# ProjectZKM/Ziren

Measured on AMD Instinct MI355X. Metric: shard-proofs/sec, higher is better.
Workload: dtype u32

## Files before the change

### ziren_amd/csrc/api_tracegen.hpp

```cpp
#pragma once
size_t zkm_tracegen_alu_width(int chip) { return chip >= 0 && chip < tracegen::NUM_ALU_CHIPS ? (size_t)tracegen::chip_width(chip) : 0; }

static size_t padded_trace_rows(size_t n_records, int fixed_log2_rows, const char* what) {
  size_t height = 16;
  if (fixed_log2_rows >= 0) {
    if (fixed_log2_rows > 30) throw std::runtime_error(std::string(what) + ": fixed log2 rows out of range");
    height = (size_t)1 << fixed_log2_rows;
    if (n_records > height) throw std::runtime_error(std::string(what) + ": fixed log2 rows is too small");
  } else {
    while (height < n_records) height <<= 1;
  }
  return height;
}

struct TraceBatch {
  zkm_ctx* ctx;
  std::vector<void*> scratch;
  std::vector<zkm_matrix*> made;
  std::vector<std::vector<zkm_syscall_event>> host_keep;
  enum { F_CPU, F_GLOBAL, F_SYSCALL_CORE };
  static constexpr int MAX_FLAGS = 256;
  uint32_t* d_flags = nullptr;
  std::vector<int> flag_kind;
  explicit TraceBatch(zkm_ctx* c) : ctx(c) {}
  zkm_matrix* matrix(size_t h, size_t w) {
    zkm_matrix* m = new zkm_matrix();
    made.push_back(m);
    m->h = h; m->w = w;
    m->d = ctx->alloc_n<uint32_t>(std::max<size_t>(h * w, 1));
    return m;
  }
  void* temp(size_t bytes) { void* p = ctx->alloc(bytes); scratch.push_back(p); return p; }
  const uint32_t* events(const void* ev, size_t bytes) {
    uint32_t* owned = nullptr;
    const uint32_t* d = ctx->events_on_device(ev, bytes, &owned);
    if (owned) scratch.push_back(owned);
    return d;
  }
  uint32_t* flag(int kind) {
    if (!d_flags) {
      d_flags = (uint32_t*)temp(MAX_FLAGS * 4);
      HIP_CHECK(hipMemsetAsync(d_flags, 0, MAX_FLAGS * 4, ctx->stream));
    }
    if ((int)flag_kind.size() == MAX_FLAGS) throw std::runtime_error("zkm_tracegen: too many generators in one batch");
    flag_kind.push_back(kind);
    return d_flags + flag_kind.size() - 1;
  }
  void finish(const char* mark) {
    const uint32_t* h_flags = flag_kind.empty() ? nullptr : ctx->download_async(d_flags, flag_kind.size());
    ctx->mark(mark);
    ctx->end_timing(false);
    for (size_t i = 0; i < flag_kind.size(); i++) {
      const uint32_t f = h_flags[i];
      if (!f) continue;
      if (flag_kind[i] == F_CPU) {
        if (f & 1) throw std::runtime_error("zkm_tracegen_cpu: an event's pc lies outside the program");
        throw std::runtime_error("zkm_tracegen_cpu: an event's clock does not fit 24 bits (a shard holds fewer than 2^24 / 5 cycles)");
      }
      if (flag_kind[i] == F_GLOBAL) {
        if (f & tracegen::GLOBAL_ERR_NOT_U16) throw std::runtime_error("zkm_tracegen_global: message[0] of an event is not a u16");
        if (f & tracegen::GLOBAL_ERR_NO_POINT) throw std::runtime_error("zkm_tracegen_global: a message has no curve point within 256 offsets");
        if (f & tracegen::GLOBAL_ERR_INFINITY) throw std::runtime_error("zkm_tracegen_global: the running sum reached the point at infinity");
        throw std::runtime_error("zkm_tracegen_global: a message's point has the running sum's x-coordinate");
      }
      throw std::runtime_error("zkm_tracegen_syscall: fixed log2 rows is too small");
    }
    for (void* p : scratch) ctx->release(p);
    scratch.clear();
    made.clear();
    host_keep.clear();
  }
  void abort() {
    (void)hipStreamSynchronize(ctx->stream);
    for (void* p : scratch) ctx->release(p);
    for (zkm_matrix* m : made) { if (m->d) ctx->release(m->d); delete m; }
    scratch.clear(); made.clear(); host_keep.clear();
  }
};

static zkm_matrix* enqueue_rows(TraceBatch& b, int chip, const void* events, size_t n_events, int fixed_log2_rows, zkm_byte_lookups* blu,
                                const uint32_t* n_dev = nullptr, const uint32_t* dev_events_given = nullptr, size_t height_given = 0) {
  static_assert(sizeof(zkm_alu_event) == 28 && sizeof(zkm_jump_event) == 28 && sizeof(zkm_mov_cond_event) == 28 &&
                sizeof(zkm_comp_alu_event) == 64, "event records mirror the #[repr(C)] executor structs");
  zkm_ctx* ctx = b.ctx;
  if (chip < 0 || chip >= tracegen::NUM_CHIPS) throw std::runtime_error("zkm_tracegen: unknown chip");
  if (n_events && !events && !dev_events_given) throw std::runtime_error("zkm_tracegen: null events");
  const size_t height = height_given ? height_given : padded_trace_rows(n_events, fixed_log2_rows, "zkm_tracegen_alu");
  const size_t w = (size_t)tracegen::chip_width(chip);
  zkm_matrix* m = b.matrix(height, w);
  m->uniform_rows = n_events == 0 && !n_dev && !dev_events_given;
  const size_t event_bytes = 4 * (size_t)tracegen::event_words(chip);
  const uint32_t* dev_events = dev_events_given ? dev_events_given : b.events(events, n_events * event_bytes);
  uint32_t* counts = blu ? blu->counts : nullptr;
  if (n_dev) {
    if (chip != tracegen::SYSCALL_CORE) throw std::runtime_error("zkm_tracegen: a device-side event count is for SyscallCore only");
    const int tiles = counts ? tracegen::TILES_PER_BLOCK : 1;
    KLAUNCH(ctx, "tracegen_alu", event_bytes * n_events + 4.0 * height * w, tracegen::alu_rows_counted<tracegen::SYSCALL_CORE>,
            dim3(div_up(height, (size_t)tiles * tracegen::THREADS)), dim3(tracegen::THREADS), counts ? 2 * tracegen::HASH_SLOTS * sizeof(uint32_t) : 0,
            dev_events, n_dev, height, m->d, counts, tiles);
    return m;
  }
  switch (chip) {
    case tracegen::ADD_SUB: launch_alu_rows<tracegen::ADD_SUB>(ctx, dev_events, n_events, height, m->d, counts); break;
    case tracegen::BITWISE: launch_alu_rows<tracegen::BITWISE>(ctx, dev_events, n_events, height, m->d, counts); break;
    case tracegen::LT: launch_alu_rows<tracegen::LT>(ctx, dev_events, n_events, height, m->d, counts); break;
    case tracegen::SHIFT_LEFT: launch_alu_rows<tracegen::SHIFT_LEFT>(ctx, dev_events, n_events, height, m->d, counts); break;
    case tracegen::SHIFT_RIGHT: launch_alu_rows<tracegen::SHIFT_RIGHT>(ctx, dev_events, n_events, height, m->d, counts); break;
    case tracegen::CLO_CLZ: launch_alu_rows<tracegen::CLO_CLZ>(ctx, dev_events, n_events, height, m->d, counts); break;
    case tracegen::JUMP: launch_alu_rows<tracegen::JUMP>(ctx, dev_events, n_events, height, m->d, counts); break;
    case tracegen::MOV_COND: launch_alu_rows<tracegen::MOV_COND>(ctx, dev_events, n_events, height, m->d, counts); break;
    case tracegen::BRANCH: launch_alu_rows<tracegen::BRANCH>(ctx, dev_events, n_events, height, m->d, counts); break;
    case tracegen::MUL: launch_alu_rows<tracegen::MUL>(ctx, dev_events, n_events, height, m->d, counts); break;
    case tracegen::DIVREM: launch_alu_rows<tracegen::DIVREM>(ctx, dev_events, n_events, height, m->d, counts); break;
    case tracegen::MEMORY_INSTRS: launch_alu_rows<tracegen::MEMORY_INSTRS>(ctx, dev_events, n_events, height, m->d, counts); break;
    case tracegen::SYSCALL_INSTRS: launch_alu_rows<tracegen::SYSCALL_INSTRS>(ctx, dev_events, n_events, height, m->d, counts); break;
    case tracegen::MISC_INSTRS: launch_alu_rows<tracegen::MISC_INSTRS>(ctx, dev_events, n_events, height, m->d, counts); break;
    case tracegen::SYSCALL_CORE: launch_alu_rows<tracegen::SYSCALL_CORE>(ctx, dev_events, n_events, height, m->d, counts); break;
    case tracegen::SYSCALL_PRECOMPILE: launch_alu_rows<tracegen::SYSCALL_PRECOMPILE>(ctx, dev_events, n_events, height, m->d, counts); break;
  }
  return m;
}

static int tracegen_single(zkm_ctx* ctx, zkm_matrix** out, const std::function<zkm_matrix*(TraceBatch&)>& enqueue) {
  API_BEGIN
  std::lock_guard<std::mutex> lk(ctx->mu);
  HIP_CHECK(hipSetDevice(ctx->device));
  CallScope call_scope(ctx);
  ctx->begin_timing();
  TraceBatch b(ctx);
  zkm_matrix* m = nullptr;
  try {
    m = enqueue(b);
    b.finish("trace generation");
  } catch (...) {
    b.abort();
    throw;
  }
  *out = m;
  API_END
}

static int tracegen_events(zkm_ctx* ctx, int chip, const void* events, size_t n_events, int fixed_log2_rows,
                           zkm_byte_lookups* blu, zkm_matrix** out) {
  return tracegen_single(ctx, out, [&](TraceBatch& b) { return enqueue_rows(b, chip, events, n_events, fixed_log2_rows, blu); });
}

int zkm_tracegen_alu(zkm_ctx* ctx, int chip, const zkm_alu_event* events, size_t n_events, int fixed_log2_rows,
                     zkm_byte_lookups* blu, zkm_matrix** out) {
  if (chip < 0 || chip >= tracegen::NUM_ALU_CHIPS) { g_err = "zkm_tracegen_alu: unknown chip"; return -1; }
  return tracegen_events(ctx, chip, events, n_events, fixed_log2_rows, blu, out);
}
size_t zkm_tracegen_jump_width(void) { return (size_t)tracegen::chip_width(tracegen::JUMP); }
int zkm_tracegen_jump(zkm_ctx* ctx, const zkm_jump_event* events, size_t n_events, int fixed_log2_rows, zkm_matrix** out) {
  return tracegen_events(ctx, tracegen::JUMP, events, n_events, fixed_log2_rows, nullptr, out);
}

static zkm_matrix* enqueue_flat(TraceBatch& b, const uint32_t* words, size_t n_words, size_t width, int fixed_log2_rows) {
  zkm_ctx* ctx = b.ctx;
  if (width == 0) throw std::runtime_error("zkm_tracegen_flat: zero width");
  if (n_words && !words) throw std::runtime_error("zkm_tracegen_flat: null records");
  const size_t rows = (n_words + width - 1) / width;
  size_t height = 16;
  if (fixed_log2_rows >= 0) {
    if (fixed_log2_rows > 30) throw std::runtime_error("zkm_tracegen_flat: fixed log2 rows out of range");
    height = (size_t)1 << fixed_log2_rows;
    if (rows > height) throw std::runtime_error("zkm_tracegen_flat: fixed log2 rows is too small");
  } else {
    while (height < rows) height <<= 1;
  }
  zkm_matrix* m = b.matrix(height, width);
  m->uniform_rows = n_words == 0;
  const uint32_t* dev = n_words ? b.events(words, n_words * 4) : nullptr;
  ctx->flush_staged();
  hipLaunchKernelGGL(open::flat_rows, dim3(div_up(width, 32), div_up(height, 32)), dim3(32, 8), 0, ctx->stream, dev, n_words, m->d, width, height);
  LAUNCH_CHECK();
  return m;
}
int zkm_tracegen_flat(zkm_ctx* ctx, const uint32_t* words, size_t n_words, size_t width, int fixed_log2_rows, zkm_matrix** out) {
  return tracegen_single(ctx, out, [&](TraceBatch& b) { return enqueue_flat(b, words, n_words, width, fixed_log2_rows); });
}

size_t zkm_tracegen_branch_width(void) { return (size_t)tracegen::chip_width(tracegen::BRANCH); }
int zkm_tracegen_branch(zkm_ctx* ctx, const zkm_branch_event* events, size_t n_events, int fixed_log2_rows, zkm_byte_lookups* blu,
                        zkm_matrix** out) {
  return tracegen_events(ctx, tracegen::BRANCH, events, n_events, fixed_log2_rows, blu, out);
}
size_t zkm_tracegen_mul_width(void) { return (size_t)tracegen::chip_width(tracegen::MUL); }
int zkm_tracegen_mul(zkm_ctx* ctx, const zkm_comp_alu_event* events, size_t n_events, int fixed_log2_rows, zkm_byte_lookups* blu,
                     zkm_matrix** out) {
  return tracegen_events(ctx, tracegen::MUL, events, n_events, fixed_log2_rows, blu, out);
}
size_t zkm_tracegen_memory_instrs_width(void) { return (size_t)tracegen::chip_width(tracegen::MEMORY_INSTRS); }
int zkm_tracegen_memory_instrs(zkm_ctx* ctx, const zkm_mem_instr_event* events, size_t n_events, int fixed_log2_rows, zkm_byte_lookups* blu,
                               zkm_matrix** out) {
  static_assert(sizeof(zkm_mem_instr_event) == 64, "event records mirror the #[repr(C)] executor structs");
  return tracegen_events(ctx, tracegen::MEMORY_INSTRS, events, n_events, fixed_log2_rows, blu, out);
}
size_t zkm_tracegen_syscall_instrs_width(void) { return (size_t)tracegen::chip_width(tracegen::SYSCALL_INSTRS); }
int zkm_tracegen_syscall_instrs(zkm_ctx* ctx, const zkm_syscall_event* events, size_t n_events, int fixed_log2_rows, zkm_matrix** out) {
  static_assert(sizeof(zkm_syscall_event) == 56, "event records mirror the #[repr(C)] executor structs");
  return tracegen_events(ctx, tracegen::SYSCALL_INSTRS, events, n_events, fixed_log2_rows, nullptr, out);
}
size_t zkm_tracegen_misc_instrs_width(void) { return (size_t)tracegen::chip_width(tracegen::MISC_INSTRS); }
int zkm_tracegen_misc_instrs(zkm_ctx* ctx, const zkm_misc_event* events, size_t n_events, int fixed_log2_rows, zkm_byte_lookups* blu,
                             zkm_matrix** out) {
  static_assert(sizeof(zkm_misc_event) == 60, "event records mirror the #[repr(C)] executor structs");
  return tracegen_events(ctx, tracegen::MISC_INSTRS, events, n_events, fixed_log2_rows, blu, out);
}
size_t zkm_tracegen_divrem_width(void) { return (size_t)tracegen::chip_width(tracegen::DIVREM); }
int zkm_tracegen_divrem(zkm_ctx* ctx, const zkm_comp_alu_event* events, size_t n_events, int fixed_log2_rows, zkm_byte_lookups* blu,
                        zkm_matrix** out) {
  return tracegen_events(ctx, tracegen::DIVREM, events, n_events, fixed_log2_rows, blu, out);
}
size_t zkm_tracegen_mov_cond_width(void) { return (size_t)tracegen::chip_width(tracegen::MOV_COND); }
int zkm_tracegen_mov_cond(zkm_ctx* ctx, const zkm_mov_cond_event* events, size_t n_events, int fixed_log2_rows, zkm_matrix** out) {
  return tracegen_events(ctx, tracegen::MOV_COND, events, n_events, fixed_log2_rows, nullptr, out);
}

size_t zkm_tracegen_cpu_width(void) { return (size_t)tracegen::CPU_WIDTH; }
static zkm_matrix* enqueue_cpu(TraceBatch& b, const zkm_cpu_event* events, size_t n_events, const zkm_instruction* program, size_t n_instr,
                               uint32_t pc_base, uint32_t shard, int fixed_log2_rows, int program_fixed_log2_rows, zkm_byte_lookups* blu,
                               zkm_matrix** program_mults_out) {
  static_assert(sizeof(zkm_cpu_event) == 4 * tracegen::CPU_EVENT_WORDS && sizeof(zkm_instruction) == 4 * tracegen::INSTRUCTION_WORDS,
                "event records mirror the #[repr(C)] executor structs");
  zkm_ctx* ctx = b.ctx;
  if (n_events && (!events || !program || !n_instr)) throw std::runtime_error("zkm_tracegen_cpu: null events or program");
  const size_t height = padded_trace_rows(n_events, fixed_log2_rows, "zkm_tracegen_cpu");
  const size_t pheight = program_mults_out ? padded_trace_rows(n_instr, program_fixed_log2_rows, "zkm_tracegen_cpu (program)") : 0;
  zkm_matrix* m = b.matrix(height, tracegen::CPU_WIDTH);
  zkm_matrix* pm = program_mults_out ? b.matrix(pheight, 1) : nullptr;
  if (pm) HIP_CHECK(hipMemsetAsync(pm->d, 0, pheight * 4, ctx->stream));
  const uint32_t* dev_events = b.events(events, n_events * sizeof(zkm_cpu_event));
  const uint32_t* d_program = (const uint32_t*)ctx->upload_staged(program, n_instr * sizeof(zkm_instruction), &b.scratch);
  uint32_t* d_bad = b.flag(TraceBatch::F_CPU);
  uint32_t* counts = blu ? blu->counts : nullptr;
  const int tiles = counts ? tracegen::TILES_PER_BLOCK : 1;
  KLAUNCH(ctx, "tracegen_cpu", 280.0 * n_events + 4.0 * height * tracegen::CPU_WIDTH, tracegen::cpu_rows,
          dim3(div_up(height, (size_t)tiles * tracegen::THREADS)), dim3(tracegen::THREADS),
          counts ? 2 * tracegen::HASH_SLOTS * sizeof(uint32_t) : 0, dev_events, n_events, d_program, n_instr,
          pc_base, shard, height, m->d, counts, tiles, (int*)d_bad, pm ? pm->d : (uint32_t*)nullptr);
  if (pm) {
    hipLaunchKernelGGL(tracegen::counts_to_field, dim3(div_up(pheight, 256)), dim3(256), 0, ctx->stream, pm->d, pheight);
    LAUNCH_CHECK();
    *program_mults_out = pm;
  }
  return m;
}

int zkm_tracegen_cpu_and_program(zkm_ctx* ctx, const zkm_cpu_event* events, size_t n_events, const zkm_instruction* program, size_t n_instr,
                                 uint32_t pc_base, uint32_t shard, int fixed_log2_rows, int program_fixed_log2_rows, zkm_byte_lookups* blu,
                                 zkm_matrix** out, zkm_matrix** program_mults_out) {
  zkm_matrix* pm = nullptr;
  const int rc = tracegen_single(ctx, out, [&](TraceBatch& b) {
    return enqueue_cpu(b, events, n_events, program, n_instr, pc_base, shard, fixed_log2_rows, program_fixed_log2_rows, blu, program_mults_out ? &pm : nullptr);
  });
  if (rc == 0 && program_mults_out) *program_mults_out = pm;
  return rc;
}

int zkm_tracegen_cpu(zkm_ctx* ctx, const zkm_cpu_event* events, size_t n_events, const zkm_instruction* program, size_t n_instr,
                     uint32_t pc_base, uint32_t shard, int fixed_log2_rows, zkm_byte_lookups* blu, zkm_matrix** out) {
  return zkm_tracegen_cpu_and_program(ctx, events, n_events, program, n_instr, pc_base, shard, fixed_log2_rows, -1, blu, out, nullptr);
}

int zkm_tracegen_program(zkm_ctx* ctx, const zkm_instruction* program, size_t n_instr, uint32_t pc_base, int fixed_log2_rows,
                         zkm_matrix** out) {
  API_BEGIN
  std::lock_guard<std::mutex> lk(ctx->mu);
  HIP_CHECK(hipSetDevice(ctx->device));
  CallScope call_scope(ctx);
  if (n_instr && !program) throw std::runtime_error("zkm_tracegen_program: null program");
  const size_t height = padded_trace_rows(n_instr, fixed_log2_rows, "zkm_tracegen_program");
  ctx->begin_call();
  zkm_matrix* m = new zkm_matrix();
  m->h = height; m->w = tracegen::PROGRAM_PREP_WIDTH;
  uint32_t* d_program = nullptr;
  try {
    m->d = ctx->alloc_n<uint32_t>(height * m->w);
    d_program = (uint32_t*)ctx->alloc(std::max<size_t>(n_instr * sizeof(zkm_instruction), 4));
    if (n_instr) HIP_CHECK(hipMemcpyAsync(d_program, program, n_instr * sizeof(zkm_instruction), hipMemcpyHostToDevice, ctx->stream));
    hipLaunchKernelGGL(tracegen::program_rows, dim3(div_up(height, 256)), dim3(256), 0, ctx->stream, (const uint32_t*)d_program, n_instr,
                       pc_base, height, m->d);
    LAUNCH_CHECK();
    ctx->sync(ctx->stream);
  } catch (...) {
    if (d_program) ctx->release(d_program);
    if (m->d) ctx->release(m->d);
    delete m;
    throw;
  }
  ctx->release(d_program);
  *out = m;
  API_END
}

int zkm_tracegen_program_mults(zkm_ctx* ctx, const zkm_cpu_event* events, size_t n_events, size_t n_instr, uint32_t pc_base,
                               int fixed_log2_rows, zkm_matrix** out) {
  API_BEGIN
  std::lock_guard<std::mutex> lk(ctx->mu);
  HIP_CHECK(hipSetDevice(ctx->device));
  CallScope call_scope(ctx);
  if (n_events && !events) throw std::runtime_error("zkm_tracegen_program_mults: null events");
  const size_t height = padded_trace_rows(n_instr, fixed_log2_rows, "zkm_tracegen_program_mults");
  ctx->begin_call();
  zkm_matrix* m = new zkm_matrix();
  m->h = height; m->w = 1;
  uint32_t* d_events = nullptr;
  try {
    m->d = ctx->alloc_n<uint32_t>(height);
    HIP_CHECK(hipMemsetAsync(m->d, 0, height * 4, ctx->stream));
    const uint32_t* dev_events = ctx->events_on_device(events, n_events * sizeof(zkm_cpu_event), &d_events);
    if (n_events) {
      hipLaunchKernelGGL(tracegen::program_count, dim3(div_up(n_events, 256)), dim3(256), 0, ctx->stream, dev_events, n_events,
                         n_instr, pc_base, m->d);
      LAUNCH_CHECK();
    }
    hipLaunchKernelGGL(tracegen::counts_to_field, dim3(div_up(height, 256)), dim3(256), 0, ctx->stream, m->d, height);
    LAUNCH_CHECK();
    ctx->sync(ctx->stream);
  } catch (...) {
    if (d_events) ctx->release(d_events);
    if (m->d) ctx->release(m->d);
    delete m;
    throw;
  }
  ctx->release(d_events);
  *out = m;
  API_END
}

static zkm_matrix* enqueue_memory_local(TraceBatch& b, const zkm_memory_local_event* events, size_t n_events, int fixed_log2_rows) {
  static_assert(sizeof(zkm_memory_local_event) == 28, "event records mirror the #[repr(C)] executor structs");
  zkm_ctx* ctx = b.ctx;
  if (n_events && !events) throw std::runtime_error("zkm_tracegen_memory_local: null events");
  const size_t height = padded_trace_rows(div_up(n_events, (size_t)tracegen::MEMORY_LOCAL_ENTRIES), fixed_log2_rows, "zkm_tracegen_memory_local");
  zkm_matrix* m = b.matrix(height, tracegen::MEMORY_LOCAL_WIDTH);
  const uint32_t* dev_events = b.events(events, n_events * sizeof(zkm_memory_local_event));
  ctx->flush_staged();
  hipLaunchKernelGGL(tracegen::memory_local_rows, dim3(div_up(height * tracegen::MEMORY_LOCAL_ENTRIES, (size_t)256)), dim3(256), 0, ctx->stream,
                     dev_events, n_events, height, m->d);
  LAUNCH_CHECK();
  return m;
}

int zkm_tracegen_memory_local(zkm_ctx* ctx, const zkm_memory_local_event* events, size_t n_events, int fixed_log2_rows, zkm_matrix** out) {
  return tracegen_single(ctx, out, [&](TraceBatch& b) { return enqueue_memory_local(b, events, n_events, fixed_log2_rows); });
}

static zkm_matrix* enqueue_global(TraceBatch& b, const zkm_global_lookup_event* events, size_t n_events, int fixed_log2_rows, zkm_byte_lookups* blu) {
  static_assert(sizeof(zkm_global_lookup_event) == 32, "event records mirror the #[repr(C)] executor structs");
  zkm_ctx* ctx = b.ctx;
  if (n_events && !events) throw std::runtime_error("zkm_tracegen_global: null events");
  if (!blu) throw std::runtime_error("zkm_tracegen_global: null byte lookups");
  const size_t height = padded_trace_rows(n_events, fixed_log2_rows, "zkm_tracegen_global");
  zkm_matrix* m = b.matrix(height, tracegen::GLOBAL_WIDTH);
  const uint32_t* d_events = b.events(events, n_events * sizeof(zkm_global_lookup_event));
  uint32_t* d_err = b.flag(TraceBatch::F_GLOBAL);
  std::vector<uint32_t*> levels;
  std::vector<size_t> sizes;
  for (size_t n = n_events + 1;; n = div_up(n, (size_t)tracegen::SCAN_CHUNK)) {
    levels.push_back((uint32_t*)b.temp(n * tracegen::POINT_WORDS * sizeof(uint32_t)));
    sizes.push_back(n);
    if (n <= (size_t)tracegen::SCAN_BLOCK) break;
  }
  const double bytes = 32.0 * n_events + 4.0 * height * tracegen::GLOBAL_WIDTH;
  KLAUNCH(ctx, "tracegen_global_points", bytes, tracegen::global_point_rows, dim3(div_up(height, (size_t)256)), dim3(256), 0,
          d_events, n_events, height, m->d, levels[0], blu->counts, d_err);
  for (size_t l = 0; l + 1 < levels.size(); l++)
    KLAUNCH(ctx, "tracegen_global_scan", 64.0 * sizes[l], tracegen::global_scan_reduce, dim3(div_up(sizes[l + 1], (size_t)64)), dim3(64), 0,
            (const uint32_t*)levels[l], sizes[l], levels[l + 1], sizes[l + 1]);
  KLAUNCH(ctx, "tracegen_global_scan", 128.0 * sizes.back(), tracegen::global_scan_block, dim3(1), dim3(tracegen::SCAN_BLOCK), 0, levels.back(),
          sizes.back());
  for (size_t l = levels.size() - 1; l-- > 0;)
    KLAUNCH(ctx, "tracegen_global_scan", 128.0 * sizes[l], tracegen::global_scan_apply, dim3(div_up(sizes[l + 1], (size_t)64)), dim3(64), 0, levels[l],
            sizes[l], (const uint32_t*)levels[l + 1], sizes[l + 1]);
  KLAUNCH(ctx, "tracegen_global_accum", bytes, tracegen::global_accum_rows, dim3(div_up(height, (size_t)256)), dim3(256), 0,
          (const uint32_t*)levels[0], n_events, height, m->d, d_err);
  return m;
}

int zkm_tracegen_global(zkm_ctx* ctx, const zkm_global_lookup_event* events, size_t n_events, int fixed_log2_rows, zkm_byte_lookups* blu,
                        zkm_matrix** out) {
  return tracegen_single(ctx, out, [&](TraceBatch& b) { return enqueue_global(b, events, n_events, fixed_log2_rows, blu); });
}

static zkm_matrix* enqueue_poseidon2_wide(TraceBatch& b, const uint32_t* events, size_t n_events, int fixed_log2_rows) {
  zkm_ctx* ctx = b.ctx;
  if (n_events && !events) throw std::runtime_error("zkm_tracegen_poseidon2_wide: null events");
  const size_t height = padded_trace_rows(n_events, fixed_log2_rows, "zkm_tracegen_poseidon2_wide");
  zkm_matrix* m = b.matrix(height, tracegen::POSEIDON2_WIDE_WIDTH);
  const uint32_t* d_events = n_events ? b.events(events, n_events * 128) : (const uint32_t*)b.temp(4);
  KLAUNCH(ctx, "tracegen_poseidon2_wide", 128.0 * n_events + 4.0 * height * tracegen::POSEIDON2_WIDE_WIDTH, tracegen::poseidon2_wide_rows,
          dim3(div_up(height, (size_t)tracegen::THREADS)), dim3(tracegen::THREADS), 0, d_events, n_events, height, m->d);
  return m;
}
int zkm_tracegen_poseidon2_wide(zkm_ctx* ctx, const uint32_t* events, size_t n_events, int fixed_log2_rows, zkm_matrix** out) {
  return tracegen_single(ctx, out, [&](TraceBatch& b) { return enqueue_poseidon2_wide(b, events, n_events, fixed_log2_rows); });
}

static zkm_matrix* enqueue_syscall(TraceBatch& b, const zkm_syscall_event* events, size_t n_events, int precompile, int fixed_log2_rows, zkm_byte_lookups* blu) {
  static_assert(sizeof(zkm_syscall_event) == 56, "event records mirror the #[repr(C)] executor structs");
  zkm_ctx* ctx = b.ctx;
  if (precompile) return enqueue_rows(b, tracegen::SYSCALL_PRECOMPILE, events, n_events, fixed_log2_rows, blu);
  if (n_events && !events) throw std::runtime_error("zkm_tracegen: null events");
  if (n_events && ctx->prefetched.count(events)) {
    const uint32_t* d_all = b.events(events, n_events * sizeof(zkm_syscall_event));
    const size_t cap = fixed_log2_rows >= 0 ? std::min(n_events, padded_trace_rows(0, fixed_log2_rows, "zkm_tracegen_syscall")) : n_events;
    uint32_t* d_kept = (uint32_t*)b.temp(cap * sizeof(zkm_syscall_event));
    uint32_t* d_n = (uint32_t*)b.temp(4);
    uint32_t* d_flag = b.flag(TraceBatch::F_SYSCALL_CORE);
    KLAUNCH(ctx, "tracegen_syscall_compact", 2.0 * n_events * sizeof(zkm_syscall_event), tracegen::syscall_core_compact, dim3(1), dim3(1024), 0,
            d_all, n_events, d_kept, d_n, cap, d_flag);
    if (fixed_log2_rows < 0) {
      const uint32_t* h_n = ctx->download_async(d_n, 1);
      ctx->sync(ctx->stream);
      return enqueue_rows(b, tracegen::SYSCALL_CORE, nullptr, *h_n, -1, blu, nullptr, d_kept);
    }
    return enqueue_rows(b, tracegen::SYSCALL_CORE, nullptr, cap, fixed_log2_rows, blu, d_n, d_kept, (size_t)1 << fixed_log2_rows);
  }
  b.host_keep.emplace_back();
  std::vector<zkm_syscall_event>& kept = b.host_keep.back();
  for (size_t i = 0; i < n_events; i++) {
    const uint32_t code = events[i].a_record.prev_value;
    if (((code >> 16) & 0xff) == 1 || ((code >> 8) & 0xff) != 0) kept.push_back(events[i]);
  }
  return enqueue_rows(b, tracegen::SYSCALL_CORE, kept.empty() ? nullptr : (const void*)kept.data(), kept.size(), fixed_log2_rows, blu);
}

int zkm_tracegen_syscall(zkm_ctx* ctx, const zkm_syscall_event* events, size_t n_events, int precompile, int fixed_log2_rows, zkm_byte_lookups* blu,
                         zkm_matrix** out) {
  return tracegen_single(ctx, out, [&](TraceBatch& b) { return enqueue_syscall(b, events, n_events, precompile, fixed_log2_rows, blu); });
}

int zkm_tracegen_memory_global(zkm_ctx* ctx, const zkm_memory_init_finalize_event* events, size_t n_events, uint32_t previous_addr, int fixed_log2_rows,
                               zkm_matrix** out) {
  API_BEGIN
  static_assert(sizeof(zkm_memory_init_finalize_event) == 16, "event records mirror the #[repr(C)] executor structs");
  std::lock_guard<std::mutex> lk(ctx->mu);
  HIP_CHECK(hipSetDevice(ctx->device));
  CallScope call_scope(ctx);
  if (n_events && !events) throw std::runtime_error("zkm_tracegen_memory_global: null events");
  const size_t height = padded_trace_rows(n_events, fixed_log2_rows, "zkm_tracegen_memory_global");
  std::vector<zkm_memory_init_finalize_event> sorted(events, events + n_events);
  std::stable_sort(sorted.begin(), sorted.end(), [](const zkm_memory_init_finalize_event& a, const zkm_memory_init_finalize_event& b) { return a.addr < b.addr; });
  ctx->begin_timing();
  zkm_matrix* m = new zkm_matrix();
  m->h = height; m->w = tracegen::MEMORY_GLOBAL_WIDTH;
  uint32_t* d_events = nullptr;
  int* d_bad = nullptr;
  try {
    m->d = ctx->alloc_n<uint32_t>(height * m->w);
    d_events = (uint32_t*)ctx->alloc(std::max<size_t>(n_events * 16, 4));
    d_bad = (int*)ctx->alloc(4);
    HIP_CHECK(hipMemsetAsync(d_bad, 0, 4, ctx->stream));
    if (n_events) HIP_CHECK(hipMemcpyAsync(d_events, sorted.data(), n_events * 16, hipMemcpyHostToDevice, ctx->stream));
    KLAUNCH(ctx, "tracegen_memory_global", 16.0 * n_events + 4.0 * height * m->w, tracegen::memory_global_rows, dim3(div_up(height, (size_t)tracegen::THREADS)),
            dim3(tracegen::THREADS), 0, (const uint32_t*)d_events, n_events, previous_addr, height, m->d, d_bad);
    int bad = 0;
    HIP_CHECK(hipMemcpyAsync(&bad, d_bad, 4, hipMemcpyDeviceToHost, ctx->stream));
    ctx->mark("trace generation");
    ctx->end_timing(false);
    if (bad) throw std::runtime_error("zkm_tracegen_memory_global: addresses are not strictly increasing (from the previous shard's last address on)");
  } catch (...) {
    if (d_events) ctx->release(d_events);
    if (d_bad) ctx->release(d_bad);
    if (m->d) ctx->release(m->d);
    delete m;
    throw;
  }
  ctx->release(d_events);
  ctx->release(d_bad);
  *out = m;
  API_END
}

int zkm_tracegen_poseidon2_permute(zkm_ctx* ctx, const zkm_poseidon2_permute_event* events, size_t n_events, int fixed_log2_rows, zkm_byte_lookups* blu,
                                   zkm_matrix** out) {
  API_BEGIN
  static_assert(sizeof(zkm_poseidon2_permute_event) == 4 * tracegen::POSEIDON2_PERMUTE_EVENT_WORDS, "flattened Poseidon2PermuteEvent is 99 words");
  std::lock_guard<std::mutex> lk(ctx->mu);
  HIP_CHECK(hipSetDevice(ctx->device));
  CallScope call_scope(ctx);
  if (n_events && !events) throw std::runtime_error("zkm_tracegen_poseidon2_permute: null events");
  const size_t height = padded_trace_rows(n_events, fixed_log2_rows, "zkm_tracegen_poseidon2_permute");
  ctx->begin_timing();
  zkm_matrix* m = new zkm_matrix();
  m->h = height; m->w = tracegen::POSEIDON2_PERMUTE_WIDTH;
  uint32_t* d_events = nullptr;
  int* d_bad = nullptr;
  try {
    m->d = ctx->alloc_n<uint32_t>(height * m->w);
    const size_t ev_bytes = n_events * sizeof(zkm_poseidon2_permute_event);
    d_events = (uint32_t*)ctx->alloc(std::max<size_t>(ev_bytes, 4));
    d_bad = (int*)ctx->alloc(4);
    HIP_CHECK(hipMemsetAsync(d_bad, 0, 4, ctx->stream));
    if (n_events) HIP_CHECK(hipMemcpyAsync(d_events, events, ev_bytes, hipMemcpyHostToDevice, ctx->stream));
    uint32_t* counts = blu ? blu->counts : nullptr;
    KLAUNCH(ctx, "tracegen_poseidon2_permute", (double)ev_bytes + 4.0 * height * m->w, tracegen::poseidon2_permute_rows,
            dim3(div_up(height, (size_t)tracegen::THREADS)), dim3(tracegen::THREADS), counts ? 2 * tracegen::HASH_SLOTS * sizeof(uint32_t) : 0,
            (const uint32_t*)d_events, n_events, height, m->d, counts, d_bad);
    int bad = 0;
    HIP_CHECK(hipMemcpyAsync(&bad, d_bad, 4, hipMemcpyDeviceToHost, ctx->stream));
    ctx->mark("trace generation");
    ctx->end_timing(false);
    if (bad) throw std::runtime_error("zkm_tracegen_poseidon2_permute: a state word is not a field element, or the post-state is not the permutation of the pre-state");
  } catch (...) {
    if (d_events) ctx->release(d_events);
    if (d_bad) ctx->release(d_bad);
    if (m->d) ctx->release(m->d);
    delete m;
    throw;
  }
  ctx->release(d_events);
  ctx->release(d_bad);
  *out = m;
  API_END
}

int zkm_tracegen_keccak_sponge(zkm_ctx* ctx, const zkm_keccak_sponge_block* blocks, size_t n_blocks, int fixed_log2_rows, zkm_byte_lookups* blu,
                               zkm_matrix** out) {
  API_BEGIN
  static_assert(sizeof(zkm_keccak_sponge_block) == 4 * tracegen::KECCAK_SPONGE_BLOCK_WORDS, "a KeccakSpongeEvent block is 337 words");
  std::lock_guard<std::mutex> lk(ctx->mu);
  HIP_CHECK(hipSetDevice(ctx->device));
  CallScope call_scope(ctx);
  if (n_blocks && !blocks) throw std::runtime_error("zkm_tracegen_keccak_sponge: null blocks");
  const size_t height = padded_trace_rows(24 * n_blocks, fixed_log2_rows, "zkm_tracegen_keccak_sponge");
  ctx->begin_timing();
  zkm_matrix* m = new zkm_matrix();
  m->h = height; m->w = tracegen::KECCAK_SPONGE_WIDTH;
  uint32_t* d_blocks = nullptr;
  int* d_bad = nullptr;
// ... 875 lines not shown
```

### ziren_amd/csrc/host_ctx.hpp

```cpp
#pragma once
static thread_local std::string g_err;

#define HIP_CHECK(expr)                                                                          \
  do {                                                                                           \
    hipError_t _e = (expr);                                                                      \
    if (_e != hipSuccess)                                                                        \
      throw std::runtime_error(std::string(#expr) + ": " + hipGetErrorString(_e) + " (" + __FILE__ + ":" + \
                               std::to_string(__LINE__) + ")");                                  \
  } while (0)
#define LAUNCH_CHECK() HIP_CHECK(hipGetLastError())
#define KLAUNCH(ctx, name, bytes, kernel, grid, block, lds, ...)                                        \
  do {                                                                                                   \
    (ctx)->flush_staged();                                                                               \
    if ((ctx)->kbegin(name, (double)(bytes))) {                                                          \
       \
      hipExtLaunchKernelGGL(kernel, grid, block, lds, (ctx)->cur, (ctx)->krecs.back().start,             \
                            (ctx)->krecs.back().stop, 0, __VA_ARGS__);                                   \
    } else {                                                                                             \
      hipLaunchKernelGGL(kernel, grid, block, lds, (ctx)->cur, __VA_ARGS__);                             \
    }                                                                                                    \
    LAUNCH_CHECK();                                                                                      \
  } while (0)

static inline int log2_strict(size_t n) {
  int k = 0;
  while (((size_t)1 << k) < n) k++;
  if (((size_t)1 << k) != n) throw std::runtime_error("height is not a power of two");
  return k;
}
static inline unsigned div_up(size_t a, size_t b) { return (unsigned)((a + b - 1) / b); }
static inline uint64_t fnv1a(const uint32_t* w, size_t n);
static inline uint64_t perm_key(const uint32_t* lookups, size_t len, uint32_t log_quotient_degree) {
  return fnv1a(lookups, len) * 1099511628211ull + log_quotient_degree + 1;
}
static inline uint64_t fnv1a(const uint32_t* w, size_t n) {
  uint64_t h = 1469598103934665603ull;
  const unsigned char* p = (const unsigned char*)w;
  for (size_t i = 0; i < n * 4; i++) { h ^= p[i]; h *= 1099511628211ull; }
  return h;
}

namespace chal {
static void duplexing(zkm_challenger* c) {
  for (uint32_t i = 0; i < c->num_inputs; i++) c->sponge_state[i] = c->input_buffer[i];
  c->num_inputs = 0;
  p2::permute_host(c->sponge_state);
  for (int i = 0; i < 8; i++) c->output_buffer[i] = c->sponge_state[i];
  c->num_outputs = 8;
}
static void observe(zkm_challenger* c, uint32_t v) {
  c->num_outputs = 0;
  c->input_buffer[c->num_inputs++] = v;
  if (c->num_inputs == 8) duplexing(c);
}
static void observe_slice(zkm_challenger* c, const uint32_t* v, size_t n) {
  for (size_t i = 0; i < n; i++) observe(c, v[i]);
}
static void observe_ext(zkm_challenger* c, const E4& e) { observe_slice(c, e.c, 4); }
static uint32_t sample(zkm_challenger* c) {
  if (c->num_inputs != 0 || c->num_outputs == 0) duplexing(c);
  return c->output_buffer[--c->num_outputs];
}
static E4 sample_ext(zkm_challenger* c) {
  E4 e;
  for (int i = 0; i < 4; i++) e.c[i] = sample(c);
  return e;
}
static uint32_t sample_bits(zkm_challenger* c, uint32_t bits) {
  return kb::from_monty(sample(c)) & ((1u << bits) - 1);
}
}

enum HandleKind { H_MATRIX = 1, H_PCS_DATA = 2, H_PK = 3, H_MAIN_DATA = 4 };
struct HandleTable {
  std::mutex mu;
  std::unordered_map<const void*, int> live;
  static HandleTable& get() { static HandleTable t; return t; }
  void add(const void* p, int kind) { std::lock_guard<std::mutex> lk(mu); live[p] = kind; }
  void drop(const void* p) { std::lock_guard<std::mutex> lk(mu); live.erase(p); }
  bool is_live(const void* p, int kind) { std::lock_guard<std::mutex> lk(mu); auto it = live.find(p); return it != live.end() && it->second == kind; }
};
template <int KIND>
struct Handle {
  Handle() { HandleTable::get().add(this, KIND); }
  Handle(const Handle&) { HandleTable::get().add(this, KIND); }
  Handle& operator=(const Handle&) { return *this; }
  ~Handle() { HandleTable::get().drop(this); }
};
static inline void check_handle(const void* p, int kind, const char* fn, const char* what) {
  if (!p) throw std::runtime_error(std::string(fn) + ": null " + what);
  if (!HandleTable::get().is_live(p, kind)) throw std::runtime_error(std::string(fn) + ": " + what + " is not a live handle (freed, or never returned by this library)");
}

struct zkm_ctx {
  int device = 0;
  hipStream_t stream = nullptr;
  hipStream_t stream2 = nullptr;
  hipStream_t up_dma = nullptr, up_tr = nullptr;
  uint32_t* up_stage[2] = {nullptr, nullptr};
  hipEvent_t up_freed[2] = {nullptr, nullptr}, up_landed[2] = {nullptr, nullptr};
  bool up_freed_set[2] = {false, false};
  int up_next = 0;
  static constexpr size_t UP_SLAB_BYTES = (size_t)32 << 20;
  hipStream_t cur = nullptr;
  hipStream_t ev_dma = nullptr;
  struct Prefetched { size_t bytes; hipEvent_t landed; };
  std::map<const void*, Prefetched> prefetched;
  const uint32_t* events_on_device(const void* events, size_t bytes, uint32_t** owned) {
    *owned = nullptr;
    auto it = prefetched.find(events);
    if (it != prefetched.end()) {
      if (bytes > it->second.bytes) throw std::runtime_error("zkm_tracegen: more events asked for than zkm_events_upload_async copied");
      HIP_CHECK(hipStreamWaitEvent(stream, it->second.landed, 0));
      return (const uint32_t*)events;
    }
    uint32_t* d = (uint32_t*)alloc(std::max<size_t>(bytes, 4));
    *owned = d;
    if (bytes) HIP_CHECK(hipMemcpyAsync(d, events, bytes, hipMemcpyHostToDevice, stream));
    return d;
  }
  std::mutex mu;
  std::multimap<size_t, void*> free_list;
  std::map<void*, size_t> live;
  std::map<int, uint32_t*> tw_fwd, tw_inv;
  std::vector<std::pair<std::string, hipEvent_t>> marks;
  std::vector<hipEvent_t> event_pool;
  std::vector<std::string> timing_names;
  std::vector<float> timing_ms;
  struct KRec { const char* name; double bytes; hipEvent_t start, stop; };
  struct KStat { double ms = 0, bytes = 0; uint32_t calls = 0; };
  std::vector<KRec> krecs;
  std::map<std::string, KStat> kstats;
  int kernel_timing = 2;
  bool lde_overlap = !(getenv("ZKM_LDE_OVERLAP") && atoi(getenv("ZKM_LDE_OVERLAP")) == 0);
  bool rows_up_front = !(getenv("ZKM_ROWS_UP_FRONT") && atoi(getenv("ZKM_ROWS_UP_FRONT")) == 0);
  bool root_poll = !(getenv("ZKM_ROOT_POLL") && atoi(getenv("ZKM_ROOT_POLL")) == 0);
  int root_spin_before_yield = getenv("ZKM_ROOT_SPIN") ? atoi(getenv("ZKM_ROOT_SPIN")) : 4096;
  int root_sleep_ns = getenv("ZKM_ROOT_SLEEP_NS") ? atoi(getenv("ZKM_ROOT_SLEEP_NS")) : 0;
  bool host_wait_blocking = getenv("ZKM_HOST_WAIT") && !strcmp(getenv("ZKM_HOST_WAIT"), "blocking");
  int wait_sleep_ns = getenv("ZKM_WAIT_SLEEP_NS") ? atoi(getenv("ZKM_WAIT_SLEEP_NS")) : 20000;
  struct TimerSlack {
    long saved = -1;
    void tighten() {
      if (saved >= 0) return;
      saved = prctl(PR_GET_TIMERSLACK, 0, 0, 0, 0);
      if (saved >= 0) prctl(PR_SET_TIMERSLACK, 1000UL, 0, 0, 0);
    }
    ~TimerSlack() { if (saved >= 0) prctl(PR_SET_TIMERSLACK, (unsigned long)saved, 0, 0, 0); }
  };
  static void sleep_ns(long ns, TimerSlack& slack) {
    slack.tighten();
    timespec ts{0, ns};
    nanosleep(&ts, nullptr);
  }
  void sync(hipStream_t s) {
    if (!host_wait_blocking) { HIP_CHECK(hipStreamSynchronize(s)); return; }
    TimerSlack slack;
    for (int i = 0;; i++) {
      const hipError_t e = hipStreamQuery(s);
      if (e == hipSuccess) return;
      if (e != hipErrorNotReady) HIP_CHECK(e);
      if (i >= 4) sleep_ns(wait_sleep_ns, slack);
    }
  }
  std::map<uint64_t, std::vector<hipFunction_t>> quotient_fns;
  std::map<uint64_t, hipFunction_t> quotient_uniform_fns;
  std::map<uint64_t, hipFunction_t> perm_fns;
  std::vector<hipModule_t> modules;
  hipEvent_t get_event() {
    hipEvent_t e;
    if (!event_pool.empty()) { e = event_pool.back(); event_pool.pop_back(); }
    else HIP_CHECK(hipEventCreate(&e));
    return e;
  }
  std::string timing_only;
  bool kbegin(const char* name, double bytes) {
    if (!(kernel_timing == 1 || (kernel_timing == 2 && bytes >= 262144.0) || (kernel_timing == 3 && timing_only == name))) return false;
    KRec r{name, bytes, get_event(), get_event()};
    krecs.push_back(r);
    return true;
  }

  char* pin = nullptr;
  size_t pin_cap = (size_t)32 << 20, pin_off = 0;
  void* pin_alloc(size_t bytes) {
    if (!pin) HIP_CHECK(hipHostMalloc((void**)&pin, pin_cap, hipHostMallocCoherent));
    size_t off = (pin_off + 63) & ~(size_t)63;
    if (off + bytes > pin_cap) return nullptr;
    pin_off = off + bytes;
    return pin + off;
  }
  void begin_call() {
    sync(stream);
    sync(stream2);
    cur = stream;
    side_join();
    pin_off = 0;
    dirty_lo = SIZE_MAX; dirty_hi = 0;
  }
  char* arena = nullptr;
  size_t dirty_lo = SIZE_MAX, dirty_hi = 0;
  void* upload_staged(const void* src, size_t bytes, std::vector<void*>* scratch = nullptr) {
    const size_t room = bytes ? bytes : 4;
    void* h = room <= ((size_t)1 << 20) ? pin_alloc(room) : nullptr;
    if (!h) return upload(src, bytes, scratch);
    if (!arena) HIP_CHECK(hipMalloc((void**)&arena, pin_cap));
    if (bytes) memcpy(h, src, bytes);
    bytes = room;
    const size_t off = (char*)h - pin;
    dirty_lo = std::min(dirty_lo, off);
    dirty_hi = std::max(dirty_hi, off + bytes);
    return arena + off;
  }
  void flush_staged() {
    if (dirty_hi <= dirty_lo) return;
    HIP_CHECK(hipMemcpyAsync(arena + dirty_lo, pin + dirty_lo, dirty_hi - dirty_lo, hipMemcpyHostToDevice, stream));
    dirty_lo = SIZE_MAX; dirty_hi = 0;
    if (cur != stream) {
      hipEvent_t e = get_event();
      HIP_CHECK(hipEventRecord(e, stream));
      HIP_CHECK(hipStreamWaitEvent(cur, e, 0));
      event_pool.push_back(e);
    }
  }
  std::vector<void*> side_deferred;
  hipEvent_t side_done = nullptr;
  bool side_pending = false;
  void release_here(void* p) {
    if (cur != stream) side_deferred.push_back(p);
    else release(p);
  }
  void side_begin() {
    hipEvent_t e = get_event();
    HIP_CHECK(hipEventRecord(e, stream));
    HIP_CHECK(hipStreamWaitEvent(stream2, e, 0));
    event_pool.push_back(e);
    cur = stream2;
  }
  void side_end() {
    if (!side_done) HIP_CHECK(hipEventCreateWithFlags(&side_done, hipEventDisableTiming));
    HIP_CHECK(hipEventRecord(side_done, stream2));
    cur = stream;
    side_pending = true;
  }
  void side_join() {
    if (!side_pending) return;
    HIP_CHECK(hipStreamWaitEvent(stream, side_done, 0));
    for (void* p : side_deferred) release(p);
    side_deferred.clear();
    side_pending = false;
  }
  void* upload(const void* src, size_t bytes, std::vector<void*>* scratch) {
    void* d = alloc(bytes);
    if (scratch) scratch->push_back(d);
    if (bytes == 0) return d;
    void* h = pin_alloc(bytes);
    if (h) {
      memcpy(h, src, bytes);
      HIP_CHECK(hipMemcpyAsync(d, h, bytes, hipMemcpyHostToDevice, cur));
    } else {
      HIP_CHECK(hipMemcpyAsync(d, src, bytes, hipMemcpyHostToDevice, cur));
      sync(cur);
    }
    return d;
  }
  template <class T>
  T* download_async(const T* dev, size_t count) {
    T* h = (T*)pin_alloc(count * sizeof(T));
    if (!h) throw std::runtime_error("pinned staging ring exhausted");
    HIP_CHECK(hipMemcpyAsync(h, dev, count * sizeof(T), hipMemcpyDeviceToHost, stream));
    return h;
  }

  size_t pool_bytes = 0;
  size_t pool_limit = getenv("ZKM_POOL_LIMIT_MB") ? (size_t)atoll(getenv("ZKM_POOL_LIMIT_MB")) << 20 : 0;
  std::vector<void*> call_allocs;
  int call_depth = 0;
  void drop_cached() {
    if (free_list.empty()) return;
    (void)hipStreamSynchronize(stream);
    if (stream2) (void)hipStreamSynchronize(stream2);
    for (auto& kv : free_list) { (void)hipFree(kv.second); pool_bytes -= kv.first; }
    free_list.clear();
  }
  void* alloc(size_t bytes) {
    if (bytes == 0) bytes = 4;
    bytes = (bytes + 255) & ~(size_t)255;
    auto it = free_list.find(bytes);
    void* p;
    if (it != free_list.end()) {
      p = it->second;
      free_list.erase(it);
    } else {
      if (pool_limit && pool_bytes + bytes > pool_limit) drop_cached();
      if (pool_limit && pool_bytes + bytes > pool_limit)
        throw std::runtime_error("out of device memory: " + std::to_string(bytes) + " bytes on top of " + std::to_string(pool_bytes) +
                                 " held would cross the context's pool limit of " + std::to_string(pool_limit) + " bytes");
      hipError_t e = hipMalloc(&p, bytes);
      if (e != hipSuccess) {
        (void)hipGetLastError();
        drop_cached();
        e = hipMalloc(&p, bytes);
      }
      if (e != hipSuccess) {
        (void)hipGetLastError();
        throw std::runtime_error(std::string("out of device memory: hipMalloc of ") + std::to_string(bytes) + " bytes failed (" + hipGetErrorString(e) + "), " +
                                 std::to_string(pool_bytes) + " bytes held by this context's pool");
      }
      pool_bytes += bytes;
    }
    live[p] = bytes;
    if (call_depth > 0) call_allocs.push_back(p);
    return p;
  }
  template <class T>
  T* alloc_n(size_t n) { return (T*)alloc(n * sizeof(T)); }
  void release(void* p) {
    if (!p) return;
    auto it = live.find(p);
    if (it == live.end()) return;
    free_list.insert({it->second, p});
    live.erase(it);
  }
  void mark(const char* name) {
    hipEvent_t e = get_event();
    HIP_CHECK(hipEventRecord(e, stream));
    marks.push_back({name, e});
  }
  void begin_timing() {
    begin_call();
    for (auto& m : marks) event_pool.push_back(m.second);
    marks.clear();
    for (auto& r : krecs) { event_pool.push_back(r.start); if (r.stop) event_pool.push_back(r.stop); }
    krecs.clear();
    mark("begin");
  }
  void end_timing(bool append) {
    sync(stream);
    sync(stream2);
    if (!append) { timing_names.clear(); timing_ms.clear(); kstats.clear(); }
    for (auto& r : krecs) {
      float ms = 0;
      if (r.stop) HIP_CHECK(hipEventElapsedTime(&ms, r.start, r.stop));
      KStat& k = kstats[r.name];
      k.ms += ms; k.bytes += r.bytes; k.calls++;
    }
    for (size_t i = 1; i < marks.size(); i++) {
      float ms = 0;
      HIP_CHECK(hipEventElapsedTime(&ms, marks[i - 1].second, marks[i].second));
      timing_names.push_back(marks[i].first);
      timing_ms.push_back(ms);
    }
  }
  const uint32_t* twiddles(int log_size, bool inverse) {
    auto& tab = inverse ? tw_inv : tw_fwd;
    auto it = tab.find(log_size);
    if (it != tab.end()) return it->second;
    size_t count = (size_t)1 << log_size;
    uint32_t* d;
    HIP_CHECK(hipMalloc(&d, count * 4));
    uint32_t w = kb::two_adic_generator(log_size);
    if (inverse) w = kb::inv(w);
    if (log_size > 0) {
      hipLaunchKernelGGL(lde::fill_stage_twiddles, dim3(div_up(count / 2, 256), log_size), dim3(256), 0, stream, d, w, log_size);
      LAUNCH_CHECK();
    }
    tab[log_size] = d;
    return d;
  }
  std::map<int, uint32_t*> ct_fwd, ct_inv;
  const uint32_t* twiddles_ct(int log_size, bool inverse) {
    auto& tab = inverse ? ct_inv : ct_fwd;
    auto it = tab.find(log_size);
    if (it != tab.end()) return it->second;
    const size_t count = (size_t)1 << log_size;
    uint32_t* d;
    HIP_CHECK(hipMalloc(&d, count * 4));
    uint32_t w = kb::two_adic_generator(log_size);
    if (inverse) w = kb::inv(w);
    hipLaunchKernelGGL(lde::fill_ct_twiddles, dim3(div_up(count, 256)), dim3(256), 0, stream, d, w, log_size);
    LAUNCH_CHECK();
    tab[log_size] = d;
    return d;
  }
  std::map<int, std::pair<uint32_t*, uint32_t*>> pow_tabs;
  std::pair<const uint32_t*, const uint32_t*> pow_tables(int k) {
    auto it = pow_tabs.find(k);
    if (it != pow_tabs.end()) return {it->second.first, it->second.second};
    const uint32_t n_hi = (uint32_t)(((size_t)1 << k) >> 10);
    uint32_t *lo, *hi;
    HIP_CHECK(hipMalloc(&lo, 1024 * 4));
    HIP_CHECK(hipMalloc(&hi, std::max<uint32_t>(n_hi, 1) * 4));
    hipLaunchKernelGGL(lde::fill_pow_tables, dim3(div_up(std::max<uint32_t>(1024, n_hi), 256)), dim3(256), 0, stream, lo, hi,
                       kb::two_adic_generator(k), n_hi);
    LAUNCH_CHECK();
    pow_tabs[k] = {lo, hi};
    return {lo, hi};
  }
  std::map<std::pair<int, int>, uint32_t*> selector_tabs;
  const uint32_t* selectors(int log_n, int lqd, uint32_t w_q, uint32_t g_inv, const uint32_t* d_consts) {
    auto key = std::make_pair(log_n, lqd);
    auto it = selector_tabs.find(key);
    if (it != selector_tabs.end()) return it->second;
    const size_t Q = (size_t)1 << (log_n + lqd);
    uint32_t* d;
    HIP_CHECK(hipMalloc(&d, 3 * Q * 4));
    flush_staged();
    hipLaunchKernelGGL(stark::fill_selectors, dim3(div_up(Q, 256)), dim3(256), 0, cur, d, log_n + lqd, lqd, w_q, g_inv, d_consts);
    LAUNCH_CHECK();
    selector_tabs[key] = d;
    return d;
  }
  std::map<int, uint32_t*> row_tabs;
  const uint32_t* row_twiddles(int k) {
    auto it = row_tabs.find(k);
    if (it != row_tabs.end()) return it->second;
    const int lb = lde::LOG_ROW_MAX, la = k - lb;
    const size_t n = (size_t)1 << k;
    uint32_t* d;
    HIP_CHECK(hipMalloc(&d, n * 4));
    auto pw = pow_tables(k);
    hipLaunchKernelGGL(lde::fill_row_twiddles, dim3(div_up(n, 256)), dim3(256), 0, stream, d, la, lb, pw.first, pw.second);
    LAUNCH_CHECK();
    row_tabs[k] = d;
    return d;
  }
  struct CosetTabs { uint32_t* twf; uint32_t* cs; };
  std::map<std::tuple<int, int, uint32_t>, CosetTabs> coset_tabs;
  CosetTabs coset_tables(int k, int bl, uint32_t shift) {
    auto key = std::make_tuple(k, bl, shift);
    auto it = coset_tabs.find(key);
    if (it != coset_tabs.end()) return it->second;
    const int lb = lde::LOG_ROW_MAX, la = k - lb;
    const size_t B = (size_t)1 << lb, A = (size_t)1 << la, cosets = (size_t)1 << bl;
    CosetTabs t;
    HIP_CHECK(hipMalloc(&t.twf, cosets * B * 4));
    HIP_CHECK(hipMalloc(&t.cs, cosets * A * 4));
    const uint32_t w_N = kb::two_adic_generator(k + bl), w_B = kb::two_adic_generator(lb);
    const uint32_t n_inv = kb::inv(kb::to_monty((uint32_t)(((size_t)1 << k) % kb::P)));
    uint32_t sj = shift;
    for (size_t j = 0; j < cosets; j++) {
      uint32_t sA = sj;
      for (int i = 0; i < la; i++) sA = kb::sqr(sA);
      hipLaunchKernelGGL(lde::fill_scaled_stage_twiddles, dim3(div_up(B / 2, 256), lb), dim3(256), 0, stream, t.twf + j * B, w_B, lb, sA);
      LAUNCH_CHECK();
      sj = kb::mul(sj, w_N);
    }
    hipLaunchKernelGGL(lde::fill_row_scales, dim3(div_up(A * cosets, 256)), dim3(256), 0, stream, t.cs, shift, w_N, n_inv, (uint32_t)A, (uint32_t)cosets);
    LAUNCH_CHECK();
    coset_tabs[key] = t;
    return t;
  }
  void drop_coset_tables() {
    for (auto& kv : coset_tabs) { (void)hipFree(kv.second.twf); (void)hipFree(kv.second.cs); }
    coset_tabs.clear();
  }
};

struct zkm_matrix : Handle<H_MATRIX> {
  uint32_t* d = nullptr;
  size_t h = 0, w = 0;
  bool owned = true;
  bool uniform_rows = false;
  hipEvent_t ready = nullptr;
};

static inline void wait_ready(hipStream_t stream, const zkm_matrix& m) {
  if (m.ready) HIP_CHECK(hipStreamWaitEvent(stream, m.ready, 0));
}

struct zkm_byte_lookups {
  uint32_t* counts = nullptr;
};

struct Tree {
  const uint32_t* h_root = nullptr;
  uint32_t* digests = nullptr;
  std::vector<size_t> layer_off;
  size_t max_height = 0;
  int log_max = 0;
  const uint32_t* node(int layer, size_t i) const { return digests + (layer_off[layer] + i) * 8; }
};

struct zkm_pcs_data : Handle<H_PCS_DATA> {
  std::vector<zkm_matrix> ldes;
  std::vector<const uint32_t*> evals;
  std::vector<size_t> eval_heights;
  std::vector<uint32_t> domain_shifts;
  std::vector<zkm_matrix> owned_evals;
  Tree tree;
  uint32_t root[8];
  int log_blowup = 1;
  uint32_t* cflags = nullptr;
  std::vector<const uint32_t*> col_flags;
};

struct zkm_pk : Handle<H_PK> {
  std::vector<zkm_matrix> prep;
  std::vector<uint32_t> local_only;
  zkm_pcs_data* data = nullptr;
  uint32_t commit[8];
  uint32_t pc_start;
  uint32_t igcs[14];
};

struct zkm_main_data : Handle<H_MAIN_DATA> {
  std::vector<size_t> order;
  std::vector<zkm_matrix> traces;
  zkm_pcs_data* data = nullptr;
  std::vector<uint32_t> public_values;
};
```

### ziren_amd/csrc/host_open.hpp

```cpp
#pragma once
static E4 host_pow2k(E4 a, int k) { return kb::epow2k(a, k); }

struct Writer {
  uint32_t* dst;
  size_t cap, n = 0;
  Writer(uint32_t* d, size_t c) : dst(d), cap(d ? c : 0) {}
  void u(uint32_t v) { if (n < cap) dst[n] = v; n++; }
  void words(const uint32_t* p, size_t cnt) {
    if (n < cap) memcpy(dst + n, p, std::min(cnt, cap - n) * 4);
    n += cnt;
  }
  void ext(const E4& e) { words(e.c, 4); }
  size_t size() const { return n; }
};

struct RoundMat {
  const uint32_t* evals; size_t n; size_t width; uint32_t shift;
  const zkm_matrix* lde;
  int n_points;
  std::vector<E4> y[2];
  size_t col0 = 0;
};
struct Round { const zkm_pcs_data* data; std::vector<RoundMat> mats; };

static const uint32_t SEPTIC_X[7] = {637514027, 1595065213, 1998064738, 72333738, 1211544370, 822986770, 1518535784};
static const uint32_t SEPTIC_Y[7] = {1604177449, 90440090, 259343427, 140470264, 1162099742, 941559812, 1064053343};

struct ChipMeta {
  const zkm_chip_desc* desc;
  int log_n;
  size_t n;
  int n_lookups, n_sends, perm_ext_w, max_values;
};

static ChipMeta chip_meta(const zkm_chip_desc* d, size_t n, size_t n_public_values) {
  ChipMeta m;
  m.desc = d; m.n = n; m.log_n = log2_strict(n);
  m.n_lookups = m.n_sends = m.max_values = 0;
  const std::string who = std::string(" (chip ") + (d->name ? d->name : "?") + ")";
  if (d->log_quotient_degree > 3) throw std::runtime_error("log_quotient_degree > 3 unsupported" + who);
  if (d->lookups_len) {
    const uint32_t* w = d->lookups;
    const size_t len = d->lookups_len;
    size_t pos = 0;
    auto need = [&](size_t k) { if (pos + k > len) throw std::runtime_error("lookup blob truncated" + who); };
    need(2);
    uint32_t ns = w[pos++], nr = w[pos++];
    if ((uint64_t)ns + nr > 4096) throw std::runtime_error("too many lookups" + who);
    m.n_sends = ns; m.n_lookups = ns + nr;
    for (uint32_t i = 0; i < ns + nr; i++) {
      need(2);
      pos++;
      uint32_t nv = w[pos++];
      if (nv > 64) throw std::runtime_error("lookup with more than 64 values" + who);
      m.max_values = std::max<int>(m.max_values, nv);
      for (uint32_t v = 0; v <= nv; v++) {
        need(2);
        uint32_t nt = w[pos++];
        if (w[pos++] >= kb::P) throw std::runtime_error("lookup constant not a field element" + who);
        need(2 * (size_t)nt);
        for (uint32_t t = 0; t < nt; t++) {
          uint32_t cw = w[pos++], weight = w[pos++];
          uint32_t col = cw & 0x7fffffffu;
          if ((cw >> 31) ? col >= d->main_width : col >= d->prep_width) throw std::runtime_error("lookup column out of range" + who);
          if (weight >= kb::P) throw std::runtime_error("lookup weight not a field element" + who);
        }
      }
    }
    if (pos != len) throw std::runtime_error("lookup blob length mismatch" + who);
  }
  int batch = 1 << d->log_quotient_degree;
  m.perm_ext_w = m.n_lookups ? (m.n_lookups + batch - 1) / batch + 1 : 0;
  if (d->program_len) {
    if (d->program_len < 4 || d->program_len != 4 + 2 * (size_t)d->program[0]) throw std::runtime_error("program blob length mismatch" + who);
    if (d->program[2] != d->num_constraints) throw std::runtime_error("program constraint count mismatch" + who);
    const uint32_t ne = std::max<uint32_t>(d->program[1], 1), nb = std::max<uint32_t>(d->program[3], 1);
    if (ne > 256 || nb > 256) throw std::runtime_error("program register count out of range" + who);
    size_t asserts = 0;
    for (uint32_t k = 0; k < d->program[0]; k++) {
      uint32_t w0 = d->program[4 + 2 * k], imm = d->program[5 + 2 * k];
      uint32_t op = w0 & 0xff, dst = (w0 >> 8) & 0xff, ra = (w0 >> 16) & 0xff, rb = w0 >> 24;
      bool ok = true;
      switch (op) {
        case ZKM_OP_LD_MAIN: ok = dst < nb && ra < 2 && imm < d->main_width; break;
        case ZKM_OP_LD_PREP: ok = dst < nb && ra < 2 && imm < d->prep_width; break;
        case ZKM_OP_LD_PERM: ok = dst < ne && ra < 2 && imm < (uint32_t)m.perm_ext_w; break;
        case ZKM_OP_LD_CONST: ok = dst < nb && imm < kb::P; break;
        case ZKM_OP_LD_PV: ok = dst < nb && imm < n_public_values; break;
        case ZKM_OP_LD_CHALLENGE: ok = dst < ne && imm < 2; break;
        case ZKM_OP_LD_LOCAL_SUM: ok = dst < ne; break;
        case ZKM_OP_LD_GLOBAL_SUM: ok = dst < nb && imm < 14; break;
        case ZKM_OP_LD_IS_FIRST: case ZKM_OP_LD_IS_LAST: case ZKM_OP_LD_IS_TRANS: ok = dst < nb; break;
        case ZKM_OP_ADD_B: case ZKM_OP_SUB_B: case ZKM_OP_MUL_B: ok = dst < nb && ra < nb && rb < nb; break;
        case ZKM_OP_NEG_B: ok = dst < nb && ra < nb; break;
        case ZKM_OP_ADD_E: case ZKM_OP_SUB_E: case ZKM_OP_MUL_E: ok = dst < ne && ra < ne && rb < ne; break;
        case ZKM_OP_NEG_E: ok = dst < ne && ra < ne; break;
        case ZKM_OP_ADD_EB: case ZKM_OP_SUB_EB: case ZKM_OP_MUL_EB: ok = dst < ne && ra < ne && rb < nb; break;
        case ZKM_OP_ASSERT_B: ok = ra < nb; asserts++; break;
        case ZKM_OP_ASSERT_E: ok = ra < ne; asserts++; break;
        default: ok = false;
      }
      if (!ok) throw std::runtime_error("invalid instruction " + std::to_string(k) + " in constraint program" + who);
    }
    if (asserts != d->num_constraints) throw std::runtime_error("program asserts do not match num_constraints" + who);
  } else if (d->num_constraints) {
    throw std::runtime_error("num_constraints > 0 but no program" + who);
  }
  return m;
}

template <typename Alloc>
static void launch_permutation_trace(zkm_ctx* ctx, const ChipMeta& c, const uint32_t* d_blob, const uint32_t* trace, const uint32_t* prep, const E4& alpha,
                                     const E4* d_beta_powers, zkm_matrix& pt, Alloc&& salloc, std::vector<stark::ScanJob>& scans) {
  const double pbytes = 4.0 * c.n * (c.desc->main_width + c.desc->prep_width + pt.w);
  auto fit = c.desc->lookups_len ? ctx->perm_fns.find(perm_key(c.desc->lookups, c.desc->lookups_len, c.desc->log_quotient_degree)) : ctx->perm_fns.end();
  if (fit != ctx->perm_fns.end()) {
    stark::PermArgs a;
    a.main = trace; a.prep = prep; a.n = c.n; a.alpha = alpha; a.beta_pows = d_beta_powers; a.perm = pt.d;
    size_t arg_size = sizeof(a);
    void* config[] = {HIP_LAUNCH_PARAM_BUFFER_POINTER, &a, HIP_LAUNCH_PARAM_BUFFER_SIZE, &arg_size, HIP_LAUNCH_PARAM_END};
    ctx->flush_staged();
    const bool timed = ctx->kbegin("perm_rows", pbytes);
    HIP_CHECK(hipExtModuleLaunchKernel(fit->second, div_up(c.n, 256) * 256, 1, 1, 256, 1, 1, 0, ctx->cur, nullptr, config,
                                       timed ? ctx->krecs.back().start : nullptr, timed ? ctx->krecs.back().stop : nullptr, 0));
  } else {
    KLAUNCH(ctx, "perm_rows", pbytes, stark::perm_rows, dim3(div_up(c.n, stark::THREADS)), dim3(stark::THREADS), 0,
            d_blob, c.n_lookups, c.n_sends, 1 << c.desc->log_quotient_degree, trace, prep, c.n, alpha, d_beta_powers, pt.d, c.perm_ext_w);
  }
  stark::ScanJob j;
  j.data = pt.d + (size_t)(c.perm_ext_w - 1) * 4 * c.n;
  j.n = c.n;
  j.nchunks = (c.n + stark::SCAN_BLOCK - 1) / stark::SCAN_BLOCK;
  j.totals = (uint32_t*)salloc(j.nchunks * 4 * 4);
  j.blk_end = (scans.empty() ? 0 : scans.back().blk_end) + (uint32_t)(j.nchunks * 4);
  j.pad = 0;
  scans.push_back(j);
}
static void launch_scans(zkm_ctx* ctx, const std::vector<stark::ScanJob>& scans, std::vector<void*>* scratch) {
  if (scans.empty()) return;
  const stark::ScanJob* d = (const stark::ScanJob*)ctx->upload_staged(scans.data(), scans.size() * sizeof(stark::ScanJob), scratch);
  double bytes = 0;
  bool multi = false;
  for (auto& j : scans) { bytes += 32.0 * j.n; multi |= j.nchunks > 1; }
  KLAUNCH(ctx, "scan", bytes, stark::scan_chunks, dim3(scans.back().blk_end), dim3(stark::THREADS), 0, d);
  if (multi) {
    KLAUNCH(ctx, "scan", 0.0, stark::scan_totals, dim3((unsigned)(4 * scans.size())), dim3(stark::THREADS), 0, d);
    KLAUNCH(ctx, "scan", bytes, stark::scan_add_offsets, dim3(scans.back().blk_end), dim3(stark::THREADS), 0, d);
  }
}

struct ShardOpening {
  struct Loose {
    zkm_ctx* ctx;
    std::vector<void*> v;
    void disown(void* p) { v.erase(std::remove(v.begin(), v.end(), p), v.end()); }
    ~Loose() { for (void* p : v) ctx->release(p); }
  };
  struct Guard { zkm_ctx* c; std::vector<zkm_pcs_data*> d; ~Guard() { for (auto p : d) free_pcs_data(c, p); } };

  zkm_ctx* ctx;
  const zkm_pk* pk;
  zkm_main_data* md;
  const zkm_fri_config* fri;
  uint32_t num_pv_elts;
  zkm_challenger* ch;
  hipStream_t st;
  const int bl;
  const size_t nc;
  std::vector<ChipMeta> chips;
  Loose loose;
  std::vector<void*>& scratch;
  Guard guard;
  E4 perm_ch[2];
  uint32_t* d_pv = nullptr;
  std::vector<zkm_matrix> perm_traces;
  std::vector<E4> local_sums;
  std::vector<std::array<uint32_t, 14>> global_sums;
  zkm_pcs_data* perm_data = nullptr;
  std::vector<zkm_matrix> qchunks;
  std::vector<uint32_t> qshifts;
  zkm_pcs_data* quot_data = nullptr;
  E4 zeta;
  std::vector<Round> rounds;
  int log_max = 0;
  std::vector<E4*> ro = std::vector<E4*>(32, nullptr);
  const uint32_t** col_ptr_lde = nullptr;
  const uint32_t** col_ptr_eval = nullptr;
  uint32_t* col_mask = nullptr;
  std::vector<E4*> layers;
  std::vector<Tree> ftrees;
  std::vector<std::array<uint32_t, 8>> commits;
  E4 final_poly;
  uint32_t pow_witness = 0;
  std::vector<size_t> indices;
  const uint32_t* gathered = nullptr;
  std::vector<uint32_t> gathered_big;

  void* salloc(size_t bytes) { void* p = ctx->alloc(bytes); scratch.push_back(p); return p; }

  ShardOpening(zkm_ctx* ctx_, const zkm_pk* pk_, zkm_main_data* md_, const zkm_chip_desc* chips_in, const zkm_fri_config* fri_, uint32_t num_pv_elts_,
               zkm_challenger* ch_)
      : ctx(ctx_), pk(pk_), md(md_), fri(fri_), num_pv_elts(num_pv_elts_), ch(ch_), st(ctx_->stream), bl((int)fri_->log_blowup), nc(md_->order.size()),
        loose{ctx_, {}}, scratch(loose.v), guard{ctx_, {}} {
  for (size_t i = 0; i < nc; i++) chips.push_back(chip_meta(&chips_in[md->order[i]], md->traces[i].h, md->public_values.size()));
  for (size_t i = 0; i < nc; i++) {
    if (chips[i].desc->main_width != md->traces[i].w) throw std::runtime_error("chip main_width does not match its trace");
    if ((int)chips[i].desc->log_quotient_degree > bl) throw std::runtime_error("log_quotient_degree > log_blowup unsupported");
    if (chips[i].desc->prep_index >= 0 && (!pk->data || (size_t)chips[i].desc->prep_index >= pk->prep.size()))
      throw std::runtime_error("chip references a preprocessed trace the proving key does not hold");
  }
  if (bl < 1 || bl > 4) throw std::runtime_error("fri.log_blowup out of range (1..4)");
  if (fri->proof_of_work_bits > 30) throw std::runtime_error("fri.proof_of_work_bits out of range (0..30)");
  if (fri->num_queries < 1 || fri->num_queries > 1024) throw std::runtime_error("fri.num_queries out of range (1..1024)");
  if (num_pv_elts > md->public_values.size()) throw std::runtime_error("num_pv_elts exceeds public_values length");
  chal::observe_slice(ch, md->public_values.data(), num_pv_elts);
  chal::observe_slice(ch, md->data->root, 8);
  perm_ch[0] = chal::sample_ext(ch);
  perm_ch[1] = chal::sample_ext(ch);
  d_pv = (uint32_t*)ctx->upload_staged(md->public_values.data(), md->public_values.size() * 4, &scratch);
  }

  void permutation_phase() {
  perm_traces.assign(nc, zkm_matrix());
  local_sums.assign(nc, kb::ezero());
  global_sums.assign(nc, std::array<uint32_t, 14>());
  std::vector<uint32_t*> d_blobs(nc, nullptr);
  std::vector<stark::ScanJob> scans;
  std::vector<const uint32_t*> sum_src;
  uint32_t* h_sums = nullptr;
  {
    int maxv = 0;
    for (auto& c : chips) maxv = std::max(maxv, c.max_values);
    std::vector<E4> bp(maxv + 2);
    bp[0] = kb::eone();
    for (int i = 1; i < maxv + 2; i++) bp[i] = kb::emul(bp[i - 1], perm_ch[1]);
    E4* d_bp = (E4*)ctx->upload_staged(bp.data(), bp.size() * sizeof(E4), &scratch);
    for (size_t i = 0; i < nc; i++)
      if (chips[i].perm_ext_w > 0) d_blobs[i] = (uint32_t*)ctx->upload_staged(chips[i].desc->lookups, chips[i].desc->lookups_len * 4, &scratch);
    for (size_t i = 0; i < nc; i++) {
      const ChipMeta& c = chips[i];
      zkm_matrix& pt = perm_traces[i];
      pt.h = c.n; pt.w = (size_t)c.perm_ext_w * 4;
      pt.d = ctx->alloc_n<uint32_t>(std::max<size_t>(pt.h * pt.w, 1));
      scratch.push_back(pt.d);
      if (c.perm_ext_w > 0) {
        const uint32_t* prep = c.desc->prep_index >= 0 ? pk->prep[c.desc->prep_index].d : nullptr;
        launch_permutation_trace(ctx, c, (const uint32_t*)d_blobs[i], (const uint32_t*)md->traces[i].d, prep, perm_ch[0], (const E4*)d_bp, pt,
                                 [&](size_t bytes) { return salloc(bytes); }, scans);
        uint32_t* last = pt.d + (size_t)(c.perm_ext_w - 1) * 4 * c.n;
        for (int e = 0; e < 4; e++) sum_src.push_back(last + (size_t)e * c.n + (c.n - 1));
      } else {
        for (int e = 0; e < 4; e++) sum_src.push_back(nullptr);
      }
      if (c.desc->commit_scope_global) {
        const zkm_matrix& m = md->traces[i];
        for (int k = 0; k < 14; k++) sum_src.push_back(m.d + (m.w - 14 + k) * m.h + (m.h - 1));
      } else {
        for (int k = 0; k < 14; k++) sum_src.push_back(nullptr);
      }
    }
    launch_scans(ctx, scans, &scratch);
    const uint32_t* d_zero = (const uint32_t*)ctx->upload_staged("\0\0\0\0", 4, &scratch);
    for (auto& p : sum_src) if (!p) p = d_zero;
    const uint32_t** d_sum_src = (const uint32_t**)ctx->upload_staged(sum_src.data(), sum_src.size() * sizeof(void*), &scratch);
    uint32_t* d_sums = (uint32_t*)salloc(sum_src.size() * 4);
    KLAUNCH(ctx, "gather_words", 0.0, open::gather_words, dim3(div_up(sum_src.size(), open::THREADS)), dim3(open::THREADS), 0,
            (const uint32_t* const*)d_sum_src, sum_src.size(), d_sums);
    h_sums = ctx->download_async(d_sums, sum_src.size());
  }
  ctx->mark("permutation traces");
  perm_data = pcs_commit(ctx, perm_traces, {}, bl);
  guard.d.push_back(perm_data);
  perm_data->owned_evals = perm_traces;
  for (auto& m : perm_traces) loose.disown(m.d);
  ctx->mark("commit permutation");
  for (size_t i = 0; i < nc; i++) {
    for (int e = 0; e < 4; e++) local_sums[i].c[e] = h_sums[18 * i + e];
    if (chips[i].desc->commit_scope_global) {
      for (int k = 0; k < 14; k++) global_sums[i][k] = h_sums[18 * i + 4 + k];
    } else {
      for (int k = 0; k < 7; k++) { global_sums[i][k] = kb::to_monty(SEPTIC_X[k]); global_sums[i][7 + k] = kb::to_monty(SEPTIC_Y[k]); }
    }
  }
  chal::observe_slice(ch, perm_data->root, 8);
  for (size_t i = 0; i < nc; i++) {
    chal::observe_ext(ch, local_sums[i]);
    chal::observe_slice(ch, global_sums[i].data(), 14);
  }
  }

  void quotient_phase() {
  E4 alpha = chal::sample_ext(ch);
  std::vector<std::function<void()>> launches;
  for (size_t i = 0; i < nc; i++) {
    const ChipMeta& c = chips[i];
    const zkm_chip_desc* d = c.desc;
    int lqd = d->log_quotient_degree;
    int lq = c.log_n + lqd;
    size_t Q = (size_t)1 << lq;
    size_t nchunks = (size_t)1 << lqd;
    uint32_t* qbuf = ctx->alloc_n<uint32_t>(Q * 4);
    scratch.push_back(qbuf);
    size_t C = d->num_constraints;
    std::vector<E4> ap(std::max<size_t>(C, 1));
    E4 p = kb::eone();
    for (size_t k = 0; k < C; k++) { ap[C - 1 - k] = p; p = kb::emul(p, alpha); }
    E4* d_ap = (E4*)ctx->upload_staged(ap.data(), ap.size() * sizeof(E4), &scratch);
    uint32_t consts[32] = {0};
    for (int k = 0; k < 14; k++) consts[k] = global_sums[i][k];
    uint32_t w_q = kb::two_adic_generator(lq);
    uint32_t s_pow_n = kb::pow(kb::GEN, (uint64_t)c.n);
    uint32_t wr = kb::two_adic_generator(lqd), wp = kb::ONE;
    for (size_t k = 0; k < nchunks; k++) {
      consts[16 + k] = kb::sub(kb::mul(s_pow_n, wp), kb::ONE);
      consts[24 + k] = kb::inv(consts[16 + k]);
      wp = kb::mul(wp, wr);
    }
    uint32_t* d_consts = (uint32_t*)ctx->upload_staged(consts, sizeof consts, &scratch);
    static const uint32_t empty_prog[4] = {0, 1, 0, 1};
    uint32_t* d_prog = (uint32_t*)ctx->upload_staged(d->program_len ? d->program : empty_prog, std::max<size_t>(d->program_len, 4) * 4, &scratch);
    stark::QuotientArgs a;
    a.program = d_prog + 4;
    a.n_instr = d->program_len ? d->program[0] : 0;
    a.n_regs = d->program_len ? d->program[1] : 1;
    a.main_lde = md->data->ldes[i].d; a.main_stride = md->data->ldes[i].h;
    a.prep_lde = d->prep_index >= 0 ? pk->data->ldes[d->prep_index].d : nullptr;
    a.prep_stride = d->prep_index >= 0 ? pk->data->ldes[d->prep_index].h : 0;
    a.perm_lde = perm_data->ldes[i].d; a.perm_stride = perm_data->ldes[i].h;
    a.log_n = c.log_n; a.lqd = lqd;
    a.alpha_pows = d_ap; a.public_values = d_pv;
    a.perm_alpha = perm_ch[0]; a.perm_beta = perm_ch[1];
    a.local_sum = local_sums[i];
    a.consts = d_consts;
    a.w_q = w_q; a.g_inv = kb::inv(kb::two_adic_generator(c.log_n));
    a.out = qbuf;
    a.selectors = ctx->selectors(c.log_n, lqd, w_q, a.g_inv, d_consts);
    a.n_base_regs = d->program_len ? std::max<uint32_t>(d->program[3], 1) : 1;
    size_t per_thread = (size_t)a.n_regs * 16 + (size_t)a.n_base_regs * 4;
    int bd = 256;
    while (per_thread * bd > 64 * 1024 && bd > 64) bd >>= 1;
    size_t lds = per_thread * bd;
    if (lds > 152 * 1024) throw std::runtime_error(std::string("constraint program of chip ") + d->name + " needs too many registers");
    double qbytes = 4.0 * Q * (d->main_width + d->prep_width + 4.0 * c.perm_ext_w) + 16.0 * Q;
    auto fit = d->program_len ? ctx->quotient_fns.find(fnv1a(d->program, d->program_len)) : ctx->quotient_fns.end();
    const bool special = fit != ctx->quotient_fns.end();
    const std::vector<hipFunction_t>* fns = special ? &fit->second : nullptr;
    hipFunction_t uni_fn = nullptr;
    a.uniforms = nullptr;
    if (special) {
      auto uit = ctx->quotient_uniform_fns.find(fit->first);
      if (uit != ctx->quotient_uniform_fns.end()) {
        uni_fn = uit->second;
        a.uniforms = ctx->alloc_n<uint32_t>(stark::QUOTIENT_UNIFORM_WORDS);
        scratch.push_back(a.uniforms);
      }
    }
    launches.push_back([this, a, fns, uni_fn, Q, bd, lds, qbytes]() mutable {
      if (fns) {
        size_t arg_size = sizeof(a);
        void* config[] = {HIP_LAUNCH_PARAM_BUFFER_POINTER, &a, HIP_LAUNCH_PARAM_BUFFER_SIZE, &arg_size, HIP_LAUNCH_PARAM_END};
        ctx->flush_staged();
        if (uni_fn)
          HIP_CHECK(hipExtModuleLaunchKernel(uni_fn, 64, 1, 1, 64, 1, 1, 0, st, nullptr, config, nullptr, nullptr, 0));
        for (hipFunction_t fn : *fns) {
          const bool timed = ctx->kbegin("quotient", qbytes);
          HIP_CHECK(hipExtModuleLaunchKernel(fn, div_up(Q, 256) * 256, 1, 1, 256, 1, 1, 0, st, nullptr, config,
                                             timed ? ctx->krecs.back().start : nullptr, timed ? ctx->krecs.back().stop : nullptr, 0));
        }
      } else {
        KLAUNCH(ctx, "quotient", qbytes, stark::quotient_kernel, dim3(div_up(Q, bd)), dim3(bd), lds, a);
      }
    });
    uint32_t wqp = kb::ONE;
    for (size_t k = 0; k < nchunks; k++) {
      zkm_matrix m; m.h = c.n; m.w = 4; m.d = qbuf + k * 4 * c.n; m.owned = (k == 0);
      qchunks.push_back(m);
      qshifts.push_back(kb::mul(kb::GEN, wqp));
      wqp = kb::mul(wqp, w_q);
    }
    if (i == 0) { launches[0](); launches[0] = [] {}; }
  }
  for (auto& l : launches) l();
  ctx->mark("quotient values");
  quot_data = pcs_commit(ctx, qchunks, qshifts, bl);
  for (auto& m : qchunks) if (m.owned) { quot_data->owned_evals.push_back(m); loose.disown(m.d); }
  guard.d.push_back(quot_data);
  ctx->mark("commit quotient");
  chal::observe_slice(ch, quot_data->root, 8);
  zeta = chal::sample_ext(ch);
  }

  void opened_values() {
  if (pk->data) {
    Round r; r.data = pk->data;
    for (size_t j = 0; j < pk->prep.size(); j++)
      r.mats.push_back(RoundMat{pk->prep[j].d, pk->prep[j].h, pk->prep[j].w, kb::ONE, &pk->data->ldes[j], pk->local_only[j] ? 1 : 2, {}});
    rounds.push_back(r);
  }
  {
    Round r; r.data = md->data;
    for (size_t i = 0; i < nc; i++)
      r.mats.push_back(RoundMat{md->traces[i].d, md->traces[i].h, md->traces[i].w, kb::ONE, &md->data->ldes[i], chips[i].desc->local_only ? 1 : 2, {}});
    rounds.push_back(r);
    Round rp; rp.data = perm_data;
    for (size_t i = 0; i < nc; i++)
      rp.mats.push_back(RoundMat{perm_traces[i].d, perm_traces[i].h, perm_traces[i].w, kb::ONE, &perm_data->ldes[i], 2, {}});
    rounds.push_back(rp);
    Round rq; rq.data = quot_data;
    for (size_t i = 0; i < qchunks.size(); i++)
      rq.mats.push_back(RoundMat{qchunks[i].d, qchunks[i].h, 4, qshifts[i], &quot_data->ldes[i], 1, {}});
    rounds.push_back(rq);
  }
  {
    std::vector<open::ColJob> cjobs;
    size_t total = 0;
    for (auto& r : rounds)
      for (auto& m : r.mats) {
        m.col0 = total;
        if (m.width == 0) continue;
        const size_t idx = (size_t)(m.lde - r.data->ldes.data());
        const uint32_t* cf = idx < r.data->col_flags.size() ? r.data->col_flags[idx] : nullptr;
        cjobs.push_back(open::ColJob{m.lde->d, m.evals, cf, m.lde->h, m.n, (uint32_t)total, (uint32_t)m.width});
        total += m.width;
      }
    const size_t tn = std::max<size_t>(total, 1);
    col_ptr_lde = (const uint32_t**)salloc(tn * sizeof(void*));
    col_ptr_eval = (const uint32_t**)salloc(tn * sizeof(void*));
    col_mask = (uint32_t*)salloc(tn * sizeof(uint32_t));
    uint32_t* cword = (uint32_t*)salloc(tn * 8 * sizeof(uint32_t));
    if (total) {
      const open::ColJob* d_c = (const open::ColJob*)ctx->upload_staged(cjobs.data(), cjobs.size() * sizeof(open::ColJob), &scratch);
      KLAUNCH(ctx, "col_tables", 0.0, open::build_col_tables, dim3(div_up(total, 256)), dim3(256), 0, d_c, (int)cjobs.size(), (uint32_t)total, col_ptr_lde,
              col_ptr_eval, col_mask, cword);
    }
  }
  {
    std::map<std::pair<size_t, uint32_t>, E4*> wcache;
    size_t total_y = 0;
    for (auto& r : rounds) for (auto& m : r.mats) total_y += m.width * 2;
    E4* d_y = (E4*)salloc(std::max<size_t>(total_y, 1) * sizeof(E4));
    std::vector<open::WeightJob> wjobs;
    std::vector<open::EvalJob> ejobs;
    std::vector<open::SumJob> sjobs;
    uint32_t wblk = 0, eblk = 0, sblk = 0;
    double wbytes = 0, ebytes = 0;
    size_t ypos = 0;
    for (auto& r : rounds)
      for (auto& m : r.mats) {
        if (m.width == 0) continue;
        auto key = std::make_pair(m.n, m.shift);
        E4* wts;
        auto it = wcache.find(key);
        if (it == wcache.end()) {
          int ln = log2_strict(m.n);
          open::WeightJob wj;
          wj.u = kb::escale(zeta, kb::inv(m.shift));
          wj.c = kb::escale(kb::esub_base(host_pow2k(wj.u, ln), kb::ONE), kb::inv(kb::to_monty((uint32_t)(m.n % kb::P))));
          wts = (E4*)salloc(m.n * sizeof(E4));
          wj.w_n = kb::two_adic_generator(ln); wj.n = m.n; wj.out = wts;
          wblk += div_up(div_up(m.n, 4), open::THREADS);
          wj.blk_end = wblk;
          wjobs.push_back(wj);
          wbytes += 16.0 * m.n;
          wcache[key] = wts;
        } else wts = it->second;
        open::EvalJob ej;
        ej.mat = m.evals; ej.weights = wts; ej.n = m.n; ej.width = (int)m.width;
        ej.colptr = col_ptr_eval + m.col0; ej.colmask = col_mask + m.col0;
        ej.groups = (int)div_up(m.width, open::EVAL_COLS);
        ej.split = 1;
        if (m.n >= 4 * open::THREADS) {
          ej.split = (int)std::min<size_t>(std::max<size_t>(1, 3072 / ej.groups), m.n / (4 * open::THREADS));
          ej.kind = m.n_points > 1 ? 1 : 0;
        } else {
          ej.kind = m.n_points > 1 ? 3 : 2;
        }
        ej.lead = 0;
        if (ej.split >= 8 && ej.groups > 1) {
          ej.split &= ~7;
          const uint32_t lead = (8 - eblk % 8) % 8;
          ej.lead = open::EVAL_XCD_AWARE | lead;
          eblk += lead;
        }
        ej.partials = (E4*)salloc((size_t)ej.split * m.width * 2 * sizeof(E4));
        eblk += (uint32_t)ej.groups * (uint32_t)ej.split;
        ej.blk_end = eblk;
        ejobs.push_back(ej);
        ebytes += 4.0 * m.n * m.width + 16.0 * m.n;
        sblk += (uint32_t)(m.width * 2);
        sjobs.push_back(open::SumJob{ej.partials, ej.split, (int)(m.width * 2), (uint32_t)ypos, sblk});
        ypos += m.width * 2;
      }
    if (!ejobs.empty()) {
      const open::WeightJob* d_w = (const open::WeightJob*)ctx->upload_staged(wjobs.data(), wjobs.size() * sizeof(open::WeightJob), &scratch);
      const open::EvalJob* d_e = (const open::EvalJob*)ctx->upload_staged(ejobs.data(), ejobs.size() * sizeof(open::EvalJob), &scratch);
      const open::SumJob* d_s = (const open::SumJob*)ctx->upload_staged(sjobs.data(), sjobs.size() * sizeof(open::SumJob), &scratch);
      KLAUNCH(ctx, "bary_weights", wbytes, open::bary_weights_batch, dim3(wblk), dim3(open::THREADS), 0, d_w);
      KLAUNCH(ctx, "eval_columns", ebytes, open::eval_columns_batch, dim3(eblk), dim3(open::THREADS), 0, d_e);
      KLAUNCH(ctx, "reduce_partials", 0.0, open::reduce_partials_batch, dim3(sblk), dim3(64), 0, d_s, d_y);
    }
    const E4* hy = ctx->download_async(d_y, std::max<size_t>(total_y, 1));
    ctx->sync(st);
    ypos = 0;
    for (auto& r : rounds)
      for (auto& m : r.mats) {
        for (int pt = 0; pt < 2; pt++) m.y[pt].clear();
        if (m.width == 0) continue;
        for (int pt = 0; pt < m.n_points; pt++) {
          m.y[pt].resize(m.width);
          for (size_t c = 0; c < m.width; c++) m.y[pt][c] = hy[ypos + c * 2 + pt];
        }
        ypos += m.width * 2;
      }
  }
  ctx->mark("open: evaluations");
  }

  void reduced_openings() {
  E4 fa = chal::sample_ext(ch);
  log_max = 0;
  std::vector<size_t> count(32, 0);
  size_t max_count = 1;
  for (auto& r : rounds) for (auto& m : r.mats) {
    int lh = log2_strict(m.lde->h);
    log_max = std::max(log_max, lh);
    count[lh] += m.width * m.n_points;
    max_count = std::max(max_count, count[lh]);
  }
  std::vector<E4> fap(max_count + 1);
  fap[0] = kb::eone();
  for (size_t i = 1; i <= max_count; i++) fap[i] = kb::emul(fap[i - 1], fa);
  E4* d_fap = (E4*)ctx->upload_staged(fap.data(), fap.size() * sizeof(E4), &scratch);
  {
    std::vector<std::vector<open::ReduceMat>> per_h(32);
    std::vector<size_t> off(32, 0);
    std::vector<std::array<E4, 2>> Y(32, {kb::ezero(), kb::ezero()});
    for (auto& r : rounds)
      for (auto& m : r.mats) {
        int lh = log2_strict(m.lde->h);
        open::ReduceMat rm;
        rm.lde = m.lde->d; rm.width = (int)m.width; rm.n_points = m.n_points;
        rm.colptr = col_ptr_lde + m.col0; rm.colmask = col_mask + m.col0;
        rm.apow_off = (uint32_t)off[lh]; rm.pad = 0;
        rm.A1 = fap[m.width];
        for (int pt = 0; pt < m.n_points; pt++) {
          E4 ysum = kb::ezero();
          for (size_t c = 0; c < m.width; c++) ysum = kb::eadd(ysum, kb::emul(fap[off[lh] + c], m.y[pt][c]));
          Y[lh][pt] = kb::eadd(Y[lh][pt], ysum);
          off[lh] += m.width;
        }
        per_h[lh].push_back(rm);
      }
    std::vector<open::ReduceMat*> d_rms(32, nullptr);
    for (int lh = 0; lh < 32; lh++)
      if (!per_h[lh].empty()) d_rms[lh] = (open::ReduceMat*)ctx->upload_staged(per_h[lh].data(), per_h[lh].size() * sizeof(open::ReduceMat), &scratch);
    for (int lh = 0; lh < 32; lh++) {
      if (per_h[lh].empty()) continue;
      size_t N = (size_t)1 << lh;
      ro[lh] = (E4*)salloc(N * sizeof(E4));
      open::ReduceMat* d_rm = d_rms[lh];
      E4 z1 = kb::escale(zeta, kb::two_adic_generator(lh - bl));
      double rbytes = 16.0 * N;
      for (auto& rm : per_h[lh]) rbytes += 4.0 * N * rm.width;
      std::pair<const uint32_t*, const uint32_t*> pw{nullptr, nullptr};
      if (lh >= 12) pw = ctx->pow_tables(lh);
      KLAUNCH(ctx, "reduce_openings", rbytes, open::reduce_openings, dim3(div_up(N, open::THREADS)), dim3(open::THREADS), 0,
              (const open::ReduceMat*)d_rm, (int)per_h[lh].size(), lh, (const E4*)d_fap, Y[lh][0], Y[lh][1], zeta, z1, kb::two_adic_generator(lh),
              pw.first, pw.second, ro[lh]);
    }
  }
  ctx->mark("open: reduced openings");
  }

  void fri_commit_phase() {
  static_assert(sizeof(merkle::DevChallenger) == sizeof(zkm_challenger), "the device challenger is the ABI's challenger");
  E4* f = ro[log_max];
  int lf = log_max;
  uint32_t neg_half = kb::neg(kb::inv(kb::to_monty(2)));
  const int n_layers = log_max - bl;
  merkle::DevChallenger* d_ch = (merkle::DevChallenger*)ctx->upload(ch, sizeof(zkm_challenger), &scratch);
  E4* d_betas = (E4*)salloc((size_t)std::max(n_layers, 1) * 2 * sizeof(E4));
  uint32_t* h_roots = (uint32_t*)ctx->pin_alloc((size_t)std::max(n_layers, 1) * 32);
  if (!h_roots) throw std::runtime_error("pinned staging ring exhausted");
  for (int i = 0; i < n_layers * 8; i++) ((volatile uint32_t*)h_roots)[i] = 0xffffffffu;
  int li = 0;
  while (lf > bl) {
    size_t len = (size_t)1 << lf, half = len / 2;
    Tree t;
    t.max_height = half; t.log_max = lf - 1;
    size_t off = 0;
    for (size_t l = half; l >= 1; l >>= 1) { t.layer_off.push_back(off); off += l; if (l == 1) break; }
    t.digests = (uint32_t*)salloc(off * 8 * 4);
    int fuse = 0;
    static const size_t FRI_LANES_MAX = getenv("ZKM_FRI_LANES_MAX") ? (size_t)atol(getenv("ZKM_FRI_LANES_MAX")) : 4096;
    if (half > FRI_LANES_MAX && half >= (size_t)merkle::FRI_FUSE_LEAVES) fuse = std::min(merkle::FRI_FUSE_MAX_LEVELS, lf - 1);
    if (half <= FRI_LANES_MAX)
      KLAUNCH(ctx, "hash_fri_leaves_lanes", 64.0 * half, merkle::hash_fri_leaves_lanes, dim3(div_up(half * 16, merkle::THREADS)), dim3(merkle::THREADS), 0,
              (const E4*)f, half, t.digests);
    else if (fuse > 0)
      KLAUNCH(ctx, "hash_fri_leaves_tree", 32.0 * half + 32.0 * half * (2.0 - 1.0 / (1 << fuse)), merkle::hash_fri_leaves_tree,
              dim3(half / merkle::FRI_FUSE_LEAVES), dim3(merkle::FRI_FUSE_LEAVES), merkle::FRI_FUSE_LEAVES * 12 * sizeof(uint32_t), (const E4*)f, half, t.digests, fuse);
    else
      KLAUNCH(ctx, "hash_fri_leaves", 64.0 * half, merkle::hash_fri_leaves, dim3(div_up(half, merkle::THREADS)), dim3(merkle::THREADS), 0,
              (const E4*)f, half, t.digests);
    int layer = fuse;
    bool tail = false;
    for (size_t l = half >> (fuse + 1); l >= 1; l >>= 1, layer++)
      if (compress_small_layer(ctx, t, layer, l, d_ch, d_betas + 2 * li, h_roots + 8 * li)) { tail = true; break; }
    if (!tail)
      KLAUNCH(ctx, "fri_root_challenge", 0.0, merkle::fri_root_challenge, dim3(1), dim3(64), 0, t.node(t.log_max, 0), h_roots + 8 * li, d_ch, d_betas + 2 * li);
    t.h_root = nullptr;
    E4* g = (E4*)salloc(half * sizeof(E4));
    KLAUNCH(ctx, "fri_fold", 48.0 * half + (ro[lf - 1] ? 16.0 * half : 0.0), open::fri_fold, dim3(div_up(half, open::THREADS)),
            dim3(open::THREADS), 0, (const E4*)f, lf, (const E4*)(d_betas + 2 * li), kb::two_adic_generator(lf),
            kb::inv(kb::two_adic_generator(lf)), neg_half, (const E4*)ro[lf - 1], g);
    layers.push_back(f);
    ftrees.push_back(t);
    f = g;
    lf--;
    li++;
  }
  const size_t nfin = (size_t)1 << lf;
  const E4* fin = ctx->download_async((const E4*)f, nfin);
  const E4* used = n_layers > 0 ? ctx->download_async((const E4*)d_betas, (size_t)n_layers * 2) : nullptr;
  ctx->sync(st);
  for (int i = 0; i < n_layers; i++) {
    std::array<uint32_t, 8> root;
    memcpy(root.data(), h_roots + 8 * i, 32);
    for (int k = 0; k < 8; k++)
      if (root[k] == 0xffffffffu) throw std::runtime_error("an FRI layer's root did not arrive in page-locked memory (internal error)");
    chal::observe_slice(ch, root.data(), 8);
    commits.push_back(root);
    const E4 beta = chal::sample_ext(ch);
    if (!kb::eq(beta, used[2 * i])) throw std::runtime_error("the device transcript of the FRI commit phase diverged from the host's (internal error)");
  }
  for (size_t i = 1; i < nfin; i++)
    if (!kb::eq(fin[i], fin[0])) throw std::runtime_error("FRI final polynomial is not constant (internal error)");
  final_poly = fin[0];
  chal::observe_ext(ch, final_poly);
  ctx->mark("open: FRI commit phase");
  }

  void grind() {
  {
    uint32_t* d_state = (uint32_t*)ctx->upload_staged(ch->sponge_state, 64, &scratch);
    uint32_t* d_in = (uint32_t*)ctx->upload_staged(ch->input_buffer, 64, &scratch);
    unsigned int* d_best = (unsigned int*)salloc(4);
    uint32_t base = 0, found = 0xffffffffu;
    const uint32_t BATCH = 1u << 20;
    while (base < kb::P) {
      HIP_CHECK(hipMemsetAsync(d_best, 0xff, 4, st));
      uint32_t total = std::min<uint64_t>(BATCH, (uint64_t)kb::P - base);
      KLAUNCH(ctx, "grind", 0.0, merkle::grind, dim3(div_up(total, merkle::THREADS)), dim3(merkle::THREADS), 0, (const uint32_t*)d_state,
              (const uint32_t*)d_in, (int)ch->num_inputs, (int)fri->proof_of_work_bits, base, total, d_best);
      const unsigned int* h_best = ctx->download_async((const unsigned int*)d_best, 1);
      ctx->sync(st);
      found = *h_best;
      if (found != 0xffffffffu) break;
      base += total;
    }
    if (found == 0xffffffffu) throw std::runtime_error("proof-of-work search exhausted the field");
    pow_witness = kb::to_monty(found);
    chal::observe(ch, pow_witness);
    if (chal::sample_bits(ch, fri->proof_of_work_bits) != 0) throw std::runtime_error("proof-of-work witness rejected by host transcript");
  }
  ctx->mark("open: grind");
  }

  void query_phase() {
  indices.assign(fri->num_queries, 0);
  for (auto& q : indices) q = chal::sample_bits(ch, log_max);
  std::vector<open::QueryWord> tmpl;
  for (auto& r : rounds) {
    const Tree& t = r.data->tree;
    const uint32_t tree_shift = (uint32_t)(log_max - t.log_max);
    for (auto& m : r.mats) {
      const uint32_t sh = tree_shift + (uint32_t)(t.log_max - log2_strict(m.lde->h));
      for (size_t c = 0; c < m.width; c++) tmpl.push_back(open::QueryWord{m.lde->d + c * m.lde->h, sh, 0, 1, 0});
    }
    for (int l = 0; l < t.log_max; l++)
      for (uint32_t k = 0; k < 8; k++) tmpl.push_back(open::QueryWord{t.node(l, 0), tree_shift + (uint32_t)l, 1, 8, k});
  }
  for (size_t tI = 0; tI < ftrees.size(); tI++) {
    for (uint32_t k = 0; k < 4; k++) tmpl.push_back(open::QueryWord{(const uint32_t*)layers[tI], (uint32_t)tI, 1, 4, k});
    const Tree& t = ftrees[tI];
    for (int l = 0; l < t.log_max; l++)
      for (uint32_t k = 0; k < 8; k++) tmpl.push_back(open::QueryWord{t.node(l, 0), (uint32_t)(tI + 1 + l), 1, 8, k});
  }
  const size_t per_query = tmpl.size(), n_gather = per_query * indices.size();
  if (n_gather) {
    std::vector<uint32_t> idx32(indices.begin(), indices.end());
    const open::QueryWord* d_tmpl = (const open::QueryWord*)ctx->upload_staged(tmpl.data(), tmpl.size() * sizeof(open::QueryWord), &scratch);
    const uint32_t* d_idx = (const uint32_t*)ctx->upload_staged(idx32.data(), idx32.size() * 4, &scratch);
    uint32_t* d_dst = (uint32_t*)salloc(n_gather * 4);
    ctx->flush_staged();
    hipLaunchKernelGGL(open::gather_queries, dim3(div_up(n_gather, open::THREADS)), dim3(open::THREADS), 0, st, d_tmpl, per_query, d_idx, indices.size(), d_dst);
    LAUNCH_CHECK();
    uint32_t* h = (uint32_t*)ctx->pin_alloc(n_gather * 4);
    if (h) {
      HIP_CHECK(hipMemcpyAsync(h, d_dst, n_gather * 4, hipMemcpyDeviceToHost, st));
      gathered = h;
    } else {
      gathered_big.resize(n_gather);
      HIP_CHECK(hipMemcpyAsync(gathered_big.data(), d_dst, n_gather * 4, hipMemcpyDeviceToHost, st));
      gathered = gathered_big.data();
    }
    ctx->sync(st);
  }
  ctx->mark("open: queries");
  }

  void serialise(Writer& out) {
  out.words(md->data->root, 8);
  out.words(perm_data->root, 8);
  out.words(quot_data->root, 8);
  out.u((uint32_t)nc);
  size_t ri = pk->data ? 1 : 0;
  Round& rmain = rounds[ri];
  Round& rperm = rounds[ri + 1];
  Round& rquot = rounds[ri + 2];
  size_t qpos = 0;
  auto put_exts = [&](const std::vector<E4>& v) { for (auto& e : v) out.ext(e); };
  for (size_t i = 0; i < nc; i++) {
    const zkm_chip_desc* d = chips[i].desc;
    out.u((uint32_t)md->order[i]);
    out.u((uint32_t)chips[i].log_n);
    if (d->prep_index >= 0) {
      RoundMat& pm = rounds[0].mats[d->prep_index];
      out.u((uint32_t)pm.width);
      put_exts(pm.y[0]);
      if (pm.n_points > 1) put_exts(pm.y[1]); else put_exts(std::vector<E4>(pm.width, kb::ezero()));
    } else out.u(0);
    RoundMat& mm = rmain.mats[i];
    out.u((uint32_t)mm.width);
    put_exts(mm.y[0]);
    if (mm.n_points > 1) put_exts(mm.y[1]); else put_exts(std::vector<E4>(mm.width, kb::ezero()));
    RoundMat& pm = rperm.mats[i];
    out.u((uint32_t)pm.width);
    put_exts(pm.y[0]); put_exts(pm.y[1]);
    size_t nch = (size_t)1 << d->log_quotient_degree;
    out.u((uint32_t)nch);
    for (size_t k = 0; k < nch; k++) put_exts(rquot.mats[qpos++].y[0]);
    out.words(global_sums[i].data(), 14);
    out.ext(local_sums[i]);
  }
  out.u((uint32_t)commits.size());
  for (auto& c : commits) out.words(c.data(), 8);
  out.u((uint32_t)indices.size());
  size_t gp = 0;
  for (size_t qi = 0; qi < indices.size(); qi++) {
    out.u((uint32_t)rounds.size());
    for (auto& r : rounds) {
      out.u((uint32_t)r.mats.size());
      for (auto& m : r.mats) { out.u((uint32_t)m.width); out.words(gathered + gp, m.width); gp += m.width; }
      out.u((uint32_t)r.data->tree.log_max);
      out.words(gathered + gp, (size_t)r.data->tree.log_max * 8); gp += (size_t)r.data->tree.log_max * 8;
    }
    out.u((uint32_t)ftrees.size());
    for (auto& t : ftrees) {
      out.words(gathered + gp, 4); gp += 4;
      out.u((uint32_t)t.log_max);
      out.words(gathered + gp, (size_t)t.log_max * 8); gp += (size_t)t.log_max * 8;
    }
  }
  out.ext(final_poly);
  out.u(pow_witness);
  out.u((uint32_t)md->public_values.size());
  out.words(md->public_values.data(), md->public_values.size());
  }
};

static void open_impl(zkm_ctx* ctx, const zkm_pk* pk, zkm_main_data* md, const zkm_chip_desc* chips_in, const zkm_fri_config* fri,
                      uint32_t num_pv_elts, zkm_challenger* ch, Writer& out) {
  ShardOpening o(ctx, pk, md, chips_in, fri, num_pv_elts, ch);
  o.permutation_phase();
  o.quotient_phase();
  o.opened_values();
  o.reduced_openings();
  o.fri_commit_phase();
  o.grind();
  o.query_phase();
  o.serialise(out);
}
```

### ziren_amd/csrc/host_pcs.hpp

```cpp
#pragma once
struct LdeJob {
  const uint32_t* in; size_t n, w; uint32_t lde_shift; uint32_t* out;
  uint32_t* cflag = nullptr;
  bool uniform = false;
};

static void lde_batch_chunk(zkm_ctx* ctx, const std::vector<LdeJob>& jobs, int bl) {
  std::vector<size_t> order(jobs.size());
  std::iota(order.begin(), order.end(), 0);
  std::stable_sort(order.begin(), order.end(), [&](size_t a, size_t b) { return jobs[a].n > jobs[b].n; });
  std::vector<lde::Batch> hb(1);
  lde::Batch& b = hb[0];
  memset(&b, 0, sizeof b);
  b.log_blowup = bl;
  const size_t cosets = (size_t)1 << bl;
  size_t tmp1_words = 0, tmp2_words = 0;
  for (size_t oi : order) if (jobs[oi].n > ((size_t)1 << lde::LOG_ROW_MAX)) { tmp1_words += jobs[oi].n * jobs[oi].w; tmp2_words += (jobs[oi].n * jobs[oi].w) << bl; }
  uint32_t* tmp1 = tmp1_words ? ctx->alloc_n<uint32_t>(tmp1_words) : nullptr;
  uint32_t* tmp2 = tmp2_words ? ctx->alloc_n<uint32_t>(tmp2_words) : nullptr;
  size_t t1 = 0, t2 = 0;
  size_t big_cols = 0, fc = 0;
  for (size_t oi : order) if (jobs[oi].n > ((size_t)1 << lde::LOG_ROW_MAX) && !jobs[oi].cflag) big_cols += jobs[oi].w;
  uint32_t* cflags = big_cols ? ctx->alloc_n<uint32_t>(2 * big_cols) : nullptr;
  if (cflags) HIP_CHECK(hipMemsetAsync(cflags, 0, 2 * big_cols * sizeof(uint32_t), ctx->cur));
// ... 15 lines not shown
    g.twb_fwd = lb > 0 ? ctx->twiddles(lb, false) : nullptr;
    if (la) {
      g.twa_inv = ctx->twiddles_ct(la, true);
      g.twa_fwd = ctx->twiddles_ct(la, false);
      auto pw = ctx->pow_tables(k);
      g.pw_lo = pw.first; g.pw_hi = pw.second;
      g.tw_rows = ctx->row_twiddles(k);
    }
    uint32_t cols = 0;
    for (; p < order.size() && jobs[order[p]].n == n; p++) {
      const LdeJob& j = jobs[order[p]];
      lde::Mat& m = b.m[nm++];
      m.in = j.in; m.out = j.out; m.col0 = cols; m.w = (uint32_t)j.w; m.shift = j.lde_shift; m.uniform = j.uniform ? 1u : 0u;
      if (la) {
        m.tmp1 = tmp1 + t1; t1 += n * j.w;
        m.tmp2 = tmp2 + t2; t2 += (n * j.w) << bl;
        if (j.cflag) m.cflag = j.cflag;
        else { m.cflag = cflags + fc; fc += 2 * j.w; }
        auto ct = ctx->coset_tables(k, bl, j.lde_shift);
        m.twf = ct.twf; m.cs = ct.cs;
      }
      cols += (uint32_t)j.w;
    }
    g.n_cols = cols;
    g.n_mats = nm - g.first_mat;
    const double cells = (double)n * cols;
    if (la) {
      const size_t per_col = ((size_t)1 << lb) >> g.logT;
      blk[lde::K_COLS_INV] += (uint32_t)(per_col * cols);
      blk[lde::K_ROWS_BIG] += (uint32_t)(((size_t)1 << la) * cols);
      blk[lde::K_COLS_FWD] += (uint32_t)(per_col * cols * cosets);
      lds_cols = std::max(lds_cols, ((size_t)1 << la) * (((size_t)1 << g.logT) + 1) * 4);
      bytes_inv += 8.0 * cells; bytes_rows += 4.0 * cells * (1 + cosets); bytes_fwd += 8.0 * cells * cosets;
      for (int mi = (int)g.first_mat; mi < nm; mi++) if (b.m[mi].uniform) bytes_inv -= 8.0 * (double)n * b.m[mi].w;
    } else {
      blk[lde::K_ROWS_SMALL] += cols;
      const size_t B = (size_t)1 << lb;
      lds_small = std::max(lds_small, (2 * (B + (B >> 5)) + 64 + (B > 64 ? (B >> 6) : 1)) * 4);
      bytes_small += 4.0 * cells * (1 + cosets);
    }
    for (int q = 0; q < 4; q++) g.blk_end[q] = blk[q];
    b.n_groups++;
  }
  const lde::Batch* d = (const lde::Batch*)ctx->upload_staged(&b, sizeof b);
  if (blk[lde::K_COLS_INV]) {
    constexpr size_t B = (size_t)1 << lde::LOG_ROW_MAX;
    const size_t big_lds = (B + (B >> 5)) * 4;
    KLAUNCH(ctx, "lde_cols_inverse", bytes_inv, lde::lde_cols<false>, dim3(blk[lde::K_COLS_INV]), dim3(lde::THREADS), lds_cols, d);
    KLAUNCH(ctx, "lde_rows", bytes_rows, lde::lde_rows_big, dim3(blk[lde::K_ROWS_BIG]), dim3(lde::THREADS), big_lds, d);
    KLAUNCH(ctx, "lde_cols_forward", bytes_fwd, lde::lde_cols<true>, dim3(blk[lde::K_COLS_FWD]), dim3(lde::THREADS), lds_cols, d);
  }
  if (blk[lde::K_ROWS_SMALL])
    KLAUNCH(ctx, "lde_rows", bytes_small, lde::lde_rows, dim3(blk[lde::K_ROWS_SMALL]), dim3(lde::THREADS), lds_small, d);
  ctx->release_here(tmp1);
  ctx->release_here(tmp2);
  ctx->release_here(cflags);
  ctx->release_here((void*)d);
}

static void lde_batch(zkm_ctx* ctx, const std::vector<LdeJob>& all, int bl) {
  constexpr size_t SCRATCH_BUDGET_WORDS = ((size_t)12 << 30) / 4;
  std::vector<LdeJob> jobs;
  size_t scratch = 0;
  for (auto& j : all) {
    if (j.w == 0) continue;
    const size_t need = j.n > ((size_t)1 << lde::LOG_ROW_MAX) ? j.n * j.w + ((j.n * j.w) << bl) : 0;
    if (!jobs.empty() && ((int)jobs.size() == lde::MAX_MATS || scratch + need > SCRATCH_BUDGET_WORDS)) { lde_batch_chunk(ctx, jobs, bl); jobs.clear(); scratch = 0; }
    jobs.push_back(j);
    scratch += need;
  }
  if (!jobs.empty()) lde_batch_chunk(ctx, jobs, bl);
}

static void lde_columns(zkm_ctx* ctx, const uint32_t* in, size_t n, size_t w, int bl, uint32_t lde_shift, uint32_t* out) {
  lde_batch(ctx, {LdeJob{in, n, w, lde_shift, out}}, bl);
}

static const uint32_t** upload_ptrs(zkm_ctx* ctx, const std::vector<const uint32_t*>& ptrs) {
  return (const uint32_t**)ctx->upload_staged(ptrs.data(), ptrs.size() * sizeof(void*));
}

static bool compress_small_layer(zkm_ctx* ctx, Tree& t, int layer, size_t len, merkle::DevChallenger* d_ch = nullptr, kb::E4* d_beta = nullptr,
                                 uint32_t* h_root_slot = nullptr) {
  static const size_t LANES_MAX = getenv("ZKM_LANES_MAX") ? (size_t)atol(getenv("ZKM_LANES_MAX")) : 4096;
  const size_t TAIL = 64;
  if (len > LANES_MAX) {
    KLAUNCH(ctx, "compress_layer", 96.0 * len, merkle::compress_layer, dim3(div_up(len, merkle::THREADS)), dim3(merkle::THREADS), 0,
            (const uint32_t*)(t.digests + t.layer_off[layer] * 8), t.digests + t.layer_off[layer + 1] * 8, len,
            (const uint32_t* const*)nullptr, 0, (const uint32_t*)nullptr);
    return false;
  }
  if (len <= TAIL) {
    uint32_t* h_root = h_root_slot ? h_root_slot : (uint32_t*)ctx->pin_alloc(32);
    if (h_root) for (int k = 0; k < 8; k++) ((volatile uint32_t*)h_root)[k] = 0xffffffffu;
    KLAUNCH(ctx, "compress_tail", 96.0 * len, merkle::compress_tail_lanes, dim3(1), dim3(1024), 0, t.digests + t.layer_off[layer] * 8, len, h_root, d_ch, d_beta);
    t.h_root = h_root;
    return true;
  }
  KLAUNCH(ctx, "compress_small", 96.0 * len, merkle::compress_layer_lanes, dim3(div_up(len * 16, merkle::THREADS)), dim3(merkle::THREADS),
          0, (const uint32_t*)(t.digests + t.layer_off[layer] * 8), t.digests + t.layer_off[layer + 1] * 8, len);
  return false;
}

static inline void cpu_relax() {
#if defined(__x86_64__) || defined(__i386__)
  __builtin_ia32_pause();
#elif defined(__aarch64__)
  __asm__ __volatile__("yield");
#endif
}

static void wait_root(zkm_ctx* ctx, const uint32_t* h_root, bool pollable) {
  if (ctx->root_poll && pollable) {
    const volatile uint32_t* v = h_root;
    auto t0 = std::chrono::steady_clock::now();
    zkm_ctx::TimerSlack slack;
    for (int spins = 0;; spins++) {
      bool all = true;
      for (int k = 0; k < 8; k++) all &= v[k] != 0xffffffffu;
      if (all) { std::atomic_thread_fence(std::memory_order_acquire); return; }
      if ((ctx->host_wait_blocking || (spins & 4095) == 4095) && std::chrono::steady_clock::now() - t0 > std::chrono::seconds(1)) {
        const hipError_t q = hipStreamQuery(ctx->stream);
        if (q == hipErrorNotReady) { t0 = std::chrono::steady_clock::now(); continue; }
        if (q != hipSuccess) HIP_CHECK(q);
        bool now = true;
        for (int k = 0; k < 8; k++) now &= v[k] != 0xffffffffu;
        if (now) { std::atomic_thread_fence(std::memory_order_acquire); return; }
        ctx->root_poll = false;
        g_err = "a finished launch's tree root is not visible in page-locked memory: root polling is off for this context (stream synchronisation instead)";
        break;
      }
      if (ctx->host_wait_blocking) { if (spins >= 64) zkm_ctx::sleep_ns(std::min(ctx->wait_sleep_ns, 10000), slack); else cpu_relax(); }
      else if (spins < ctx->root_spin_before_yield) cpu_relax();
      else if (ctx->root_sleep_ns > 0) zkm_ctx::sleep_ns(ctx->root_sleep_ns, slack);
      else sched_yield();
    }
  }
  ctx->sync(ctx->stream);
}

static void build_tree(zkm_ctx* ctx, const std::vector<zkm_matrix>& mats, Tree& t,
                       const std::function<void(size_t)>& prepare_height = nullptr, const std::vector<const uint32_t*>* col_flags = nullptr,
                       bool rows_up_front = false) {
  auto wait_height = [&](size_t h) {
    if (prepare_height) prepare_height(h);
  };
  size_t maxh = 0;
  for (auto& m : mats) maxh = std::max(maxh, m.h);
  t.max_height = maxh;
  t.log_max = log2_strict(maxh);
  t.layer_off.clear();
  size_t off = 0;
  for (size_t len = maxh; len >= 1; len >>= 1) { t.layer_off.push_back(off); off += len; if (len == 1) break; }
  t.digests = ctx->alloc_n<uint32_t>(off * 8);
  auto cols_of_height = [&](size_t h) {
    std::vector<const uint32_t*> ptrs;
    for (auto& m : mats)
      if (m.h == h)
        for (size_t c = 0; c < m.w; c++) ptrs.push_back(m.d + c * m.h);
    return ptrs;
  };
  std::vector<const uint32_t**> to_free;
  std::map<size_t, const uint32_t**> flag_tables;
  uint32_t* prefixes = nullptr;
  if (col_flags) {
    size_t n_tab = 0;
    for (size_t i = 0; i < mats.size(); i++) {
      const size_t h = mats[i].h;
      if (h == maxh || flag_tables.count(h)) continue;
      size_t first = 0;
      while (mats[first].h != h) first++;
      if (!(*col_flags)[first]) { flag_tables[h] = nullptr; continue; }
      std::vector<const uint32_t*> fp;
      for (size_t j = 0; j < mats.size(); j++)
        if (mats[j].h == h)
          for (size_t c = 0; c < mats[j].w; c++) fp.push_back((*col_flags)[j] ? (*col_flags)[j] + 2 * c : nullptr);
      flag_tables[h] = upload_ptrs(ctx, fp);
      to_free.push_back(flag_tables[h]);
      n_tab++;
    }
    if (n_tab) prefixes = ctx->alloc_n<uint32_t>(32 * n_tab);
  }
  size_t prefix_no = 0;
  std::map<size_t, std::pair<const uint32_t**, size_t>> tables;
  for (auto& m : mats)
    if (!tables.count(m.h)) {
      auto ptrs = cols_of_height(m.h);
      const uint32_t** d = ptrs.empty() ? nullptr : upload_ptrs(ctx, ptrs);
      if (d) to_free.push_back(d);
      tables[m.h] = {d, ptrs.size()};
    }
  int fuse = 0;
  if (maxh >= (size_t)merkle::FUSE_LEAVES) {
    while (fuse < merkle::FUSE_MAX_LEVELS && (maxh >> (fuse + 1)) >= 1) {
      bool injected = false;
      for (auto& m : mats) injected |= m.h == (maxh >> (fuse + 1));
      if (injected) break;
      fuse++;
    }
  }
  {
    const uint32_t** d = tables[maxh].first;
    struct { size_t n; size_t size() const { return n; } } ptrs{tables[maxh].second};
    wait_height(maxh);
    if (fuse > 0)
      KLAUNCH(ctx, "hash_leaves_tree", 4.0 * maxh * ptrs.size() + 32.0 * maxh * (2.0 - 1.0 / (1 << fuse)), merkle::hash_leaves_tree,
              dim3(maxh / merkle::FUSE_LEAVES), dim3(merkle::FUSE_LEAVES), merkle::FUSE_LEAVES * 12 * sizeof(uint32_t), d, (int)ptrs.size(), maxh,
              t.digests, fuse);
    else
      KLAUNCH(ctx, "hash_leaves", 4.0 * maxh * ptrs.size() + 32.0 * maxh, merkle::hash_leaves, dim3(div_up(maxh, merkle::THREADS)),
              dim3(merkle::THREADS), 0, d, (int)ptrs.size(), maxh, t.digests);
  }
  size_t min_h = maxh;
  for (auto& m : mats) min_h = std::min(min_h, m.h);
  std::map<size_t, uint32_t*> rowdig;
  uint32_t* rowdig_buf = nullptr;
  if (rows_up_front && min_h < maxh) {
    std::vector<size_t> hs;
    size_t rows = 0;
    for (auto& kv : tables)
      if (kv.first < maxh && kv.second.first) { hs.push_back(kv.first); rows += kv.first; }
    std::sort(hs.begin(), hs.end(), [&](size_t a, size_t b) {
      const size_t pa = (tables[a].second + 7) / 8, pb = (tables[b].second + 7) / 8;
      return pa != pb ? pa > pb : a > b;
    });
    rowdig_buf = ctx->alloc_n<uint32_t>(rows * 8);
    std::vector<merkle::RowGroup> groups;
    size_t off = 0, blocks = 0;
    double bytes = 0;
    for (size_t h : hs) {
      wait_height(h);
      const uint32_t* prefix = nullptr;
      if (flag_tables.count(h) && flag_tables[h]) {
        uint32_t* out = prefixes + 32 * prefix_no++;
        KLAUNCH(ctx, "sponge_prefix", 0.0, merkle::sponge_prefix, dim3(1), dim3(64), 0, (const uint32_t* const*)flag_tables[h], (int)tables[h].second, out);
        prefix = out;
      }
      rowdig[h] = rowdig_buf + off * 8;
      groups.push_back(merkle::RowGroup{(const uint32_t* const*)tables[h].first, prefix, rowdig[h], (uint32_t)h, (int)tables[h].second, (uint32_t)blocks});
      off += h;
      blocks += div_up(h, merkle::THREADS);
      bytes += 4.0 * h * tables[h].second + 32.0 * h;
    }
    const merkle::RowGroup* d_groups = (const merkle::RowGroup*)ctx->upload_staged(groups.data(), groups.size() * sizeof(merkle::RowGroup));
    to_free.push_back((const uint32_t**)d_groups);
    KLAUNCH(ctx, "hash_rows", bytes, merkle::hash_rows, dim3((unsigned)blocks), dim3(merkle::THREADS), 0, d_groups, (int)groups.size());
  }
  int layer = fuse;
  for (size_t len = maxh >> (fuse + 1); len >= 1; len >>= 1, layer++) {
    if (min_h > len) {
      if (compress_small_layer(ctx, t, layer, len)) break;
      continue;
    }
    if (rowdig.count(len)) {
      KLAUNCH(ctx, "compress_layer_rowdig", 96.0 * len + 32.0 * len, merkle::compress_layer_rowdig, dim3(div_up(len, merkle::THREADS)), dim3(merkle::THREADS), 0,
              (const uint32_t*)(t.digests + t.layer_off[layer] * 8), t.digests + t.layer_off[layer + 1] * 8, len, (const uint32_t*)rowdig[len]);
      if (len == 1) break;
      continue;
    }
    const uint32_t** d = tables.count(len) ? tables[len].first : nullptr;
    struct { size_t n; size_t size() const { return n; } } ptrs{tables.count(len) ? tables[len].second : 0};
    if (d) wait_height(len);
    const uint32_t* prefix = nullptr;
    if (d && flag_tables.count(len) && flag_tables[len]) {
      uint32_t* out = prefixes + 32 * prefix_no++;
      KLAUNCH(ctx, "sponge_prefix", 0.0, merkle::sponge_prefix, dim3(1), dim3(64), 0, (const uint32_t* const*)flag_tables[len], (int)ptrs.size(), out);
      prefix = out;
    }
    KLAUNCH(ctx, "compress_layer", 96.0 * len + 4.0 * len * ptrs.size(), merkle::compress_layer, dim3(div_up(len, merkle::THREADS)),
            dim3(merkle::THREADS), 0, (const uint32_t*)(t.digests + t.layer_off[layer] * 8), t.digests + t.layer_off[layer + 1] * 8,
            len, (const uint32_t* const*)d, (int)ptrs.size(), prefix);
    if (len == 1) break;
  }
  for (auto d : to_free) ctx->release((void*)d);
  ctx->release(prefixes);
  ctx->release(rowdig_buf);
}

static void free_pcs_data(zkm_ctx* ctx, zkm_pcs_data* d) {
  if (!d) return;
  for (auto& m : d->ldes) ctx->release(m.d);
  for (auto& m : d->owned_evals) ctx->release(m.d);
  ctx->release(d->tree.digests);
  ctx->release(d->cflags);
  delete d;
}

static zkm_pcs_data* pcs_commit(zkm_ctx* ctx, const std::vector<zkm_matrix>& mats, const std::vector<uint32_t>& shifts,
                                int log_blowup) {
  zkm_pcs_data* d = new zkm_pcs_data();
  uint32_t* cflags = nullptr;
  try {
    d->log_blowup = log_blowup;
    for (size_t i = 0; i < mats.size(); i++) {
      const zkm_matrix& m = mats[i];
      zkm_matrix l;
      l.h = m.h << log_blowup;
      l.w = m.w;
      l.d = ctx->alloc_n<uint32_t>(l.h * l.w);
      d->ldes.push_back(l);
      d->evals.push_back(m.d);
      d->eval_heights.push_back(m.h);
      d->domain_shifts.push_back(shifts.empty() ? kb::ONE : shifts[i]);
    }
    auto shift_of = [&](size_t i) { return kb::mul(kb::GEN, kb::inv(d->domain_shifts[i])); };
    size_t flag_words = 0;
    for (auto& m : mats) if (m.h > ((size_t)1 << lde::LOG_ROW_MAX)) flag_words += 2 * m.w;
    cflags = flag_words ? ctx->alloc_n<uint32_t>(flag_words) : nullptr;
    if (cflags) HIP_CHECK(hipMemsetAsync(cflags, 0, flag_words * sizeof(uint32_t), ctx->stream));
    std::vector<const uint32_t*> col_flags(mats.size(), nullptr);
    {
      size_t off = 0;
      for (size_t i = 0; i < mats.size(); i++)
        if (mats[i].h > ((size_t)1 << lde::LOG_ROW_MAX)) { col_flags[i] = cflags + off; off += 2 * mats[i].w; }
    }
    auto job_of = [&](size_t i) { return LdeJob{mats[i].d, mats[i].h, mats[i].w, shift_of(i), d->ldes[i].d, const_cast<uint32_t*>(col_flags[i]), mats[i].uniform_rows}; };
    std::vector<char> extended(mats.size(), 0);
    size_t top = 0;
    for (auto& l : d->ldes) top = std::max(top, l.h);
    {
      const bool overlap = ctx->lde_overlap;
      std::vector<LdeJob> tall, rest;
      size_t rest_cells = 0;
      for (size_t i = 0; i < mats.size(); i++)
        if (!mats[i].ready || hipEventQuery(mats[i].ready) == hipSuccess) {
          (d->ldes[i].h == top ? tall : rest).push_back(job_of(i));
          if (d->ldes[i].h != top) rest_cells += mats[i].h * mats[i].w;
          extended[i] = 1;
        }
      if (overlap && !tall.empty() && rest_cells >= ((size_t)1 << 22)) {
        lde_batch(ctx, tall, log_blowup);
        ctx->side_begin();
        try { lde_batch(ctx, rest, log_blowup); } catch (...) { ctx->side_end(); ctx->side_join(); throw; }
        ctx->side_end();
      } else {
        tall.insert(tall.end(), rest.begin(), rest.end());
        lde_batch(ctx, tall, log_blowup);
      }
    }
    auto extend_height = [&](size_t lde_height) {
      if (lde_height < top) ctx->side_join();
      std::vector<LdeJob> jobs;
      for (size_t i = 0; i < mats.size(); i++) {
        if (extended[i] || d->ldes[i].h != lde_height) continue;
        wait_ready(ctx->stream, mats[i]);
        jobs.push_back(job_of(i));
        extended[i] = 1;
      }
      lde_batch(ctx, jobs, log_blowup);
    };
    const bool rows_up_front = ctx->rows_up_front && std::all_of(extended.begin(), extended.end(), [](char e) { return e != 0; });
    build_tree(ctx, d->ldes, d->tree, extend_height, &col_flags, rows_up_front);
    ctx->side_join();
    d->cflags = cflags;
    d->col_flags = col_flags;
    cflags = nullptr;
    for (size_t i = 0; i < mats.size(); i++)
      if (!extended[i]) throw std::runtime_error("pcs_commit: a matrix was not reached by the tree (internal error)");
    const uint32_t* h_root = d->tree.h_root ? d->tree.h_root : ctx->download_async(d->tree.node(d->tree.log_max, 0), 8);
    ctx->sync(ctx->stream);
    d->tree.h_root = nullptr;
    memcpy(d->root, h_root, 32);
  } catch (...) {
    ctx->cur = ctx->stream;
    try { ctx->side_join(); } catch (...) {}
    ctx->release(cflags);
    free_pcs_data(ctx, d);
    throw;
  }
  return d;
}
```

### ziren_amd/csrc/open.cuh

```cuda
#pragma once
#include "kb31.cuh"
#include "gptr.cuh"

namespace open {

constexpr int THREADS = 256;

struct ColJob { const uint32_t* lde; const uint32_t* evals; const uint32_t* cflag; size_t N, n; uint32_t col0, width; };
__global__ __launch_bounds__(256) void build_col_tables(const ColJob* __restrict__ jobs, int n_jobs, uint32_t total, const uint32_t** __restrict__ lde_ptr,
                                                        const uint32_t** __restrict__ eval_ptr, uint32_t* __restrict__ mask, uint32_t* __restrict__ cword) {
  const uint32_t t = blockIdx.x * blockDim.x + threadIdx.x;
  if (t >= total) return;
  int j = 0;
  while (j + 1 < n_jobs && t >= jobs[j + 1].col0) j++;
  const ColJob J = jobs[j];
  const uint32_t c = t - J.col0;
  if (J.cflag && J.cflag[2 * c] == 0) {
    const uint32_t w0 = J.cflag[2 * c + 1];
    const uint32_t w = kb::umin32(w0, w0 - kb::P);
#pragma unroll
    for (int k = 0; k < 8; k++) cword[8 * (size_t)t + k] = w;
    lde_ptr[t] = cword + 8 * (size_t)t;
    eval_ptr[t] = cword + 8 * (size_t)t;
    mask[t] = 0;
  } else {
    lde_ptr[t] = J.lde + (size_t)c * J.N;
    eval_ptr[t] = J.evals + (size_t)c * J.n;
    mask[t] = 0xffffffffu;
  }
}

struct WeightJob { kb::E4 u, c; uint32_t w_n, blk_end; size_t n; kb::E4* out; };
struct EvalJob {
  const uint32_t* mat; const kb::E4* weights; kb::E4* partials;
  const uint32_t* const* colptr; const uint32_t* colmask;
  size_t n;
  int width, groups, split, kind;
  uint32_t blk_end;
  uint32_t lead;
};
constexpr uint32_t EVAL_XCD_AWARE = 0x100;
struct SumJob { const kb::E4* partials; int split, count; uint32_t out0, blk_end; };
template <class J>
__device__ __forceinline__ const J& find_job(const J* __restrict__ jobs, uint32_t& local) {
  uint32_t j = 0, start = 0;
  const uint32_t b = blockIdx.x;
  while (b >= jobs[j].blk_end) { start = jobs[j].blk_end; j++; }
  local = b - start;
  return jobs[j];
}

__device__ __forceinline__ void bary_weights_body(kb::E4 u, kb::E4 c, uint32_t w_n, size_t n, kb::E4* __restrict__ out, uint32_t bx) {
  const size_t i0 = ((size_t)bx * blockDim.x + threadIdx.x) * 4;
  if (i0 >= n) return;
  uint32_t wi[4];
  wi[0] = kb::pow(w_n, (uint64_t)i0);
#pragma unroll
  for (int k = 1; k < 4; k++) wi[k] = kb::mul(wi[k - 1], w_n);
  kb::E4 d[4];
#pragma unroll
  for (int k = 0; k < 4; k++) d[k] = i0 + k < n ? kb::esub_base(u, wi[k]) : kb::eone();
  const kb::E4 p1 = kb::emul(d[0], d[1]), p2 = kb::emul(p1, d[2]), p3 = kb::emul(p2, d[3]);
  kb::E4 inv = kb::einv(p3), di[4];
  di[3] = kb::emul(inv, p2);
  inv = kb::emul(inv, d[3]);
  di[2] = kb::emul(inv, p1);
  inv = kb::emul(inv, d[2]);
  di[1] = kb::emul(inv, d[0]);
  di[0] = kb::emul(inv, d[1]);
#pragma unroll
  for (int k = 0; k < 4; k++)
    if (i0 + k < n) out[i0 + k] = kb::emul(kb::escale(di[k], wi[k]), c);
}
__global__ __launch_bounds__(THREADS) void bary_weights(kb::E4 u, kb::E4 c, uint32_t w_n, size_t n, kb::E4* __restrict__ out) {
  bary_weights_body(u, c, w_n, n, out, blockIdx.x);
}
__global__ __launch_bounds__(THREADS) void bary_weights_batch(const WeightJob* __restrict__ jobs) {
  uint32_t bx;
  const WeightJob& j = find_job(jobs, bx);
  bary_weights_body(j.u, j.c, j.w_n, j.n, j.out, bx);
}

constexpr int EVAL_COLS = 4;

constexpr int EVAL_WORDS = EVAL_COLS * 8;
__device__ __forceinline__ void block_reduce_store(kb::E4 (&acc)[EVAL_COLS][2], int c0, int width, kb::E4* __restrict__ partials,
                                                   uint32_t* lds , uint32_t by) {
  const int tid = threadIdx.x;
#pragma unroll
  for (int c = 0; c < EVAL_COLS; c++)
#pragma unroll
    for (int pt = 0; pt < 2; pt++)
#pragma unroll
      for (int e = 0; e < 4; e++) lds[((c * 2 + pt) * 4 + e) * THREADS + tid] = acc[c][pt].c[e];
  __syncthreads();
  uint32_t* seg = lds + EVAL_WORDS * THREADS;
  {
    const int word = tid >> 3, part = tid & 7;
    const uint32_t* src = lds + word * THREADS + part * (THREADS / 8);
    uint32_t t = 0;
#pragma unroll 8
    for (int k = 0; k < THREADS / 8; k++) t = kb::add(t, src[k]);
    seg[word * 8 + part] = t;
  }
  __syncthreads();
  if (tid < EVAL_WORDS) {
    uint32_t t = 0;
#pragma unroll
    for (int k = 0; k < 8; k++) t = kb::add(t, seg[tid * 8 + k]);
    const int c = tid >> 3, pt = (tid >> 2) & 1, e = tid & 3;
    if (c0 + c < width) partials[((size_t)by * width + c0 + c) * 2 + pt].c[e] = t;
  }
}

template <bool TWO>
__device__ __forceinline__ void eval_columns_body(const uint32_t* const* __restrict__ colptr, const uint32_t* __restrict__ colmask, size_t n, int width,
                                                  const kb::E4* __restrict__ weights,
                                                  kb::E4* __restrict__ partials, uint32_t* red, uint32_t bx, uint32_t by, uint32_t ny) {
  const int c0 = bx * EVAL_COLS;
  const uint32_t* cols[EVAL_COLS];
  uint32_t msk[EVAL_COLS];
#pragma unroll
  for (int c = 0; c < EVAL_COLS; c++) {
    cols[c] = gp::load(colptr + min(c0 + c, width - 1));
    msk[c] = gp::load(colmask + min(c0 + c, width - 1));
  }
  kb::E4 acc[EVAL_COLS][2];
#pragma unroll
  for (int c = 0; c < EVAL_COLS; c++) { acc[c][0] = kb::ezero(); acc[c][1] = kb::ezero(); }
  const size_t stride = (size_t)ny * THREADS * 4;
  for (size_t r = ((size_t)by * THREADS + threadIdx.x) * 4; r < n; r += stride) {
    kb::E4 w[4];
    uint4 v[EVAL_COLS];
    uint32_t vnext[EVAL_COLS];
    const size_t rn = r + 4 == n ? 0 : r + 4;
#pragma unroll
    for (int k = 0; k < 4; k++) w[k] = gp::load_e4(weights + r + k);
#pragma unroll
    for (int c = 0; c < EVAL_COLS; c++) {
      v[c] = gp::load(reinterpret_cast<const uint4*>(cols[c] + ((uint32_t)r & msk[c])));
      if (TWO) vnext[c] = gp::load(cols[c] + ((uint32_t)rn & msk[c]));
    }
#pragma unroll
    for (int c = 0; c < EVAL_COLS; c++) {
      const uint32_t x[5] = {v[c].x, v[c].y, v[c].z, v[c].w, TWO ? vnext[c] : 0u};
#pragma unroll
      for (int e = 0; e < 4; e++) {
        acc[c][0].c[e] = kb::reduce96_bounded(0, (uint64_t)w[0].c[e] * x[0] + (uint64_t)w[1].c[e] * x[1] + (uint64_t)w[2].c[e] * x[2] +
                                                     (uint64_t)w[3].c[e] * x[3] + (uint64_t)acc[c][0].c[e] * kb::ONE);
        if (TWO)
          acc[c][1].c[e] = kb::reduce96_bounded(0, (uint64_t)w[0].c[e] * x[1] + (uint64_t)w[1].c[e] * x[2] + (uint64_t)w[2].c[e] * x[3] +
                                                       (uint64_t)w[3].c[e] * x[4] + (uint64_t)acc[c][1].c[e] * kb::ONE);
      }
    }
  }
  block_reduce_store(acc, c0, width, partials, red, by);
}

__device__ __forceinline__ void eval_columns_small_body(const uint32_t* const* __restrict__ colptr, const uint32_t* __restrict__ colmask, size_t n, int width,
                                                        const kb::E4* __restrict__ weights,
                                                        int two_points, kb::E4* __restrict__ partials, uint32_t* red, uint32_t bx) {
  const int c0 = bx * EVAL_COLS;
  kb::E4 acc[EVAL_COLS][2];
#pragma unroll
  for (int c = 0; c < EVAL_COLS; c++) { acc[c][0] = kb::ezero(); acc[c][1] = kb::ezero(); }
  for (size_t r = threadIdx.x; r < n; r += THREADS) {
    kb::E4 w = weights[r];
    size_t rn = r + 1 == n ? 0 : r + 1;
#pragma unroll
    for (int c = 0; c < EVAL_COLS; c++) {
      const uint32_t* col = colptr[min(c0 + c, width - 1)];
      const uint32_t mk = colmask[min(c0 + c, width - 1)];
      acc[c][0] = kb::eadd(acc[c][0], kb::escale(w, col[(uint32_t)r & mk]));
      if (two_points) acc[c][1] = kb::eadd(acc[c][1], kb::escale(w, col[(uint32_t)rn & mk]));
    }
  }
  block_reduce_store(acc, c0, width, partials, red, 0);
}
__global__ __launch_bounds__(THREADS) void eval_columns_batch(const EvalJob* __restrict__ jobs) {
  __shared__ uint32_t red[EVAL_WORDS * THREADS + EVAL_WORDS * 8];
  uint32_t local;
  const EvalJob& j = find_job(jobs, local);
  uint32_t bx = local % (uint32_t)j.groups, by = local / (uint32_t)j.groups;
  if (j.lead & EVAL_XCD_AWARE) {
    const uint32_t lead = j.lead & 0xff;
    if (local < lead) return;
    local -= lead;
    const uint32_t x = local & 7, s = local >> 3;
    bx = s % (uint32_t)j.groups;
    by = (s / (uint32_t)j.groups) * 8 + x;
  }
  if (j.kind == 0) eval_columns_body<false>(j.colptr, j.colmask, j.n, j.width, j.weights, j.partials, red, bx, by, (uint32_t)j.split);
  else if (j.kind == 1) eval_columns_body<true>(j.colptr, j.colmask, j.n, j.width, j.weights, j.partials, red, bx, by, (uint32_t)j.split);
  else eval_columns_small_body(j.colptr, j.colmask, j.n, j.width, j.weights, j.kind == 3, j.partials, red, bx);
}

__device__ __forceinline__ void reduce_partials_body(const kb::E4* __restrict__ partials, int split, int count, kb::E4* __restrict__ out, int i) {
  kb::E4 acc = kb::ezero();
  for (int s = threadIdx.x; s < split; s += 64) acc = kb::eadd(acc, partials[(size_t)s * count + i]);
#pragma unroll
  for (int e = 0; e < 4; e++) {
    uint32_t v = acc.c[e];
#pragma unroll
    for (int d = 32; d > 0; d >>= 1) v = kb::add(v, __shfl_xor(v, d));
    acc.c[e] = v;
  }
  if (threadIdx.x == 0) out[i] = acc;
}
__global__ __launch_bounds__(64) void reduce_partials_batch(const SumJob* __restrict__ jobs, kb::E4* __restrict__ out) {
  uint32_t i;
  const SumJob& j = find_job(jobs, i);
  reduce_partials_body(j.partials, j.split, j.count, out + j.out0, (int)i);
}

__device__ __forceinline__ uint32_t load_row(const uint32_t* base, uint32_t off) {
#if defined(__HIP_DEVICE_COMPILE__)
  return *(const uint32_t __attribute__((address_space(1)))*)((const char __attribute__((address_space(1)))*)base + off);
#else
  return *(const uint32_t*)((const char*)base + off);
#endif
}
struct ReduceMat {
  const uint32_t* lde;
  const uint32_t* const* colptr; const uint32_t* colmask;
  int width;
  int n_points;
  uint32_t apow_off;
  uint32_t pad;
  kb::E4 A1;
};

__global__ __launch_bounds__(THREADS) void reduce_openings(const ReduceMat* __restrict__ mats, int n_mats, int log_N,
                                                           const kb::E4* __restrict__ alpha_pows, kb::E4 Y0, kb::E4 Y1, kb::E4 z0, kb::E4 z1,
                                                           uint32_t w_N, const uint32_t* __restrict__ pw_lo, const uint32_t* __restrict__ pw_hi,
                                                           kb::E4* __restrict__ ro) {
  size_t N = (size_t)1 << log_N;
  size_t r = (size_t)blockIdx.x * blockDim.x + threadIdx.x;
  if (r >= N) return;
  const uint32_t ex = kb::bitrev((uint32_t)r, log_N);
  const uint32_t wp = pw_lo ? kb::mul(pw_lo[ex & 1023], pw_hi[ex >> 10]) : kb::pow(w_N, (uint64_t)ex);
  uint32_t x = kb::mul(kb::GEN, wp);
  const kb::E4 e0 = kb::esub_base(z0, x), e1 = kb::esub_base(z1, x);
  const kb::E4 e01 = kb::einv(kb::emul(e0, e1));
  kb::E4 d0 = kb::emul(e01, e1);
  kb::E4 d1 = kb::emul(e01, e0);
  kb::E4 T0 = kb::ezero(), T1 = kb::ezero();
  bool two = false;
  const uint32_t roff = (uint32_t)r * 4u;
  for (int m = 0; m < n_mats; m++) {
    const ReduceMat& M = mats[m];
    const kb::E4* __restrict__ ap = alpha_pows + M.apow_off;
    kb::Acc96 s0 = kb::acc96_zero(), s1 = kb::acc96_zero(), s2 = kb::acc96_zero(), s3 = kb::acc96_zero();
#if defined(__HIP_DEVICE_COMPILE__)
    typedef const uint32_t* __attribute__((address_space(4))) const* PtrTable;
    typedef const uint32_t __attribute__((address_space(4)))* MaskTable;
    const PtrTable cp = (PtrTable)(uint64_t)M.colptr;
    const MaskTable cm = (MaskTable)(uint64_t)M.colmask;
#else
    const uint32_t* const* cp = M.colptr;
    const uint32_t* cm = M.colmask;
#endif
    int c = 0;
    for (; c + 8 <= M.width; c += 8) {
      uint32_t v[8];
#pragma unroll
      for (int k = 0; k < 8; k++) v[k] = load_row(cp[c + k], roff & cm[c + k]);
#pragma unroll
      for (int k = 0; k < 8; k++) {
        const kb::E4 a = ap[c + k];
        kb::acc96_fma_uniform(s0, a.c[0], v[k]);
        kb::acc96_fma_uniform(s1, a.c[1], v[k]);
        kb::acc96_fma_uniform(s2, a.c[2], v[k]);
        kb::acc96_fma_uniform(s3, a.c[3], v[k]);
      }
    }
    for (; c < M.width; c++) {
      const kb::E4 a = ap[c];
      const uint32_t v = load_row(cp[c], roff & cm[c]);
      kb::acc96_fma_uniform(s0, a.c[0], v);
      kb::acc96_fma_uniform(s1, a.c[1], v);
      kb::acc96_fma_uniform(s2, a.c[2], v);
      kb::acc96_fma_uniform(s3, a.c[3], v);
    }
    const kb::E4 S = M.width <= 126
                         ? kb::E4{{kb::reduce96_bounded(s0.hi, s0.lo), kb::reduce96_bounded(s1.hi, s1.lo), kb::reduce96_bounded(s2.hi, s2.lo),
                                   kb::reduce96_bounded(s3.hi, s3.lo)}}
                         : kb::E4{{kb::acc96_reduce(s0), kb::acc96_reduce(s1), kb::acc96_reduce(s2), kb::acc96_reduce(s3)}};
    T0 = kb::eadd(T0, S);
    if (M.n_points > 1) { T1 = kb::eadd(T1, kb::emul(M.A1, S)); two = true; }
  }
  kb::E4 acc = kb::emul(kb::esub(Y0, T0), d0);
  if (two) acc = kb::eadd(acc, kb::emul(kb::esub(Y1, T1), d1));
  ro[r] = acc;
}


__global__ __launch_bounds__(THREADS) void fri_fold(const kb::E4* __restrict__ f, int log_len, const kb::E4* __restrict__ betas,
                                                    uint32_t w_len, uint32_t w_len_inv, uint32_t neg_half,
                                                    const kb::E4* __restrict__ ro_next,
                                                    kb::E4* __restrict__ g) {
  size_t half = (size_t)1 << (log_len - 1);
  size_t j = (size_t)blockIdx.x * blockDim.x + threadIdx.x;
  if (j >= half) return;
  const kb::E4 beta = betas[0], beta_sq = betas[1];
  kb::E4 e0 = f[2 * j], e1 = f[2 * j + 1];
  uint32_t e = kb::bitrev((uint32_t)(2 * j), log_len);
  uint32_t xinv = kb::pow(w_len_inv, (uint64_t)e);
  uint32_t x = kb::pow(w_len, (uint64_t)e);
  kb::E4 t = kb::emul(kb::esub_base(beta, x), kb::esub(e1, e0));
  kb::E4 r = kb::eadd(e0, kb::escale(t, kb::mul(neg_half, xinv)));
  if (ro_next) r = kb::eadd(r, kb::emul(beta_sq, ro_next[j]));
  g[j] = r;
}

struct QueryWord {
  const uint32_t* base;
  uint32_t shift, flip, step, k;
};
__global__ __launch_bounds__(THREADS) void gather_queries(const QueryWord* __restrict__ tmpl, size_t per_query, const uint32_t* __restrict__ indices,
                                                          size_t n_queries, uint32_t* __restrict__ dst) {
  const size_t i = (size_t)blockIdx.x * blockDim.x + threadIdx.x;
  if (i >= per_query * n_queries) return;
  const size_t qi = i / per_query;
  const QueryWord w = tmpl[i - qi * per_query];
  const size_t q = indices[qi];
  dst[i] = w.base[(((q >> w.shift) ^ w.flip) * w.step) + w.k];
}

__global__ __launch_bounds__(THREADS) void gather_words(const uint32_t* const* __restrict__ src, size_t count, uint32_t* __restrict__ dst) {
  size_t i = (size_t)blockIdx.x * blockDim.x + threadIdx.x;
  if (i < count) dst[i] = *src[i];
}

__global__ void transpose(const uint32_t* __restrict__ in, uint32_t* __restrict__ out, size_t rows, size_t cols) {
  __shared__ uint32_t tile[32][33];
  size_t bx = (size_t)blockIdx.x * 32, by = (size_t)blockIdx.y * 32;
  for (int j = threadIdx.y; j < 32; j += blockDim.y) {
    size_t r = by + j, c = bx + threadIdx.x;
    if (r < rows && c < cols) tile[j][threadIdx.x] = in[r * cols + c];
  }
  __syncthreads();
  for (int j = threadIdx.y; j < 32; j += blockDim.y) {
    size_t c = bx + j, r = by + threadIdx.x;
    if (r < rows && c < cols) out[c * rows + r] = tile[threadIdx.x][j];
  }
}

__global__ void transpose_slab(const uint32_t* __restrict__ in, uint32_t* __restrict__ out, size_t rows, size_t cols, size_t r0,
                               size_t height) {
  __shared__ uint32_t tile[32][33];
  size_t bx = (size_t)blockIdx.x * 32, by = (size_t)blockIdx.y * 32;
  for (int j = threadIdx.y; j < 32; j += blockDim.y) {
    size_t r = by + j, c = bx + threadIdx.x;
    if (r < rows && c < cols) {
      uint32_t w = in[r * cols + c];
      w = w >= kb::P ? w - kb::P : w;
      w = w >= kb::P ? w - kb::P : w;
      tile[j][threadIdx.x] = w;
    }
  }
  __syncthreads();
  for (int j = threadIdx.y; j < 32; j += blockDim.y) {
    size_t c = bx + j, r = by + threadIdx.x;
    if (r < rows && c < cols) out[c * height + r0 + r] = tile[threadIdx.x][j];
  }
}

__global__ void flat_rows(const uint32_t* __restrict__ in, size_t n_words, uint32_t* __restrict__ out, size_t cols, size_t height) {
  __shared__ uint32_t tile[32][33];
  size_t bx = (size_t)blockIdx.x * 32, by = (size_t)blockIdx.y * 32;
  for (int j = threadIdx.y; j < 32; j += blockDim.y) {
    size_t r = by + j, c = bx + threadIdx.x;
    uint32_t w = 0;
    if (r < height && c < cols && r * cols + c < n_words) {
      w = in[r * cols + c];
      w = w >= kb::P ? w - kb::P : w;
      w = w >= kb::P ? w - kb::P : w;
    }
    tile[j][threadIdx.x] = w;
  }
  __syncthreads();
  for (int j = threadIdx.y; j < 32; j += blockDim.y) {
    size_t c = bx + j, r = by + threadIdx.x;
    if (r < height && c < cols) out[c * height + r] = tile[threadIdx.x][j];
  }
}

}
```

### ziren_amd/csrc/zkm_hip.hip

```cpp
#include "../../include/zkm_hip.h"

#include <hip/hip_runtime.h>
#include <hip/hip_ext.h>

#include <algorithm>
#include <array>
#include <atomic>
#include <chrono>
#include <cstdlib>
#include <cstdio>
#include <cstring>
#include <functional>
#include <map>
#include <mutex>
#include <numeric>
#include <stdexcept>
#include <string>
#include <unordered_map>
#include <exception>
#include <vector>

#include <sched.h>
#include <time.h>
#include <sys/prctl.h>

#include "kb31.cuh"
#include "poseidon2.cuh"
#include "lde.cuh"
#include "merkle.cuh"
#include "stark.cuh"
#include "open.cuh"
#include "tracegen.cuh"

using kb::E4;

#include "host_ctx.hpp"
#include "host_pcs.hpp"
#include "host_open.hpp"

template <int CHIP>
static void launch_alu_rows(zkm_ctx* ctx, const uint32_t* d_events, size_t n_events, size_t height, uint32_t* out, uint32_t* counts) {
  KLAUNCH(ctx, "tracegen_alu", 4.0 * tracegen::event_words(CHIP) * n_events + 4.0 * height * tracegen::chip_width(CHIP), tracegen::alu_rows<CHIP>,
          dim3(div_up(height, (counts ? tracegen::TILES_PER_BLOCK : 1) * tracegen::THREADS)), dim3(tracegen::THREADS),
          counts ? 2 * tracegen::HASH_SLOTS * sizeof(uint32_t) : 0, d_events, n_events, height, out, counts,
          counts ? tracegen::TILES_PER_BLOCK : 1);
}

#define API_BEGIN try {
#define API_END                              \
  }                                          \
  catch (const std::exception& e) {          \
    g_err = e.what();                        \
    return -1;                               \
  }                                          \
  catch (...) {                              \
    g_err = "unknown exception (not derived from std::exception)"; \
    return -1;                               \
  }                                          \
  return 0;

struct CallScope {
  zkm_ctx* c;
  int exceptions;
  explicit CallScope(zkm_ctx* ctx) : c(ctx), exceptions(std::uncaught_exceptions()) {
    if (c->call_depth++ == 0) c->call_allocs.clear();
  }
  ~CallScope() {
    if (--c->call_depth > 0) return;
    if (std::uncaught_exceptions() > exceptions) {
      (void)hipStreamSynchronize(c->stream);
      (void)hipStreamSynchronize(c->stream2);
      if (c->ev_dma) (void)hipStreamSynchronize(c->ev_dma);
      (void)hipGetLastError();
      c->cur = c->stream;
      c->side_pending = false;
      for (void* p : c->side_deferred) c->release(p);
      c->side_deferred.clear();
      for (void* p : c->call_allocs) c->release(p);
    }
    c->call_allocs.clear();
  }
};

extern "C" {

const char* zkm_last_error(void) { return g_err.c_str(); }

#ifndef ZKM_SOURCES_DIGEST
#define ZKM_SOURCES_DIGEST "unrecorded"
#endif
#ifndef ZKM_HIPCC_VERSION
#define ZKM_HIPCC_VERSION "unknown"
#endif
static const char build_info_string[] = "ZKM_SOURCES_DIGEST=" ZKM_SOURCES_DIGEST ";hipcc=" ZKM_HIPCC_VERSION ";arch=gfx950";
const char* zkm_build_info(void) { return build_info_string; }

int zkm_ctx_create(int device, zkm_ctx** out) {
  API_BEGIN
  int count = 0;
  hipError_t e = hipGetDeviceCount(&count);
  if (e != hipSuccess || count == 0)
    throw std::runtime_error("no HIP device available: libzkm_hip has no CPU fallback (hipGetDeviceCount: " +
                             std::string(hipGetErrorString(e)) + ")");
  if (device < 0 || device >= count) throw std::runtime_error("device index out of range");
  HIP_CHECK(hipSetDevice(device));
  zkm_ctx* c = new zkm_ctx();
  c->device = device;
  HIP_CHECK(hipStreamCreateWithFlags(&c->stream, hipStreamNonBlocking));
  HIP_CHECK(hipStreamCreateWithFlags(&c->stream2, hipStreamNonBlocking));
  c->cur = c->stream;
  HIP_CHECK(p2::upload_tables());
  HIP_CHECK(p2f::upload_tables());
  HIP_CHECK(tracegen::upload_tables());
  HIP_CHECK(septic::upload_tables());
  {
    static const uint32_t DUMMY_X[7] = {1706420302, 1319108093, 148224806, 26874985, 1766171812, 1645633948, 2028659224};
    static const uint32_t DUMMY_Y[7] = {942390502, 1239997438, 458866455, 1843332012, 1309764648, 572807436, 74267719};
    uint32_t consts[28];
    for (int k = 0; k < 7; k++) {
      consts[k] = kb::to_monty(SEPTIC_X[k]); consts[7 + k] = kb::to_monty(SEPTIC_Y[k]);
      consts[14 + k] = kb::to_monty(DUMMY_X[k]); consts[21 + k] = kb::to_monty(DUMMY_Y[k]);
    }
    HIP_CHECK(hipMemcpyToSymbol(HIP_SYMBOL(tracegen::d_global_consts), consts, sizeof consts));
  }
  HIP_CHECK(hipFuncSetAttribute((const void*)lde::lde_rows, hipFuncAttributeMaxDynamicSharedMemorySize, 160 * 1024));
  HIP_CHECK(hipFuncSetAttribute((const void*)lde::lde_rows_big, hipFuncAttributeMaxDynamicSharedMemorySize, 160 * 1024));
  HIP_CHECK(hipFuncSetAttribute((const void*)tracegen::alu_rows<tracegen::ADD_SUB>, hipFuncAttributeMaxDynamicSharedMemorySize, 64 * 1024));
  HIP_CHECK(hipFuncSetAttribute((const void*)tracegen::alu_rows<tracegen::BITWISE>, hipFuncAttributeMaxDynamicSharedMemorySize, 64 * 1024));
  HIP_CHECK(hipFuncSetAttribute((const void*)tracegen::alu_rows<tracegen::LT>, hipFuncAttributeMaxDynamicSharedMemorySize, 64 * 1024));
  HIP_CHECK(hipFuncSetAttribute((const void*)tracegen::alu_rows<tracegen::SHIFT_LEFT>, hipFuncAttributeMaxDynamicSharedMemorySize, 64 * 1024));
  HIP_CHECK(hipFuncSetAttribute((const void*)tracegen::alu_rows<tracegen::SHIFT_RIGHT>, hipFuncAttributeMaxDynamicSharedMemorySize, 64 * 1024));
  HIP_CHECK(hipFuncSetAttribute((const void*)tracegen::alu_rows<tracegen::CLO_CLZ>, hipFuncAttributeMaxDynamicSharedMemorySize, 64 * 1024));
  HIP_CHECK(hipFuncSetAttribute((const void*)tracegen::alu_rows<tracegen::JUMP>, hipFuncAttributeMaxDynamicSharedMemorySize, 64 * 1024));
  HIP_CHECK(hipFuncSetAttribute((const void*)tracegen::alu_rows<tracegen::MOV_COND>, hipFuncAttributeMaxDynamicSharedMemorySize, 64 * 1024));
  HIP_CHECK(hipFuncSetAttribute((const void*)tracegen::alu_rows<tracegen::MUL>, hipFuncAttributeMaxDynamicSharedMemorySize, 64 * 1024));
  HIP_CHECK(hipFuncSetAttribute((const void*)tracegen::alu_rows<tracegen::DIVREM>, hipFuncAttributeMaxDynamicSharedMemorySize, 64 * 1024));
  HIP_CHECK(hipFuncSetAttribute((const void*)tracegen::cpu_rows, hipFuncAttributeMaxDynamicSharedMemorySize, 64 * 1024));
  HIP_CHECK(hipFuncSetAttribute((const void*)tracegen::alu_rows<tracegen::MEMORY_INSTRS>, hipFuncAttributeMaxDynamicSharedMemorySize, 64 * 1024));
  HIP_CHECK(hipFuncSetAttribute((const void*)tracegen::alu_rows<tracegen::MISC_INSTRS>, hipFuncAttributeMaxDynamicSharedMemorySize, 64 * 1024));
  HIP_CHECK(hipFuncSetAttribute((const void*)tracegen::alu_rows<tracegen::BRANCH>, hipFuncAttributeMaxDynamicSharedMemorySize, 64 * 1024));
  {
    const void* big_field_kernels[] = {
        (const void*)tracegen::u8_pair_histogram, (const void*)tracegen::ed_add_rows, (const void*)tracegen::ed_decompress_rows,
        (const void*)tracegen::weierstrass_rows<8, false>, (const void*)tracegen::weierstrass_rows<8, true>,
        (const void*)tracegen::weierstrass_rows<12, false>, (const void*)tracegen::weierstrass_rows<12, true>,
        (const void*)tracegen::uint256_mul_rows, (const void*)tracegen::u256x2048_mul_rows, (const void*)tracegen::weierstrass_decompress_rows<8, false>, (const void*)tracegen::weierstrass_decompress_rows<12, true>,
        (const void*)tracegen::fp_tower_rows<8, 0>, (const void*)tracegen::fp_tower_rows<8, 1>, (const void*)tracegen::fp_tower_rows<8, 2>,
        (const void*)tracegen::fp_tower_rows<12, 0>, (const void*)tracegen::fp_tower_rows<12, 1>, (const void*)tracegen::fp_tower_rows<12, 2>};
    for (const void* k : big_field_kernels) HIP_CHECK(hipFuncSetAttribute(k, hipFuncAttributeMaxDynamicSharedMemorySize, 160 * 1024));
  }
  HIP_CHECK(hipFuncSetAttribute((const void*)lde::lde_cols<false>, hipFuncAttributeMaxDynamicSharedMemorySize, 160 * 1024));
  HIP_CHECK(hipFuncSetAttribute((const void*)lde::lde_cols<true>, hipFuncAttributeMaxDynamicSharedMemorySize, 160 * 1024));
  HIP_CHECK(hipFuncSetAttribute((const void*)stark::quotient_kernel, hipFuncAttributeMaxDynamicSharedMemorySize, 152 * 1024));
  *out = c;
  API_END
}

void zkm_ctx_destroy(zkm_ctx* ctx) {
  if (!ctx) return;
  (void)hipSetDevice(ctx->device);
  (void)hipStreamSynchronize(ctx->stream);
  for (auto& kv : ctx->prefetched) { (void)hipEventSynchronize(kv.second.landed); (void)hipEventDestroy(kv.second.landed); }
  for (auto& kv : ctx->free_list) (void)hipFree(kv.second);
  for (auto& kv : ctx->live) (void)hipFree(kv.first);
  for (auto& kv : ctx->tw_fwd) (void)hipFree(kv.second);
  for (auto& kv : ctx->tw_inv) (void)hipFree(kv.second);
  for (auto& kv : ctx->pow_tabs) { (void)hipFree(kv.second.first); (void)hipFree(kv.second.second); }
  ctx->drop_coset_tables();
  for (auto& kv : ctx->row_tabs) (void)hipFree(kv.second);
  for (auto& kv : ctx->ct_fwd) (void)hipFree(kv.second);
  for (auto& kv : ctx->ct_inv) (void)hipFree(kv.second);
  for (auto& kv : ctx->selector_tabs) (void)hipFree(kv.second);
  for (auto& m : ctx->marks) (void)hipEventDestroy(m.second);
  for (auto& e : ctx->event_pool) (void)hipEventDestroy(e);
  for (auto& m : ctx->modules) (void)hipModuleUnload(m);
  if (ctx->pin) (void)hipHostFree(ctx->pin);
  if (ctx->arena) (void)hipFree(ctx->arena);
  if (ctx->ev_dma) (void)hipStreamDestroy(ctx->ev_dma);
  (void)hipStreamDestroy(ctx->stream);
  (void)hipStreamDestroy(ctx->stream2);
  if (ctx->up_dma) {
    (void)hipStreamDestroy(ctx->up_dma);
    (void)hipStreamDestroy(ctx->up_tr);
    for (int k = 0; k < 2; k++) { (void)hipFree(ctx->up_stage[k]); (void)hipEventDestroy(ctx->up_freed[k]); (void)hipEventDestroy(ctx->up_landed[k]); }
  }
  delete ctx;
}

int zkm_ctx_trim(zkm_ctx* ctx) {
  API_BEGIN
  std::lock_guard<std::mutex> lk(ctx->mu);
  HIP_CHECK(hipSetDevice(ctx->device));
  CallScope call_scope(ctx);
  ctx->sync(ctx->stream);
  for (auto& kv : ctx->free_list) { HIP_CHECK(hipFree(kv.second)); ctx->pool_bytes -= kv.first; }
  ctx->free_list.clear();
  ctx->drop_coset_tables();
  for (auto& kv : ctx->selector_tabs) HIP_CHECK(hipFree(kv.second));
  ctx->selector_tabs.clear();
  for (auto& kv : ctx->row_tabs) HIP_CHECK(hipFree(kv.second));
  ctx->row_tabs.clear();
  API_END
}

int zkm_ctx_set_memory_limit(zkm_ctx* ctx, size_t bytes) {
  API_BEGIN
  if (!ctx) throw std::runtime_error("zkm_ctx_set_memory_limit: null context");
  std::lock_guard<std::mutex> lk(ctx->mu);
  ctx->pool_limit = bytes;
  if (bytes && ctx->pool_bytes > bytes) {
    HIP_CHECK(hipSetDevice(ctx->device));
    ctx->drop_cached();
  }
  API_END
}
size_t zkm_ctx_memory_held(zkm_ctx* ctx) {
  if (!ctx) return 0;
  std::lock_guard<std::mutex> lk(ctx->mu);
  return ctx->pool_bytes;
}

int zkm_ctx_synchronize(zkm_ctx* ctx) {
  API_BEGIN
  ctx->sync(ctx->stream);
  if (ctx->ev_dma) ctx->sync(ctx->ev_dma);
  API_END
}

int zkm_ctx_last_timings(zkm_ctx* ctx, const char** names, float* ms, int cap) {
  int n = (int)ctx->timing_names.size();
  for (int i = 0; i < n && i < cap; i++) { names[i] = ctx->timing_names[i].c_str(); ms[i] = ctx->timing_ms[i]; }
  return n;
}

int zkm_ctx_kernel_timings(zkm_ctx* ctx, const char** names, float* ms, uint32_t* calls, double* bytes, int cap) {
  int i = 0;
  for (auto& kv : ctx->kstats) {
    if (i < cap) { names[i] = kv.first.c_str(); ms[i] = (float)kv.second.ms; calls[i] = kv.second.calls; bytes[i] = kv.second.bytes; }
    i++;
  }
  return i;
}
void zkm_ctx_set_kernel_timing(zkm_ctx* ctx, int mode) { ctx->kernel_timing = mode; }
void zkm_ctx_set_kernel_timing_only(zkm_ctx* ctx, const char* name) { ctx->timing_only = name ? name : ""; ctx->kernel_timing = 3; }
void zkm_ctx_set_host_wait(zkm_ctx* ctx, int blocking) { std::lock_guard<std::mutex> lk(ctx->mu); ctx->host_wait_blocking = blocking != 0; }
void zkm_ctx_set_lde_overlap(zkm_ctx* ctx, int on) { std::lock_guard<std::mutex> lk(ctx->mu); ctx->lde_overlap = on != 0; }
void zkm_ctx_set_rows_up_front(zkm_ctx* ctx, int on) { std::lock_guard<std::mutex> lk(ctx->mu); ctx->rows_up_front = on != 0; }

int zkm_ctx_register_quotient_kernel(zkm_ctx* ctx, const uint32_t* program, uint32_t program_len, const void* code_object,
                                     size_t code_object_len) {
  API_BEGIN
  std::lock_guard<std::mutex> lk(ctx->mu);
  HIP_CHECK(hipSetDevice(ctx->device));
  CallScope call_scope(ctx);
  if (!program_len || !code_object_len) throw std::runtime_error("empty program or code object");
  std::vector<std::pair<const char*, size_t>> parts;
  std::vector<std::vector<char>> copies;
  const char* bytes = (const char*)code_object;
  if (code_object_len >= 16 && memcmp(bytes, "ZKMQPART", 8) == 0) {
    uint32_t count;
    memcpy(&count, bytes + 8, 4);
    size_t at = 16 + 8 * (size_t)count;
    if (count == 0 || count > 4096 || at > code_object_len) throw std::runtime_error("malformed quotient kernel container");
    for (uint32_t i = 0; i < count; i++) {
      uint64_t len;
      memcpy(&len, bytes + 16 + 8 * (size_t)i, 8);
      if (len == 0 || len > code_object_len - at) throw std::runtime_error("malformed quotient kernel container");
      copies.emplace_back(bytes + at, bytes + at + len);
      at += len;
    }
    for (auto& c : copies) parts.push_back({c.data(), c.size()});
  } else {
    parts.push_back({bytes, code_object_len});
  }
  std::vector<hipFunction_t> fns;
  std::vector<hipModule_t> mods;
  try {
    for (auto& part : parts) {
      hipModule_t mod;
      HIP_CHECK(hipModuleLoadData(&mod, part.first));
      mods.push_back(mod);
      hipFunction_t fn;
      if (hipModuleGetFunction(&fn, mod, "zkm_quotient_specialized") != hipSuccess) throw std::runtime_error("code object lacks zkm_quotient_specialized");
      fns.push_back(fn);
    }
  } catch (...) {
    for (hipModule_t m : mods) (void)hipModuleUnload(m);
    throw;
  }
  for (hipModule_t m : mods) ctx->modules.push_back(m);
  const uint64_t key = fnv1a(program, program_len);
  ctx->quotient_fns[key] = fns;
  ctx->quotient_uniform_fns.erase(key);
  hipFunction_t uni;
  if (hipModuleGetFunction(&uni, mods[0], "zkm_quotient_uniforms") == hipSuccess) ctx->quotient_uniform_fns[key] = uni;
  else (void)hipGetLastError();
  API_END
}

int zkm_ctx_register_perm_kernel(zkm_ctx* ctx, const uint32_t* lookups, uint32_t lookups_len, uint32_t log_quotient_degree,
                                 const void* code_object, size_t code_object_len) {
  API_BEGIN
  std::lock_guard<std::mutex> lk(ctx->mu);
  HIP_CHECK(hipSetDevice(ctx->device));
  CallScope call_scope(ctx);
  if (lookups_len < 2 || !code_object_len) throw std::runtime_error("empty lookups blob or code object");
  std::vector<char> copy((const char*)code_object, (const char*)code_object + code_object_len);
  hipModule_t mod;
  HIP_CHECK(hipModuleLoadData(&mod, copy.data()));
  hipFunction_t fn;
  if (hipModuleGetFunction(&fn, mod, "zkm_perm_rows_specialized") != hipSuccess) {
    (void)hipModuleUnload(mod);
    throw std::runtime_error("code object lacks zkm_perm_rows_specialized");
  }
  ctx->modules.push_back(mod);
  ctx->perm_fns[perm_key(lookups, lookups_len, log_quotient_degree)] = fn;
  API_END
}

void* zkm_host_alloc(zkm_ctx* ctx, size_t bytes) {
  std::lock_guard<std::mutex> lk(ctx->mu);
  void* p = nullptr;
  if (hipSetDevice(ctx->device) != hipSuccess) return nullptr;
  if (hipHostMalloc(&p, bytes ? bytes : 1, hipHostMallocDefault) != hipSuccess) return nullptr;
  return p;
}
void zkm_host_free(zkm_ctx* ctx, void* p) {
  if (!p) return;
  std::lock_guard<std::mutex> lk(ctx->mu);
  (void)hipSetDevice(ctx->device);
  (void)hipHostFree(p);
}

// ... 465 lines not shown
```

Before: 9.235.

## Skip known-zero quotients, drop constant columns, and shortcut padded trace tails

Trace matrices now record how many real rows they hold, and the opening step uses that to evaluate only real rows. The padded tail is folded in through precomputed weight sums and the last-row value. Columns marked constant are removed from the compact column lists, and their contribution is subtracted once from the opening values rather than read per row. Chips with uniform rows and no preprocessed trace or local sum get a zero-filled quotient instead of a constraint evaluation. This adds several kernels and relies on assumptions that padded rows repeat the last row and that uniform chips have a zero quotient, which risks wrong proofs if either assumption fails.

```diff
diff --git a/ziren_amd/csrc/api_tracegen.hpp b/ziren_amd/csrc/api_tracegen.hpp
--- a/ziren_amd/csrc/api_tracegen.hpp
+++ b/ziren_amd/csrc/api_tracegen.hpp
@@ -89,6 +89,7 @@
   const size_t w = (size_t)tracegen::chip_width(chip);
   zkm_matrix* m = b.matrix(height, w);
   m->uniform_rows = n_events == 0 && !n_dev && !dev_events_given;
+  if (!n_dev) { m->real_rows = known::real_rows_of(n_events, height); m->tail_no_lookups = true; }
   const size_t event_bytes = 4 * (size_t)tracegen::event_words(chip);
   const uint32_t* dev_events = dev_events_given ? dev_events_given : b.events(events, n_events * event_bytes);
   uint32_t* counts = blu ? blu->counts : nullptr;
@@ -170,6 +171,7 @@
   }
   zkm_matrix* m = b.matrix(height, width);
   m->uniform_rows = n_words == 0;
+  m->real_rows = known::real_rows_of(rows, height);
   const uint32_t* dev = n_words ? b.events(words, n_words * 4) : nullptr;
   ctx->flush_staged();
   hipLaunchKernelGGL(open::flat_rows, dim3(div_up(width, 32), div_up(height, 32)), dim3(32, 8), 0, ctx->stream, dev, n_words, m->d, width, height);
@@ -228,6 +230,8 @@
   const size_t height = padded_trace_rows(n_events, fixed_log2_rows, "zkm_tracegen_cpu");
   const size_t pheight = program_mults_out ? padded_trace_rows(n_instr, program_fixed_log2_rows, "zkm_tracegen_cpu (program)") : 0;
   zkm_matrix* m = b.matrix(height, tracegen::CPU_WIDTH);
+  m->real_rows = known::real_rows_of(n_events, height);
+  m->tail_no_lookups = true;
   zkm_matrix* pm = program_mults_out ? b.matrix(pheight, 1) : nullptr;
   if (pm) HIP_CHECK(hipMemsetAsync(pm->d, 0, pheight * 4, ctx->stream));
   const uint32_t* dev_events = b.events(events, n_events * sizeof(zkm_cpu_event));
diff --git a/ziren_amd/csrc/host_ctx.hpp b/ziren_amd/csrc/host_ctx.hpp
--- a/ziren_amd/csrc/host_ctx.hpp
+++ b/ziren_amd/csrc/host_ctx.hpp
@@ -134,7 +134,10 @@
   int kernel_timing = 2;
   bool lde_overlap = !(getenv("ZKM_LDE_OVERLAP") && atoi(getenv("ZKM_LDE_OVERLAP")) == 0);
   bool rows_up_front = !(getenv("ZKM_ROWS_UP_FRONT") && atoi(getenv("ZKM_ROWS_UP_FRONT")) == 0);
-  bool root_poll = !(getenv("ZKM_ROOT_POLL") && atoi(getenv("ZKM_ROOT_POLL")) == 0);
+  bool skip_uniform_quotient = !(getenv("ZKM_SKIP_UNIFORM_QUOTIENT") && atoi(getenv("ZKM_SKIP_UNIFORM_QUOTIENT")) == 0);
+  bool open_drop_constant = !(getenv("ZKM_OPEN_DROP_CONSTANT") && atoi(getenv("ZKM_OPEN_DROP_CONSTANT")) == 0);
+  bool tail_rows = !(getenv("ZKM_TAIL_ROWS") && atoi(getenv("ZKM_TAIL_ROWS")) == 0);
+  bool root_poll =!(getenv("ZKM_ROOT_POLL") && atoi(getenv("ZKM_ROOT_POLL")) == 0);
   int root_spin_before_yield = getenv("ZKM_ROOT_SPIN") ? atoi(getenv("ZKM_ROOT_SPIN")) : 4096;
   int root_sleep_ns = getenv("ZKM_ROOT_SLEEP_NS") ? atoi(getenv("ZKM_ROOT_SLEEP_NS")) : 0;
   bool host_wait_blocking = getenv("ZKM_HOST_WAIT") && !strcmp(getenv("ZKM_HOST_WAIT"), "blocking");
@@ -462,6 +465,8 @@
   size_t h = 0, w = 0;
   bool owned = true;
   bool uniform_rows = false;
+  size_t real_rows = 0;
+  bool tail_no_lookups = false;
   hipEvent_t ready = nullptr;
 };
 
@@ -493,6 +498,7 @@
   int log_blowup = 1;
   uint32_t* cflags = nullptr;
   std::vector<const uint32_t*> col_flags;
+  std::vector<size_t> real_rows;
 };
 
 struct zkm_pk : Handle<H_PK> {
diff --git a/ziren_amd/csrc/host_open.hpp b/ziren_amd/csrc/host_open.hpp
--- a/ziren_amd/csrc/host_open.hpp
+++ b/ziren_amd/csrc/host_open.hpp
@@ -20,6 +20,8 @@
   int n_points;
   std::vector<E4> y[2];
   size_t col0 = 0;
+  int job = -1;
+  size_t real = 0;
 };
 struct Round { const zkm_pcs_data* data; std::vector<RoundMat> mats; };
 
@@ -187,6 +189,11 @@
   const uint32_t** col_ptr_lde = nullptr;
   const uint32_t** col_ptr_eval = nullptr;
   uint32_t* col_mask = nullptr;
+  uint32_t* col_word = nullptr;
+  const uint32_t** list_lde = nullptr;
+  const uint32_t** list_eval = nullptr;
+  uint32_t* list_idx = nullptr;
+  uint32_t* list_count = nullptr;
   std::vector<E4*> layers;
   std::vector<Tree> ftrees;
   std::vector<std::array<uint32_t, 8>> commits;
@@ -243,6 +250,7 @@
       pt.h = c.n; pt.w = (size_t)c.perm_ext_w * 4;
       pt.d = ctx->alloc_n<uint32_t>(std::max<size_t>(pt.h * pt.w, 1));
       scratch.push_back(pt.d);
+      pt.real_rows = known::perm_real_rows(md->traces[i].real_rows, md->traces[i].tail_no_lookups, c.desc->prep_index);
       if (c.perm_ext_w > 0) {
         const uint32_t* prep = c.desc->prep_index >= 0 ? pk->prep[c.desc->prep_index].d : nullptr;
         launch_permutation_trace(ctx, c, (const uint32_t*)d_blobs[i], (const uint32_t*)md->traces[i].d, prep, perm_ch[0], (const E4*)d_bp, pt,
@@ -301,6 +309,21 @@
     size_t nchunks = (size_t)1 << lqd;
     uint32_t* qbuf = ctx->alloc_n<uint32_t>(Q * 4);
     scratch.push_back(qbuf);
+    if (known::quotient_is_zero(ctx->skip_uniform_quotient, md->traces[i].uniform_rows, d->prep_index, local_sums[i])) {
+      launches.push_back([this, qbuf, Q]() {
+        KLAUNCH(ctx, "quotient", 16.0 * Q, open::zero_quads, dim3(div_up(Q, open::THREADS)), dim3(open::THREADS), 0, (uint4*)qbuf, Q);
+      });
+      const uint32_t w_q = kb::two_adic_generator(lq);
+      uint32_t wqp = kb::ONE;
+      for (size_t k = 0; k < nchunks; k++) {
+        zkm_matrix m; m.h = c.n; m.w = 4; m.d = qbuf + k * 4 * c.n; m.owned = (k == 0);
+        m.uniform_rows = true;
+        qchunks.push_back(m);
+        qshifts.push_back(kb::mul(kb::GEN, wqp));
+        wqp = kb::mul(wqp, w_q);
+      }
+      continue;
+    }
     size_t C = d->num_constraints;
     std::vector<E4> ap(std::max<size_t>(C, 1));
     E4 p = kb::eone();
@@ -420,6 +443,8 @@
         if (m.width == 0) continue;
         const size_t idx = (size_t)(m.lde - r.data->ldes.data());
         const uint32_t* cf = idx < r.data->col_flags.size() ? r.data->col_flags[idx] : nullptr;
+        m.job = (int)cjobs.size();
+        m.real = ctx->tail_rows && idx < r.data->real_rows.size() ? r.data->real_rows[idx] : 0;
         cjobs.push_back(open::ColJob{m.lde->d, m.evals, cf, m.lde->h, m.n, (uint32_t)total, (uint32_t)m.width});
         total += m.width;
       }
@@ -427,11 +452,19 @@
     col_ptr_lde = (const uint32_t**)salloc(tn * sizeof(void*));
     col_ptr_eval = (const uint32_t**)salloc(tn * sizeof(void*));
     col_mask = (uint32_t*)salloc(tn * sizeof(uint32_t));
-    uint32_t* cword = (uint32_t*)salloc(tn * 8 * sizeof(uint32_t));
+    col_word = (uint32_t*)salloc(tn * 8 * sizeof(uint32_t));
     if (total) {
       const open::ColJob* d_c = (const open::ColJob*)ctx->upload_staged(cjobs.data(), cjobs.size() * sizeof(open::ColJob), &scratch);
       KLAUNCH(ctx, "col_tables", 0.0, open::build_col_tables, dim3(div_up(total, 256)), dim3(256), 0, d_c, (int)cjobs.size(), (uint32_t)total, col_ptr_lde,
-              col_ptr_eval, col_mask, cword);
+              col_ptr_eval, col_mask, col_word);
+      if (ctx->open_drop_constant) {
+        list_lde = (const uint32_t**)salloc(tn * sizeof(void*));
+        list_eval = (const uint32_t**)salloc(tn * sizeof(void*));
+        list_idx = (uint32_t*)salloc(tn * sizeof(uint32_t));
+        list_count = (uint32_t*)salloc(cjobs.size() * sizeof(uint32_t));
+        KLAUNCH(ctx, "col_tables", 0.0, open::compact_col_tables, dim3(cjobs.size()), dim3(64), 0, d_c, (const uint32_t* const*)col_ptr_lde,
+                (const uint32_t* const*)col_ptr_eval, (const uint32_t*)col_mask, list_lde, list_eval, list_idx, list_count);
+      }
     }
   }
   {
@@ -442,8 +475,18 @@
     std::vector<open::WeightJob> wjobs;
     std::vector<open::EvalJob> ejobs;
     std::vector<open::SumJob> sjobs;
-    uint32_t wblk = 0, eblk = 0, sblk = 0;
-    double wbytes = 0, ebytes = 0;
+    std::vector<open::TailWeightJob> twjobs;
+    std::vector<open::TailJob> tjobs;
+    std::map<std::tuple<size_t, uint32_t, size_t>, std::pair<E4*, int>> tcache;
+    uint32_t wblk = 0, eblk = 0, sblk = 0, tblk = 0;
+    double wbytes = 0, ebytes = 0, tbytes = 0;
+    E4* tail_parts = nullptr;
+    size_t tail_parts_used = 0;
+    if (ctx->tail_rows) {
+      size_t cap = 1;
+      for (auto& r : rounds) for (auto& m : r.mats) if (m.width) cap += div_up(m.n, (size_t)open::TAIL_CHUNK);
+      tail_parts = (E4*)salloc(cap * sizeof(E4));
+    }
     size_t ypos = 0;
     for (auto& r : rounds)
       for (auto& m : r.mats) {
@@ -466,11 +509,16 @@
         } else wts = it->second;
         open::EvalJob ej;
         ej.mat = m.evals; ej.weights = wts; ej.n = m.n; ej.width = (int)m.width;
-        ej.colptr = col_ptr_eval + m.col0; ej.colmask = col_mask + m.col0;
+        if (list_count) {
+          ej.colptr = list_eval + m.col0; ej.colmask = nullptr; ej.idx = list_idx + m.col0; ej.ncols = list_count + m.job;
+        } else {
+          ej.colptr = col_ptr_eval + m.col0; ej.colmask = col_mask + m.col0; ej.idx = nullptr; ej.ncols = nullptr;
+        }
+        ej.rows = known::eval_rows(ctx->tail_rows, m.n, m.real);
         ej.groups = (int)div_up(m.width, open::EVAL_COLS);
         ej.split = 1;
         if (m.n >= 4 * open::THREADS) {
-          ej.split = (int)std::min<size_t>(std::max<size_t>(1, 3072 / ej.groups), m.n / (4 * open::THREADS));
+          ej.split = (int)std::min<size_t>(std::max<size_t>(1, 3072 / ej.groups), std::max<size_t>(1, ej.rows / (4 * open::THREADS)));
           ej.kind = m.n_points > 1 ? 1 : 0;
         } else {
           ej.kind = m.n_points > 1 ? 3 : 2;
@@ -482,21 +530,43 @@
           ej.lead = open::EVAL_XCD_AWARE | lead;
           eblk += lead;
         }
-        ej.partials = (E4*)salloc((size_t)ej.split * m.width * 2 * sizeof(E4));
+        const bool tail = ej.rows < m.n;
+        const size_t split_cap = m.n >= 4 * open::THREADS ? std::min<size_t>(std::max<size_t>(1, 3072 / ej.groups), m.n / (4 * open::THREADS)) : 1;
+        ej.partials = (E4*)salloc((split_cap + (ctx->tail_rows ? 1 : 0)) * m.width * 2 * sizeof(E4));
         eblk += (uint32_t)ej.groups * (uint32_t)ej.split;
         ej.blk_end = eblk;
         ejobs.push_back(ej);
-        ebytes += 4.0 * m.n * m.width + 16.0 * m.n;
+        ebytes += 4.0 * ej.rows * m.width + 16.0 * ej.rows;
+        if (tail) {
+          auto tkey = std::make_tuple(m.n, m.shift, ej.rows);
+          auto tit = tcache.find(tkey);
+          if (tit == tcache.end()) {
+            const uint32_t blocks = (uint32_t)div_up(m.n - ej.rows, (size_t)open::TAIL_CHUNK);
+            E4* parts = tail_parts + tail_parts_used;
+            tail_parts_used += blocks;
+            tblk += blocks;
+            twjobs.push_back(open::TailWeightJob{wts, m.n, ej.rows, parts, tblk, 0});
+            tbytes += 16.0 * (m.n - ej.rows);
+            tit = tcache.emplace(tkey, std::make_pair(parts, (int)blocks)).first;
+          }
+          tjobs.push_back(open::TailJob{ej.colptr, ej.colmask, ej.idx, ej.ncols, wts, tit->second.first, ej.partials + (size_t)ej.split * m.width * 2, m.n,
+                                        (int)m.width, tit->second.second, m.n_points > 1 ? 1 : 0, 0});
+        }
         sblk += (uint32_t)(m.width * 2);
-        sjobs.push_back(open::SumJob{ej.partials, ej.split, (int)(m.width * 2), (uint32_t)ypos, sblk});
+        sjobs.push_back(open::SumJob{ej.partials, ej.split + (tail ? 1 : 0), (int)(m.width * 2), (uint32_t)ypos, sblk,
+                                     list_count ? col_mask + m.col0 : nullptr, list_count ? col_word + 8 * m.col0 : nullptr});
         ypos += m.width * 2;
       }
     if (!ejobs.empty()) {
       const open::WeightJob* d_w = (const open::WeightJob*)ctx->upload_staged(wjobs.data(), wjobs.size() * sizeof(open::WeightJob), &scratch);
       const open::EvalJob* d_e = (const open::EvalJob*)ctx->upload_staged(ejobs.data(), ejobs.size() * sizeof(open::EvalJob), &scratch);
       const open::SumJob* d_s = (const open::SumJob*)ctx->upload_staged(sjobs.data(), sjobs.size() * sizeof(open::SumJob), &scratch);
+      const open::TailWeightJob* d_tw = tjobs.empty() ? nullptr : (const open::TailWeightJob*)ctx->upload_staged(twjobs.data(), twjobs.size() * sizeof(open::TailWeightJob), &scratch);
+      const open::TailJob* d_t = tjobs.empty() ? nullptr : (const open::TailJob*)ctx->upload_staged(tjobs.data(), tjobs.size() * sizeof(open::TailJob), &scratch);
       KLAUNCH(ctx, "bary_weights", wbytes, open::bary_weights_batch, dim3(wblk), dim3(open::THREADS), 0, d_w);
+      if (!tjobs.empty()) KLAUNCH(ctx, "bary_weights", tbytes, open::tail_weight_sums, dim3(tblk), dim3(open::THREADS), 0, d_tw);
       KLAUNCH(ctx, "eval_columns", ebytes, open::eval_columns_batch, dim3(eblk), dim3(open::THREADS), 0, d_e);
+      if (!tjobs.empty()) KLAUNCH(ctx, "eval_columns", 0.0, open::eval_tails_batch, dim3(tjobs.size()), dim3(open::THREADS), 0, d_t);
       KLAUNCH(ctx, "reduce_partials", 0.0, open::reduce_partials_batch, dim3(sblk), dim3(64), 0, d_s, d_y);
     }
     const E4* hy = ctx->download_async(d_y, std::max<size_t>(total_y, 1));
@@ -533,6 +603,8 @@
   E4* d_fap = (E4*)ctx->upload_staged(fap.data(), fap.size() * sizeof(E4), &scratch);
   {
     std::vector<std::vector<open::ReduceMat>> per_h(32);
+    std::vector<std::vector<open::DropJob>> drops(32);
+    std::vector<int> y_slot(32, -1);
     std::vector<size_t> off(32, 0);
     std::vector<std::array<E4, 2>> Y(32, {kb::ezero(), kb::ezero()});
     for (auto& r : rounds)
@@ -541,6 +613,11 @@
         open::ReduceMat rm;
         rm.lde = m.lde->d; rm.width = (int)m.width; rm.n_points = m.n_points;
         rm.colptr = col_ptr_lde + m.col0; rm.colmask = col_mask + m.col0;
+        rm.aidx = nullptr; rm.ncols = nullptr;
+        if (list_count && m.width) {
+          rm.colptr = list_lde + m.col0; rm.aidx = list_idx + m.col0; rm.ncols = list_count + m.job;
+          drops[lh].push_back(open::DropJob{(uint32_t)m.col0, (uint32_t)m.width, (uint32_t)m.n_points, (uint32_t)off[lh]});
+        }
         rm.apow_off = (uint32_t)off[lh]; rm.pad = 0;
         rm.A1 = fap[m.width];
         for (int pt = 0; pt < m.n_points; pt++) {
@@ -554,6 +631,27 @@
     std::vector<open::ReduceMat*> d_rms(32, nullptr);
     for (int lh = 0; lh < 32; lh++)
       if (!per_h[lh].empty()) d_rms[lh] = (open::ReduceMat*)ctx->upload_staged(per_h[lh].data(), per_h[lh].size() * sizeof(open::ReduceMat), &scratch);
+    E4* d_Y = nullptr;
+    if (list_count) {
+      std::vector<open::DropJob> djobs;
+      std::vector<open::DropHeight> dheights;
+      std::vector<E4> y_in;
+      for (int lh = 0; lh < 32; lh++) {
+        if (per_h[lh].empty()) continue;
+        y_slot[lh] = (int)dheights.size();
+        const uint32_t job0 = (uint32_t)djobs.size();
+        djobs.insert(djobs.end(), drops[lh].begin(), drops[lh].end());
+        dheights.push_back(open::DropHeight{job0, (uint32_t)djobs.size()});
+        y_in.push_back(Y[lh][0]); y_in.push_back(Y[lh][1]);
+      }
+      if (djobs.empty()) djobs.push_back(open::DropJob{0, 0, 1, 0});
+      const open::DropJob* d_dj = (const open::DropJob*)ctx->upload_staged(djobs.data(), djobs.size() * sizeof(open::DropJob), &scratch);
+      const open::DropHeight* d_dh = (const open::DropHeight*)ctx->upload_staged(dheights.data(), dheights.size() * sizeof(open::DropHeight), &scratch);
+      const E4* d_yin = (const E4*)ctx->upload_staged(y_in.data(), y_in.size() * sizeof(E4), &scratch);
+      d_Y = (E4*)salloc(y_in.size() * sizeof(E4));
+      KLAUNCH(ctx, "col_tables", 0.0, open::drop_constant_terms, dim3(dheights.size()), dim3(64), 0, d_dj, d_dh, (const uint32_t*)col_mask,
+              (const uint32_t*)col_word, (const E4*)d_fap, d_yin, d_Y);
+    }
     for (int lh = 0; lh < 32; lh++) {
       if (per_h[lh].empty()) continue;
       size_t N = (size_t)1 << lh;
@@ -564,9 +662,14 @@
       for (auto& rm : per_h[lh]) rbytes += 4.0 * N * rm.width;
       std::pair<const uint32_t*, const uint32_t*> pw{nullptr, nullptr};
       if (lh >= 12) pw = ctx->pow_tables(lh);
-      KLAUNCH(ctx, "reduce_openings", rbytes, open::reduce_openings, dim3(div_up(N, open::THREADS)), dim3(open::THREADS), 0,
-              (const open::ReduceMat*)d_rm, (int)per_h[lh].size(), lh, (const E4*)d_fap, Y[lh][0], Y[lh][1], zeta, z1, kb::two_adic_generator(lh),
-              pw.first, pw.second, ro[lh]);
+      if (d_Y)
+        KLAUNCH(ctx, "reduce_openings", rbytes, open::reduce_openings<true>, dim3(div_up(N, open::THREADS)), dim3(open::THREADS), 0,
+                (const open::ReduceMat*)d_rm, (int)per_h[lh].size(), lh, (const E4*)d_fap, Y[lh][0], Y[lh][1], (const E4*)(d_Y + 2 * y_slot[lh]), zeta, z1,
+                kb::two_adic_generator(lh), pw.first, pw.second, ro[lh]);
+      else
+        KLAUNCH(ctx, "reduce_openings", rbytes, open::reduce_openings<false>, dim3(div_up(N, open::THREADS)), dim3(open::THREADS), 0,
+                (const open::ReduceMat*)d_rm, (int)per_h[lh].size(), lh, (const E4*)d_fap, Y[lh][0], Y[lh][1], (const E4*)nullptr, zeta, z1,
+                kb::two_adic_generator(lh), pw.first, pw.second, ro[lh]);
     }
   }
   ctx->mark("open: reduced openings");
diff --git a/ziren_amd/csrc/host_pcs.hpp b/ziren_amd/csrc/host_pcs.hpp
--- a/ziren_amd/csrc/host_pcs.hpp
+++ b/ziren_amd/csrc/host_pcs.hpp
@@ -341,6 +341,7 @@
       d->evals.push_back(m.d);
       d->eval_heights.push_back(m.h);
       d->domain_shifts.push_back(shifts.empty() ? kb::ONE : shifts[i]);
+      d->real_rows.push_back(m.real_rows);
     }
     auto shift_of = [&](size_t i) { return kb::mul(kb::GEN, kb::inv(d->domain_shifts[i])); };
     size_t flag_words = 0;
diff --git a/ziren_amd/csrc/known_values.hpp b/ziren_amd/csrc/known_values.hpp
--- /dev/null
+++ b/ziren_amd/csrc/known_values.hpp
@@ -0,0 +1,31 @@
+#pragma once
+#include <stddef.h>
+#include "kb31.cuh"
+
+namespace known {
+
+inline bool quotient_is_zero(bool enabled, bool uniform_rows, int prep_index, const kb::E4& local_sum) {
+  return enabled && uniform_rows && prep_index < 0 && kb::eq(local_sum, kb::ezero());
+}
+
+inline size_t real_rows_of(size_t rows, size_t height) {
+  const size_t r = rows ? rows : 1;
+  return r < height ? r : 0;
+}
+
+inline size_t perm_real_rows(size_t main_real_rows, bool tail_no_lookups, int prep_index) {
+  return tail_no_lookups && prep_index < 0 ? main_real_rows : 0;
+}
+
+inline size_t eval_rows(bool enabled, size_t n, size_t real_rows) {
+  if (!enabled || real_rows == 0 || real_rows >= n) return n;
+  const size_t l = (real_rows + 3) & ~(size_t)3;
+  return l < n ? l : n;
+}
+
+KB_HD void tail_terms(const kb::E4& W, const kb::E4& w_last, uint32_t v_pad, uint32_t v_0, kb::E4& t0, kb::E4& t1) {
+  t0 = kb::escale(W, v_pad);
+  t1 = kb::eadd(kb::escale(kb::esub(W, w_last), v_pad), kb::escale(w_last, v_0));
+}
+
+}
diff --git a/ziren_amd/csrc/open.cuh b/ziren_amd/csrc/open.cuh
--- a/ziren_amd/csrc/open.cuh
+++ b/ziren_amd/csrc/open.cuh
@@ -30,17 +30,44 @@
   }
 }
 
+__global__ __launch_bounds__(64) void compact_col_tables(const ColJob* __restrict__ jobs, const uint32_t* const* __restrict__ lde_ptr,
+                                                         const uint32_t* const* __restrict__ eval_ptr, const uint32_t* __restrict__ mask,
+                                                         const uint32_t** __restrict__ c_lde, const uint32_t** __restrict__ c_eval,
+                                                         uint32_t* __restrict__ c_idx, uint32_t* __restrict__ count) {
+  const ColJob J = jobs[blockIdx.x];
+  const uint32_t lane = threadIdx.x;
+  uint32_t cnt = 0;
+  for (uint32_t base = 0; base < J.width; base += 64) {
+    const uint32_t c = base + lane;
+    const bool keep = c < J.width && mask[J.col0 + c] != 0;
+    const uint64_t kept = __ballot(keep);
+    if (keep) {
+      const size_t pos = (size_t)J.col0 + cnt + __popcll(kept & (((uint64_t)1 << lane) - 1));
+      c_lde[pos] = lde_ptr[J.col0 + c];
+      c_eval[pos] = eval_ptr[J.col0 + c];
+      c_idx[pos] = c;
+    }
+    cnt += (uint32_t)__popcll(kept);
+  }
+  if (lane == 0) count[blockIdx.x] = cnt;
+}
+
 struct WeightJob { kb::E4 u, c; uint32_t w_n, blk_end; size_t n; kb::E4* out; };
 struct EvalJob {
   const uint32_t* mat; const kb::E4* weights; kb::E4* partials;
   const uint32_t* const* colptr; const uint32_t* colmask;
+  const uint32_t* idx; const uint32_t* ncols;
   size_t n;
+  size_t rows;
   int width, groups, split, kind;
   uint32_t blk_end;
   uint32_t lead;
 };
 constexpr uint32_t EVAL_XCD_AWARE = 0x100;
-struct SumJob { const kb::E4* partials; int split, count; uint32_t out0, blk_end; };
+struct SumJob {
+  const kb::E4* partials; int split, count; uint32_t out0, blk_end;
+  const uint32_t* dropmask; const uint32_t* cword;
+};
 template <class J>
 __device__ __forceinline__ const J& find_job(const J* __restrict__ jobs, uint32_t& local) {
   uint32_t j = 0, start = 0;
@@ -84,8 +111,8 @@
 constexpr int EVAL_COLS = 4;
 
 constexpr int EVAL_WORDS = EVAL_COLS * 8;
-__device__ __forceinline__ void block_reduce_store(kb::E4 (&acc)[EVAL_COLS][2], int c0, int width, kb::E4* __restrict__ partials,
-                                                   uint32_t* lds , uint32_t by) {
+__device__ __forceinline__ void block_reduce_store(kb::E4 (&acc)[EVAL_COLS][2], int c0, int cnt, const uint32_t* __restrict__ idx, int width,
+                                                   kb::E4* __restrict__ partials, uint32_t* lds , uint32_t by) {
   const int tid = threadIdx.x;
 #pragma unroll
   for (int c = 0; c < EVAL_COLS; c++)
@@ -109,27 +136,36 @@
 #pragma unroll
     for (int k = 0; k < 8; k++) t = kb::add(t, seg[tid * 8 + k]);
     const int c = tid >> 3, pt = (tid >> 2) & 1, e = tid & 3;
-    if (c0 + c < width) partials[((size_t)by * width + c0 + c) * 2 + pt].c[e] = t;
-  }
-}
+    if (c0 + c < cnt) {
+      const uint32_t col = idx ? gp::load(idx + c0 + c) : (uint32_t)(c0 + c);
+      partials[((size_t)by * width + col) * 2 + pt].c[e] = t;
+    }
+  }
+}
+__device__ __forceinline__ int listed_columns(const uint32_t* __restrict__ ncols, int width) { return ncols ? (int)gp::load(ncols) : width; }
 
 template <bool TWO>
-__device__ __forceinline__ void eval_columns_body(const uint32_t* const* __restrict__ colptr, const uint32_t* __restrict__ colmask, size_t n, int width,
-                                                  const kb::E4* __restrict__ weights,
-                                                  kb::E4* __restrict__ partials, uint32_t* red, uint32_t bx, uint32_t by, uint32_t ny) {
+__device__ __forceinline__ void eval_columns_body(const EvalJob& j, uint32_t* red, uint32_t bx, uint32_t by) {
+  const uint32_t* const* __restrict__ colptr = j.colptr;
+  const uint32_t* __restrict__ colmask = j.colmask;
+  const kb::E4* __restrict__ weights = j.weights;
+  const size_t n = j.n, rows = j.rows;
+  const uint32_t ny = (uint32_t)j.split;
   const int c0 = bx * EVAL_COLS;
+  const int cnt = listed_columns(j.ncols, j.width);
+  if (c0 >= cnt) return;
   const uint32_t* cols[EVAL_COLS];
   uint32_t msk[EVAL_COLS];
 #pragma unroll
   for (int c = 0; c < EVAL_COLS; c++) {
-    cols[c] = gp::load(colptr + min(c0 + c, width - 1));
-    msk[c] = gp::load(colmask + min(c0 + c, width - 1));
+    cols[c] = gp::load(colptr + min(c0 + c, cnt - 1));
+    msk[c] = colmask ? gp::load(colmask + min(c0 + c, cnt - 1)) : 0xffffffffu;
   }
   kb::E4 acc[EVAL_COLS][2];
 #pragma unroll
   for (int c = 0; c < EVAL_COLS; c++) { acc[c][0] = kb::ezero(); acc[c][1] = kb::ezero(); }
   const size_t stride = (size_t)ny * THREADS * 4;
-  for (size_t r = ((size_t)by * THREADS + threadIdx.x) * 4; r < n; r += stride) {
+  for (size_t r = ((size_t)by * THREADS + threadIdx.x) * 4; r < rows; r += stride) {
     kb::E4 w[4];
     uint4 v[EVAL_COLS];
     uint32_t vnext[EVAL_COLS];
@@ -154,28 +190,32 @@
       }
     }
   }
-  block_reduce_store(acc, c0, width, partials, red, by);
-}
-
-__device__ __forceinline__ void eval_columns_small_body(const uint32_t* const* __restrict__ colptr, const uint32_t* __restrict__ colmask, size_t n, int width,
-                                                        const kb::E4* __restrict__ weights,
-                                                        int two_points, kb::E4* __restrict__ partials, uint32_t* red, uint32_t bx) {
+  block_reduce_store(acc, c0, cnt, j.idx, j.width, j.partials, red, by);
+}
+
+__device__ __forceinline__ void eval_columns_small_body(const EvalJob& j, int two_points, uint32_t* red, uint32_t bx) {
+  const uint32_t* const* __restrict__ colptr = j.colptr;
+  const uint32_t* __restrict__ colmask = j.colmask;
+  const kb::E4* __restrict__ weights = j.weights;
+  const size_t n = j.n, rows = j.rows;
   const int c0 = bx * EVAL_COLS;
+  const int cnt = listed_columns(j.ncols, j.width);
+  if (c0 >= cnt) return;
   kb::E4 acc[EVAL_COLS][2];
 #pragma unroll
   for (int c = 0; c < EVAL_COLS; c++) { acc[c][0] = kb::ezero(); acc[c][1] = kb::ezero(); }
-  for (size_t r = threadIdx.x; r < n; r += THREADS) {
+  for (size_t r = threadIdx.x; r < rows; r += THREADS) {
     kb::E4 w = weights[r];
     size_t rn = r + 1 == n ? 0 : r + 1;
 #pragma unroll
     for (int c = 0; c < EVAL_COLS; c++) {
-      const uint32_t* col = colptr[min(c0 + c, width - 1)];
-      const uint32_t mk = colmask[min(c0 + c, width - 1)];
+      const uint32_t* col = colptr[min(c0 + c, cnt - 1)];
+      const uint32_t mk = colmask ? colmask[min(c0 + c, cnt - 1)] : 0xffffffffu;
       acc[c][0] = kb::eadd(acc[c][0], kb::escale(w, col[(uint32_t)r & mk]));
       if (two_points) acc[c][1] = kb::eadd(acc[c][1], kb::escale(w, col[(uint32_t)rn & mk]));
     }
   }
-  block_reduce_store(acc, c0, width, partials, red, 0);
+  block_reduce_store(acc, c0, cnt, j.idx, j.width, j.partials, red, 0);
 }
 __global__ __launch_bounds__(THREADS) void eval_columns_batch(const EvalJob* __restrict__ jobs) {
   __shared__ uint32_t red[EVAL_WORDS * THREADS + EVAL_WORDS * 8];
@@ -190,9 +230,61 @@
     bx = s % (uint32_t)j.groups;
     by = (s / (uint32_t)j.groups) * 8 + x;
   }
-  if (j.kind == 0) eval_columns_body<false>(j.colptr, j.colmask, j.n, j.width, j.weights, j.partials, red, bx, by, (uint32_t)j.split);
-  else if (j.kind == 1) eval_columns_body<true>(j.colptr, j.colmask, j.n, j.width, j.weights, j.partials, red, bx, by, (uint32_t)j.split);
-  else eval_columns_small_body(j.colptr, j.colmask, j.n, j.width, j.weights, j.kind == 3, j.partials, red, bx);
+  if (j.kind == 0) eval_columns_body<false>(j, red, bx, by);
+  else if (j.kind == 1) eval_columns_body<true>(j, red, bx, by);
+  else eval_columns_small_body(j, j.kind == 3, red, bx);
+}
+
+constexpr int TAIL_CHUNK = 8192;
+__device__ __forceinline__ kb::E4 block_sum(const kb::E4& mine, uint32_t* lds ) {
+  const int tid = threadIdx.x;
+#pragma unroll
+  for (int e = 0; e < 4; e++) lds[e * THREADS + tid] = mine.c[e];
+  __syncthreads();
+  for (int s = THREADS / 2; s > 0; s >>= 1) {
+    if (tid < s) {
+#pragma unroll
+      for (int e = 0; e < 4; e++) lds[e * THREADS + tid] = kb::add(lds[e * THREADS + tid], lds[e * THREADS + tid + s]);
+    }
+    __syncthreads();
+  }
+  return kb::E4{{lds[0], lds[THREADS], lds[2 * THREADS], lds[3 * THREADS]}};
+}
+struct TailWeightJob { const kb::E4* weights; size_t n, rows; kb::E4* partials; uint32_t blk_end, pad; };
+__global__ __launch_bounds__(THREADS) void tail_weight_sums(const TailWeightJob* __restrict__ jobs) {
+  __shared__ uint32_t red[4 * THREADS];
+  uint32_t bx;
+  const TailWeightJob& j = find_job(jobs, bx);
+  const size_t r0 = j.rows + (size_t)bx * TAIL_CHUNK, r1 = min(r0 + (size_t)TAIL_CHUNK, j.n);
+  kb::E4 acc = kb::ezero();
+  for (size_t r = r0 + threadIdx.x; r < r1; r += THREADS) acc = kb::eadd(acc, gp::load_e4(j.weights + r));
+  const kb::E4 sum = block_sum(acc, red);
+  if (threadIdx.x == 0) j.partials[bx] = sum;
+}
+struct TailJob {
+  const uint32_t* const* colptr; const uint32_t* colmask; const uint32_t* idx; const uint32_t* ncols;
+  const kb::E4* weights; const kb::E4* wparts;
+  kb::E4* out;
+  size_t n;
+  int width, n_wparts, two_points, pad;
+};
+__global__ __launch_bounds__(THREADS) void eval_tails_batch(const TailJob* __restrict__ jobs) {
+  __shared__ uint32_t red[4 * THREADS];
+  const TailJob& j = jobs[blockIdx.x];
+  kb::E4 acc = kb::ezero();
+  for (int s = threadIdx.x; s < j.n_wparts; s += THREADS) acc = kb::eadd(acc, gp::load_e4(j.wparts + s));
+  const kb::E4 W = block_sum(acc, red);
+  const kb::E4 w_last = gp::load_e4(j.weights + (j.n - 1));
+  const int cnt = listed_columns(j.ncols, j.width);
+  for (int c = threadIdx.x; c < cnt; c += THREADS) {
+    const uint32_t* col = gp::load(j.colptr + c);
+    const uint32_t mk = j.colmask ? gp::load(j.colmask + c) : 0xffffffffu;
+    const uint32_t oc = j.idx ? gp::load(j.idx + c) : (uint32_t)c;
+    kb::E4 t0, t1;
+    known::tail_terms(W, w_last, gp::load(col + ((uint32_t)(j.n - 1) & mk)), gp::load(col), t0, t1);
+    gp::store_e4(j.out + 2 * (size_t)oc, t0);
+    gp::store_e4(j.out + 2 * (size_t)oc + 1, j.two_points ? t1 : kb::ezero());
+  }
 }
 
 __device__ __forceinline__ void reduce_partials_body(const kb::E4* __restrict__ partials, int split, int count, kb::E4* __restrict__ out, int i) {
@@ -210,6 +302,10 @@
 __global__ __launch_bounds__(64) void reduce_partials_batch(const SumJob* __restrict__ jobs, kb::E4* __restrict__ out) {
   uint32_t i;
   const SumJob& j = find_job(jobs, i);
+  if (j.dropmask && gp::load(j.dropmask + (i >> 1)) == 0) {
+    if (threadIdx.x == 0) out[j.out0 + i] = kb::efrom(gp::load(j.cword + 8 * (size_t)(i >> 1)));
+    return;
+  }
   reduce_partials_body(j.partials, j.split, j.count, out + j.out0, (int)i);
 }
 
@@ -228,10 +324,43 @@
   uint32_t apow_off;
   uint32_t pad;
   kb::E4 A1;
+  const uint32_t* aidx; const uint32_t* ncols;
 };
 
+struct DropJob { uint32_t col0, width, n_points, apow_off; };
+struct DropHeight { uint32_t job0, job1; };
+__global__ __launch_bounds__(64) void drop_constant_terms(const DropJob* __restrict__ jobs, const DropHeight* __restrict__ heights,
+                                                          const uint32_t* __restrict__ mask, const uint32_t* __restrict__ cword,
+                                                          const kb::E4* __restrict__ alpha_pows, const kb::E4* __restrict__ y_in,
+                                                          kb::E4* __restrict__ y_out) {
+  const DropHeight H = heights[blockIdx.x];
+  kb::E4 acc[2] = {kb::ezero(), kb::ezero()};
+  for (uint32_t jb = H.job0; jb < H.job1; jb++) {
+    const DropJob J = jobs[jb];
+    for (uint32_t c = threadIdx.x; c < J.width; c += 64) {
+      if (mask[J.col0 + c] != 0) continue;
+      const uint32_t w = cword[8 * (size_t)(J.col0 + c)];
+      acc[0] = kb::eadd(acc[0], kb::escale(alpha_pows[J.apow_off + c], w));
+      if (J.n_points > 1) acc[1] = kb::eadd(acc[1], kb::escale(alpha_pows[J.apow_off + J.width + c], w));
+    }
+  }
+#pragma unroll
+  for (int pt = 0; pt < 2; pt++)
+#pragma unroll
+    for (int e = 0; e < 4; e++) {
+      uint32_t v = acc[pt].c[e];
+#pragma unroll
+      for (int d = 32; d > 0; d >>= 1) v = kb::add(v, __shfl_xor(v, d));
+      acc[pt].c[e] = v;
+    }
+  if (threadIdx.x == 0)
+    for (int pt = 0; pt < 2; pt++) y_out[2 * blockIdx.x + pt] = kb::esub(y_in[2 * blockIdx.x + pt], acc[pt]);
+}
+
+template <bool COMPACT>
 __global__ __launch_bounds__(THREADS) void reduce_openings(const ReduceMat* __restrict__ mats, int n_mats, int log_N,
-                                                           const kb::E4* __restrict__ alpha_pows, kb::E4 Y0, kb::E4 Y1, kb::E4 z0, kb::E4 z1,
+                                                           const kb::E4* __restrict__ alpha_pows, kb::E4 Y0, kb::E4 Y1, const kb::E4* __restrict__ yp,
+                                                           kb::E4 z0, kb::E4 z1,
                                                            uint32_t w_N, const uint32_t* __restrict__ pw_lo, const uint32_t* __restrict__ pw_hi,
                                                            kb::E4* __restrict__ ro) {
   size_t N = (size_t)1 << log_N;
@@ -256,27 +385,31 @@
     typedef const uint32_t __attribute__((address_space(4)))* MaskTable;
     const PtrTable cp = (PtrTable)(uint64_t)M.colptr;
     const MaskTable cm = (MaskTable)(uint64_t)M.colmask;
+    const MaskTable ai = (MaskTable)(uint64_t)M.aidx;
+    const int cols = COMPACT ? (M.ncols ? (int)*(MaskTable)(uint64_t)M.ncols : 0) : M.width;
 #else
     const uint32_t* const* cp = M.colptr;
     const uint32_t* cm = M.colmask;
+    const uint32_t* ai = M.aidx;
+    const int cols = COMPACT ? (M.ncols ? (int)*M.ncols : 0) : M.width;
 #endif
     int c = 0;
-    for (; c + 8 <= M.width; c += 8) {
+    for (; c + 8 <= cols; c += 8) {
       uint32_t v[8];
 #pragma unroll
-      for (int k = 0; k < 8; k++) v[k] = load_row(cp[c + k], roff & cm[c + k]);
+      for (int k = 0; k < 8; k++) v[k] = load_row(cp[c + k], COMPACT ? roff : roff & cm[c + k]);
 #pragma unroll
       for (int k = 0; k < 8; k++) {
-        const kb::E4 a = ap[c + k];
+        const kb::E4 a = ap[COMPACT ? (int)ai[c + k] : c + k];
         kb::acc96_fma_uniform(s0, a.c[0], v[k]);
         kb::acc96_fma_uniform(s1, a.c[1], v[k]);
         kb::acc96_fma_uniform(s2, a.c[2], v[k]);
         kb::acc96_fma_uniform(s3, a.c[3], v[k]);
       }
     }
-    for (; c < M.width; c++) {
-      const kb::E4 a = ap[c];
-      const uint32_t v = load_row(cp[c], roff & cm[c]);
+    for (; c < cols; c++) {
+      const kb::E4 a = ap[COMPACT ? (int)ai[c] : c];
+      const uint32_t v = load_row(cp[c], COMPACT ? roff : roff & cm[c]);
       kb::acc96_fma_uniform(s0, a.c[0], v);
       kb::acc96_fma_uniform(s1, a.c[1], v);
       kb::acc96_fma_uniform(s2, a.c[2], v);
@@ -289,8 +422,9 @@
     T0 = kb::eadd(T0, S);
     if (M.n_points > 1) { T1 = kb::eadd(T1, kb::emul(M.A1, S)); two = true; }
   }
-  kb::E4 acc = kb::emul(kb::esub(Y0, T0), d0);
-  if (two) acc = kb::eadd(acc, kb::emul(kb::esub(Y1, T1), d1));
+  const kb::E4 y0 = COMPACT ? yp[0] : Y0, y1 = COMPACT ? yp[1] : Y1;
+  kb::E4 acc = kb::emul(kb::esub(y0, T0), d0);
+  if (two) acc = kb::eadd(acc, kb::emul(kb::esub(y1, T1), d1));
   ro[r] = acc;
 }
 
@@ -332,6 +466,11 @@
   if (i < count) dst[i] = *src[i];
 }
 
+__global__ __launch_bounds__(THREADS) void zero_quads(uint4* __restrict__ dst, size_t quads) {
+  const size_t i = (size_t)blockIdx.x * blockDim.x + threadIdx.x;
+  if (i < quads) gp::store(dst + i, make_uint4(0u, 0u, 0u, 0u));
+}
+
 __global__ void transpose(const uint32_t* __restrict__ in, uint32_t* __restrict__ out, size_t rows, size_t cols) {
   __shared__ uint32_t tile[32][33];
   size_t bx = (size_t)blockIdx.x * 32, by = (size_t)blockIdx.y * 32;
diff --git a/ziren_amd/csrc/zkm_hip.hip b/ziren_amd/csrc/zkm_hip.hip
--- a/ziren_amd/csrc/zkm_hip.hip
+++ b/ziren_amd/csrc/zkm_hip.hip
@@ -16,6 +16,7 @@
 #include <numeric>
 #include <stdexcept>
 #include <string>
+#include <tuple>
 #include <unordered_map>
 #include <exception>
 #include <vector>
@@ -29,6 +30,7 @@
 #include "lde.cuh"
 #include "merkle.cuh"
 #include "stark.cuh"
+#include "known_values.hpp"
 #include "open.cuh"
 #include "tracegen.cuh"
 
```

Result: faster. 22.52, median of 6 (+143.9%).
